# folkol/query-engines

Measured on AMD Instinct MI355X. Metric: rows/sec filter+project+group-by over 1B-row Arrow batch; % HBM roofline, higher is better.
Workload: dtype int64; 1 GPU; C4: SELECT k, SUM(a+b), COUNT(*), MIN(a), MAX(b) WHERE a > 2^19 GROUP BY k; rows_per_gpu=1000000000, groups=1024, columns=k, a, b int64 (Arrow, no nulls), parallelism=hash-sharded partial aggregate x1

## Files before the change

### include/qe_hip.h

```cpp
#ifndef QE_HIP_H
#define QE_HIP_H

#include <stddef.h>
#include <stdint.h>

#ifdef __cplusplus
extern "C" {
#endif

#define QE_ABI_VERSION 1

#define QE_OK 0
#define QE_ERR_INVALID_ARG (-1)
#define QE_ERR_UNSUPPORTED (-2)
#define QE_ERR_OOM (-3)
#define QE_ERR_DEVICE (-4)
#define QE_ERR_CAPACITY (-5)
#define QE_ERR_COMM (-6)
#define QE_NEED_EXACT 1

#define QE_TYPE_INT64 1
#define QE_TYPE_FLOAT64 2
#define QE_TYPE_BOOL 3
#define QE_TYPE_UTF8 4
#define QE_TYPE_INT32 5
#define QE_TYPE_UINT8 6
#define QE_TYPE_DATE32 7

typedef struct qe_column {
  int32_t type;
  int32_t max_len;
  int64_t length;
  uint8_t* validity;
  void* values;
  int32_t* offsets;
} qe_column;

typedef struct qe_scalar {
  int32_t type;
  int32_t is_null;
  int64_t bits;
} qe_scalar;

typedef struct qe_operand {
  const qe_column* col;
  qe_scalar lit;
} qe_operand;

typedef struct qe_ctx qe_ctx;

int qe_ctx_create(int device, void* stream, qe_ctx** out);
int qe_ctx_create_owned(int device, qe_ctx** out);
int qe_ctx_set_jit(qe_ctx* ctx, int32_t enable);
int qe_ctx_destroy(qe_ctx* ctx);
void* qe_ctx_stream(qe_ctx* ctx);
int qe_ctx_synchronize(qe_ctx* ctx);
const char* qe_last_error(void);
int qe_abi_version(void);

int qe_device_alloc(qe_ctx* ctx, size_t bytes, void** out);
int qe_device_free(qe_ctx* ctx, void* ptr);
int qe_release_cached_memory(int device);
int qe_copy_to_device(qe_ctx* ctx, void* dst, const void* src, size_t bytes);
int qe_copy_to_host(qe_ctx* ctx, void* dst, const void* src, size_t bytes);
int qe_file_to_device(qe_ctx* ctx, const char* path, int64_t offset, int64_t bytes, void* dst);

#define QE_GEN_MOD 1
#define QE_GEN_RAW 2
#define QE_GEN_UNIT53 3
#define QE_GEN_MOD_F64 4
int qe_generate(qe_ctx* ctx, qe_column* out, int32_t dist, int64_t param, uint64_t seed,
                uint64_t col, int64_t row0, int32_t null_permille);

int qe_stream_read(qe_ctx* ctx, const qe_column* cols, int32_t ncols, double* ms);
int qe_stream_read_best(qe_ctx* ctx, const qe_column* cols, int32_t ncols, int32_t reps, double* ms,
                        char* shape, int32_t shape_len);

#define QE_OP_ADD 1
#define QE_OP_SUB 2
#define QE_OP_MUL 3
#define QE_OP_DIV 4
#define QE_OP_EQ 10
#define QE_OP_NE 11
#define QE_OP_LT 12
#define QE_OP_LE 13
#define QE_OP_GT 14
#define QE_OP_GE 15
#define QE_OP_AND 20
#define QE_OP_OR 21
#define QE_OP_NOT 22
#define QE_OP_IS_NULL 23
#define QE_OP_IS_NOT_NULL 24

int qe_eval_arith(qe_ctx* ctx, int32_t op, const qe_operand* lhs, const qe_operand* rhs,
                  qe_column* out);

int qe_eval_cmp(qe_ctx* ctx, int32_t op, const qe_operand* lhs, const qe_operand* rhs,
                qe_column* out);

int qe_eval_bool(qe_ctx* ctx, int32_t op, const qe_column* lhs, const qe_column* rhs,
                 qe_column* out);

int qe_cast_utf8_to_f64(qe_ctx* ctx, const qe_column* in, qe_column* out, int64_t* error_row);

int qe_filter_count(qe_ctx* ctx, const qe_column* mask, int64_t* out_count);
int qe_filter_apply(qe_ctx* ctx, const qe_column* mask, const qe_column* inputs,
                    int32_t ncols, qe_column* outs, int64_t* out_count);
int qe_filter_apply_async(qe_ctx* ctx, const qe_column* mask, const qe_column* inputs,
                          int32_t ncols, qe_column* outs, int64_t* d_count);
int qe_eval_arith_dlen(qe_ctx* ctx, int32_t op, const qe_operand* lhs, const qe_operand* rhs,
                       qe_column* out, const int64_t* d_len);

#define QE_SORT_DESC 1
#define QE_SORT_NULLS_FIRST 2
int qe_sort_indices(qe_ctx* ctx, const qe_column* keys, const int32_t* flags, int32_t nkeys,
                    int64_t limit, qe_column* out_indices);
int qe_take(qe_ctx* ctx, const qe_column* indices, const qe_column* inputs, int32_t ncols,
            qe_column* outs, const int64_t* utf8_capacity);
int qe_sort_layout(int32_t* tile_rows, int32_t* small_max);

#define QE_JOIN_INNER 0
#define QE_JOIN_LEFT  1
typedef struct qe_join qe_join;

int qe_join_build(qe_ctx* ctx, const qe_column* key, qe_join** out);
int qe_join_destroy(qe_join* j);
int qe_join_probe(qe_join* j, const qe_column* key, int32_t kind,
                  qe_column* probe_idx, qe_column* build_idx, int64_t* pairs);
int qe_join_probe_mask(qe_join* j, const qe_column* key, int32_t anti, qe_column* mask);
int qe_join_stats(qe_join* j, int64_t* build_rows, int64_t* distinct, int64_t* max_dup, int64_t* slots);
int qe_take_or_null(qe_ctx* ctx, const qe_column* indices, const qe_column* inputs, int32_t ncols,
                    qe_column* outs, const int64_t* utf8_capacity);

#define QE_AGG_SUM 1
#define QE_AGG_MIN 2
#define QE_AGG_MAX 3
#define QE_AGG_COUNT 4
#define QE_AGG_COUNT_STAR 5
#define QE_AGG_AVG 6

typedef struct qe_global_agg {
  int64_t rows;
  int64_t count;
  int32_t type;
  int32_t valid;
  int64_t sum;
  int64_t min;
  int64_t max;
  double avg;
} qe_global_agg;
int qe_agg_global(qe_ctx* ctx, const qe_column* col, const qe_column* mask ,
                  qe_global_agg* out);
#define QE_GLOBAL_PARTIAL_BYTES 128
#define QE_GLOBAL_EXACT_BYTES 320
int qe_agg_global_partial(qe_ctx* ctx, const qe_column* col, const qe_column* mask ,
                          int64_t row_base, void* partial);
int qe_agg_global_merge(qe_ctx* ctx, int32_t type, const void* partials, int32_t n, qe_global_agg* out);
int qe_agg_global_exact_partial(qe_ctx* ctx, const qe_column* col, const qe_column* mask ,
                                void* words);
int qe_agg_global_merge_exact(qe_ctx* ctx, const void* words, int32_t n, qe_global_agg* out);

#define QE_MAX_KEYS 4
#define QE_MAX_AGGS 8
#define QE_MAX_COLS 8
#define QE_MAX_TERMS 8
#define QE_MAX_TOKENS 16

typedef struct qe_agg_desc {
  int32_t fn;
  int32_t input_type;
} qe_agg_desc;

typedef struct qe_hashagg qe_hashagg;
typedef struct qe_strdict qe_strdict;

int qe_hashagg_create(qe_ctx* ctx, int32_t nkeys, const int32_t* key_types, int32_t naggs,
                      const qe_agg_desc* aggs, int64_t expected_groups, qe_hashagg** out);
#define QE_HASHAGG_DETERMINISTIC 1
#define QE_HASHAGG_FAST_FP64 2
int qe_hashagg_create_ex(qe_ctx* ctx, int32_t nkeys, const int32_t* key_types, int32_t naggs,
                         const qe_agg_desc* aggs, int64_t expected_groups, int32_t flags, qe_hashagg** out);
int qe_hashagg_destroy(qe_hashagg* agg);
int qe_hashagg_reset(qe_hashagg* agg);

int qe_hashagg_update(qe_hashagg* agg, const qe_column* keys, const qe_column* agg_inputs,
                      const qe_column* mask);

#define QE_TOK_COL 1
#define QE_TOK_LIT 2
#define QE_TOK_ADD 3
#define QE_TOK_SUB 4
#define QE_TOK_MUL 5
#define QE_TOK_DIV 6

typedef struct qe_pred_term {
  int32_t col;
  int32_t op;
  int32_t rhs_col;
  int32_t reserved;
  qe_scalar lit;
} qe_pred_term;

typedef struct qe_token {
  int32_t op;
  int32_t arg;
  qe_scalar lit;
} qe_token;

typedef struct qe_agg_program {
  int32_t ntokens;
  int32_t reserved;
  qe_token tokens[QE_MAX_TOKENS];
} qe_agg_program;

typedef struct qe_fused_spec {
  int32_t mask_col;
  int32_t nterms;
  qe_pred_term terms[QE_MAX_TERMS];
  int32_t key_cols[QE_MAX_KEYS];
  qe_agg_program inputs[QE_MAX_AGGS];
} qe_fused_spec;

int qe_hashagg_update_fused(qe_hashagg* agg, const qe_column* cols, int32_t ncols,
                            const qe_fused_spec* spec);

typedef struct qe_select_spec {
  int32_t mask_col;
  int32_t nterms;
  qe_pred_term terms[QE_MAX_TERMS];
  int32_t nout;
  int32_t reserved;
  qe_agg_program outputs[QE_MAX_AGGS];
} qe_select_spec;
int qe_select_project(qe_ctx* ctx, const qe_column* cols, int32_t ncols, const qe_select_spec* spec,
                      qe_column* outs, int64_t* out_count);
typedef struct qe_select_pending qe_select_pending;
int qe_select_project_async(qe_ctx* ctx, const qe_column* cols, int32_t ncols, const qe_select_spec* spec,
                            qe_column* outs, qe_select_pending** pending);
int qe_select_pending_wait(qe_select_pending* pending, int64_t* out_count);
#define QE_SELECT_SCHEME_RESIDENT 1
#define QE_SELECT_SCHEME_TWOPASS 2
#define QE_SELECT_SCHEME_SCANNED 3
#define QE_SELECT_SCHEME_LOOKBACK_PERSISTENT 4
#define QE_SELECT_SCHEME_LOOKBACK_COUNTER 5
typedef struct qe_select_layout {
  int32_t scheme;
  int32_t staged;
  int32_t block;
  int32_t reserved;
  int64_t tile_rows;
  int64_t tiles;
  int64_t group_rows;
} qe_select_layout;
int qe_select_project_layout(qe_ctx* ctx, const qe_column* cols, int32_t ncols, const qe_select_spec* spec,
                             const qe_column* outs, qe_select_layout* out);

int qe_hashagg_num_groups(qe_hashagg* agg, int64_t* out);
int qe_hashagg_finalize(qe_hashagg* agg, qe_column* out_keys, qe_column* out_aggs,
                        int64_t* out_groups);
int qe_hashagg_finalize_sizes(qe_hashagg* agg, int64_t* groups, int64_t* key_bytes);
int qe_hashagg_key_bytes_bound(qe_hashagg* agg, int32_t key, int64_t* per_group);

int qe_hashagg_record_bytes(qe_hashagg* agg, int64_t* out);
int qe_hashagg_export_counts(qe_hashagg* agg, int32_t nparts, int64_t* counts);
int qe_hashagg_export(qe_hashagg* agg, int32_t nparts, void* dst);
int qe_hashagg_import(qe_hashagg* agg, const void* records, int64_t nrecords);

#define QE_KEYED_HEADER 128
int qe_hashagg_export_keyed_sizes(qe_hashagg* agg, int32_t nparts, int64_t* block_bytes);
int qe_hashagg_export_keyed(qe_hashagg* agg, int32_t nparts, void* dst);
int qe_hashagg_import_keyed(qe_hashagg* agg, const void* blocks, int32_t nblocks, const int64_t* block_bytes);
int qe_hashagg_merge(qe_hashagg* dst, qe_hashagg* src);
int qe_hashagg_bind_key_dict(qe_hashagg* agg, int32_t key, qe_strdict* dict);
int qe_hashagg_key_layout(qe_hashagg* agg, int32_t* dictionary_keyed, int32_t* device_nkeys, int32_t* device_types);

#define QE_SLOT_HEADER 64
int qe_hashagg_export_slots(qe_hashagg* agg, int32_t nparts, int64_t slot_records, void* dst);
int qe_hashagg_import_slots(qe_hashagg* agg, const void* slots, int32_t nslots, int64_t slot_records,
                            int64_t* max_count, int64_t* nrecords);
int qe_hashagg_slot_capacity(qe_hashagg* agg, int32_t world, int64_t* slot_records);

int qe_hashagg_set_async(qe_hashagg* agg, int32_t enable);

#define QE_COMM_ID_BYTES 128
typedef struct qe_comm qe_comm;
int qe_comm_unique_id(void* id );
int qe_comm_create(qe_ctx* ctx, int32_t world, int32_t rank, const void* id, qe_comm** out);
int qe_comm_destroy(qe_comm* comm);
int qe_comm_loopback_hub_create(int32_t world, void** hub);
int qe_comm_loopback_hub_destroy(void* hub);
int qe_comm_create_loopback(qe_ctx* ctx, int32_t world, int32_t rank, void* hub, qe_comm** out);
int qe_hashagg_exchange(qe_comm* comm, qe_hashagg* partial, qe_hashagg* owner, int64_t slot_records,
                        int64_t* nrecords);

int qe_hashagg_set_row_base(qe_hashagg* agg, int64_t row_base);

int qe_hashagg_last_kernel_time(qe_hashagg* agg, double* ms, int32_t* launches);
int qe_hashagg_last_kernel_signature(qe_hashagg* agg, uint64_t* sig);
int qe_hashagg_last_kernel_kind(qe_hashagg* agg, int32_t* specialized, char* note, int32_t note_len);
int qe_hashagg_last_chunk_stats(qe_hashagg* agg, int64_t* chunks, int64_t* full_chunks, int64_t* records);

int qe_strdict_create(qe_ctx* ctx, int64_t expected_distinct, qe_strdict** out);
int qe_strdict_destroy(qe_strdict* dict);
int qe_strdict_size(qe_strdict* dict, int64_t* out);
int qe_strdict_encode(qe_strdict* dict, const qe_column* in, qe_column* codes);
int qe_strdict_decode_bytes(qe_strdict* dict, const qe_column* codes, int64_t* out_bytes);
int qe_strdict_decode(qe_strdict* dict, const qe_column* codes, qe_column* out);
int qe_strdict_decode_trusted(qe_strdict* dict, const qe_column* codes, qe_column* out);
int qe_strdict_encode_packed(qe_ctx* ctx, const qe_column* in, qe_column* codes);
int qe_strdict_decode_packed(qe_ctx* ctx, const qe_column* codes, qe_column* out);
int qe_strdict_encode_tuple(qe_strdict* dict, const qe_column* keys, int32_t nkeys, qe_column* codes);
int qe_strdict_decode_tuple(qe_strdict* dict, const qe_column* codes, int32_t nkeys, qe_column* outs);
int qe_hash_partition(qe_ctx* ctx, const qe_column* cols, int32_t ncols, int32_t nparts, int32_t* part);

#ifndef ARROW_C_DATA_INTERFACE
#define ARROW_C_DATA_INTERFACE
#define ARROW_FLAG_DICTIONARY_ORDERED 1
#define ARROW_FLAG_NULLABLE 2
#define ARROW_FLAG_MAP_KEYS_SORTED 4
struct ArrowSchema {
  const char* format;
  const char* name;
  const char* metadata;
  int64_t flags;
  int64_t n_children;
  struct ArrowSchema** children;
  struct ArrowSchema* dictionary;
  void (*release)(struct ArrowSchema*);
  void* private_data;
};
struct ArrowArray {
  int64_t length;
  int64_t null_count;
  int64_t offset;
  int64_t n_buffers;
  int64_t n_children;
  const void** buffers;
  struct ArrowArray** children;
  struct ArrowArray* dictionary;
  void (*release)(struct ArrowArray*);
  void* private_data;
};
#endif
#ifndef ARROW_C_DEVICE_DATA_INTERFACE
#define ARROW_C_DEVICE_DATA_INTERFACE
typedef int32_t ArrowDeviceType;
struct ArrowDeviceArray {
  struct ArrowArray array;
  int64_t device_id;
  ArrowDeviceType device_type;
  void* sync_event;
  int64_t reserved[3];
};
#endif
#define QE_ARROW_DEVICE_CPU 1
#define QE_ARROW_DEVICE_ROCM 10
typedef struct ArrowSchema ArrowSchema;
typedef struct ArrowArray ArrowArray;
typedef struct ArrowDeviceArray ArrowDeviceArray;

typedef struct qe_batch qe_batch;
int qe_batch_import(qe_ctx* ctx, const ArrowSchema* schema, const ArrowArray* array, qe_batch** out);
int qe_batch_import_device(qe_ctx* ctx, const ArrowSchema* schema, const ArrowDeviceArray* array,
                           qe_batch** out);
int qe_batch_destroy(qe_batch* batch);
int qe_batch_num_columns(const qe_batch* batch, int32_t* ncols, int64_t* length);
int qe_batch_column(const qe_batch* batch, int32_t i, qe_column* out, const char** name);
int qe_batch_export(qe_ctx* ctx, const qe_column* cols, int32_t ncols, const char* const* names,
                    ArrowSchema* out_schema, ArrowArray* out_array);

typedef struct qe_csv_options {
  int32_t delimiter;
  int32_t has_header;
  int32_t nfields;
  int32_t flags;
  const int32_t* field_index;
} qe_csv_options;
#define QE_CSV_PARTIAL_TAIL 1
typedef struct qe_csv_table qe_csv_table;
int qe_csv_parse(qe_ctx* ctx, const uint8_t* data, int64_t nbytes, const qe_csv_options* opt,
                 qe_csv_table** out);
int qe_csv_rows(const qe_csv_table* table, int64_t* rows);
int qe_csv_consumed(const qe_csv_table* table, int64_t* bytes);
int qe_csv_column(const qe_csv_table* table, int32_t i, qe_column* out);
int qe_csv_column_bytes(const qe_csv_table* table, int32_t i, int64_t* nbytes);
int qe_csv_column_copy(const qe_csv_table* table, int32_t i, qe_column* dst);
int qe_csv_column_max_len(const qe_csv_table* table, int32_t i, int64_t* nbytes);
int qe_csv_destroy(qe_csv_table* table);
int qe_csv_record_end(const uint8_t* data, int64_t nbytes, int32_t eof, int64_t* cut);

#ifdef __cplusplus
}
#endif
#endif
```

### query-engines_amd/csrc/qe_comm.hip

```cpp
#include <dlfcn.h>
#include <rccl/rccl.h>
#include <string.h>

#include <condition_variable>
#include <mutex>
#include <string>
#include <type_traits>
#include <vector>

#include "qe_internal.hpp"

namespace {

struct Rccl {
  ncclResult_t (*get_unique_id)(ncclUniqueId*) = nullptr;
  ncclResult_t (*comm_init_rank)(ncclComm_t*, int, ncclUniqueId, int) = nullptr;
  ncclResult_t (*comm_destroy)(ncclComm_t) = nullptr;
  ncclResult_t (*send)(const void*, size_t, ncclDataType_t, int, ncclComm_t, hipStream_t) = nullptr;
  ncclResult_t (*recv)(void*, size_t, ncclDataType_t, int, ncclComm_t, hipStream_t) = nullptr;
  ncclResult_t (*group_start)() = nullptr;
  ncclResult_t (*group_end)() = nullptr;
  const char* (*error_string)(ncclResult_t) = nullptr;
  bool ok = false;
  std::string why;
};

const Rccl& rccl() {
  static Rccl r;
  static std::once_flag once;
  std::call_once(once, [] {
    void* h = nullptr;
    for (const char* name : {"librccl.so.1", "librccl.so"}) {
      h = dlopen(name, RTLD_NOW | RTLD_LOCAL);
      if (h) break;
    }
    if (!h) {
      const char* e = dlerror();
      r.why = e ? e : "librccl.so.1 not found";
      return;
    }
    bool all = true;
    auto sym = [&](auto& fp, const char* name) {
      fp = reinterpret_cast<std::remove_reference_t<decltype(fp)>>(dlsym(h, name));
      all = all && fp != nullptr;
    };
    sym(r.get_unique_id, "ncclGetUniqueId");
    sym(r.comm_init_rank, "ncclCommInitRank");
    sym(r.comm_destroy, "ncclCommDestroy");
    sym(r.send, "ncclSend");
    sym(r.recv, "ncclRecv");
    sym(r.group_start, "ncclGroupStart");
    sym(r.group_end, "ncclGroupEnd");
    sym(r.error_string, "ncclGetErrorString");
    r.ok = all;
    if (!all) r.why = "librccl is missing an entry point";
  });
  return r;
}

#define QE_NCCL(call)                                                                               \
  do {                                                                                              \
    const ncclResult_t qe_r_ = (call);                                                              \
    if (qe_r_ != ncclSuccess)                                                                       \
      return ::qe::fail(QE_ERR_COMM, "%s failed: %s", #call, rccl().error_string(qe_r_));           \
  } while (0)

}

struct qe_loop_hub {
  int32_t world = 0;
  std::mutex mu;
  std::condition_variable cv;
  int32_t arrived = 0;
  uint64_t generation = 0;
  std::vector<const uint8_t*> send;
  std::vector<const size_t*> soff, sbytes;
  std::vector<int> failed;
  void barrier() {
    std::unique_lock<std::mutex> g(mu);
    const uint64_t gen = generation;
    if (++arrived == world) {
      arrived = 0;
      ++generation;
      cv.notify_all();
    } else {
      cv.wait(g, [&] { return generation != gen; });
    }
  }
};

struct qe_comm {
  qe_ctx* ctx = nullptr;
  ncclComm_t comm = nullptr;
  qe_loop_hub* hub = nullptr;
  int32_t world = 0, rank = 0;
  uint8_t* buf = nullptr;
  size_t buf_bytes = 0;
};

using namespace qe;

namespace {

int comm_buffer(qe_comm* c, size_t bytes) {
  if (bytes <= c->buf_bytes) return QE_OK;
  dev_free(c->ctx, c->buf);
  c->buf = nullptr;
  c->buf_bytes = 0;
  QE_TRY(dev_alloc(c->ctx, bytes, (void**)&c->buf));
  c->buf_bytes = bytes;
  return QE_OK;
}

int exchange_bytes(qe_comm* c, const uint8_t* send, const size_t* soff, const size_t* sbytes, uint8_t* recv,
                   const size_t* roff, const size_t* rbytes) {
  if (c->hub) {
    qe_loop_hub* h = c->hub;
    int st = ctx_sync(c->ctx);
    h->send[c->rank] = send;
    h->soff[c->rank] = soff;
    h->sbytes[c->rank] = sbytes;
    h->failed[c->rank] = st != QE_OK;
    h->barrier();
    for (int p = 0; p < c->world && st == QE_OK; ++p)
      if (h->failed[p]) st = fail(QE_ERR_COMM, "loopback exchange: rank %d failed before the exchange", p);
    for (int p = 0; p < c->world && st == QE_OK; ++p) {
      if (h->sbytes[p][c->rank] != rbytes[p])
        st = fail(QE_ERR_COMM, "loopback exchange: rank %d sends %zu bytes to rank %d, which expects %zu", p,
                  h->sbytes[p][c->rank], c->rank, rbytes[p]);
      else if (rbytes[p] && hipMemcpyAsync(recv + roff[p], h->send[p] + h->soff[p][c->rank], rbytes[p],
                                           hipMemcpyDeviceToDevice, c->ctx->stream) != hipSuccess)
        st = fail(QE_ERR_DEVICE, "loopback exchange: copy from rank %d failed", p);
    }
    if (st == QE_OK) st = ctx_sync(c->ctx);
    h->barrier();
    return st;
  }
  const Rccl& R = rccl();
  QE_NCCL(R.group_start());
  ncclResult_t r = ncclSuccess;
  for (int p = 0; p < c->world && r == ncclSuccess; ++p) {
    if (sbytes[p]) r = R.send(send + soff[p], sbytes[p], ncclUint8, p, c->comm, c->ctx->stream);
    if (r == ncclSuccess && rbytes[p]) r = R.recv(recv + roff[p], rbytes[p], ncclUint8, p, c->comm, c->ctx->stream);
  }
  const ncclResult_t e = R.group_end();
  QE_NCCL(r);
  QE_NCCL(e);
  return QE_OK;
}

int exchange_keyed(qe_comm* c, qe_hashagg* partial, qe_hashagg* owner, int64_t* nrecords) {
  const int world = c->world;
  std::vector<int64_t> sb(world), rb(world);
  QE_TRY(qe_hashagg_export_keyed_sizes(partial, world, sb.data()));
  QE_TRY(comm_buffer(c, (size_t)2 * world * 8));
  int64_t* dsz = (int64_t*)c->buf;
  QE_HIP(hipMemcpyAsync(dsz, sb.data(), (size_t)world * 8, hipMemcpyHostToDevice, c->ctx->stream));
  std::vector<size_t> o8(world), l8(world, 8);
  for (int p = 0; p < world; ++p) o8[p] = (size_t)p * 8;
  QE_TRY(exchange_bytes(c, (const uint8_t*)dsz, o8.data(), l8.data(), (uint8_t*)(dsz + world), o8.data(), l8.data()));
  QE_HIP(hipMemcpyAsync(rb.data(), dsz + world, (size_t)world * 8, hipMemcpyDeviceToHost, c->ctx->stream));
  QE_TRY(ctx_sync(c->ctx));
  std::vector<size_t> so(world), sl(world), ro(world), rl(world);
  size_t a = 0, b = 0;
  for (int p = 0; p < world; ++p) {
    so[p] = a;
    sl[p] = (size_t)sb[p];
    a += sl[p];
    ro[p] = b;
    rl[p] = (size_t)rb[p];
    b += rl[p];
  }
  QE_TRY(comm_buffer(c, std::max<size_t>(a + b, 8)));
  uint8_t* send = c->buf;
  uint8_t* recv = c->buf + a;
  QE_TRY(qe_hashagg_export_keyed(partial, world, send));
  QE_TRY(exchange_bytes(c, send, so.data(), sl.data(), recv, ro.data(), rl.data()));
  QE_TRY(qe_hashagg_import_keyed(owner, recv, world, rb.data()));
  if (nrecords) {
    std::vector<int64_t> nrec(world, 0);
    for (int p = 0; p < world; ++p)
      if (rb[p]) QE_HIP(hipMemcpyAsync(&nrec[p], recv + ro[p] + 8, 8, hipMemcpyDeviceToHost, c->ctx->stream));
    QE_TRY(ctx_sync(c->ctx));
    int64_t n = 0;
    for (int64_t x : nrec) n += x;
    *nrecords = n;
  }
  return QE_OK;
}

}

extern "C" {

int qe_comm_unique_id(void* id) {
  QE_CHECK(id, QE_ERR_INVALID_ARG, "null id");
  const Rccl& R = rccl();
  QE_CHECK(R.ok, QE_ERR_COMM, "RCCL unavailable: %s", R.why.c_str());
  static_assert(sizeof(ncclUniqueId) == QE_COMM_ID_BYTES, "unique id size");
  ncclUniqueId u;
  QE_NCCL(R.get_unique_id(&u));
  memcpy(id, &u, sizeof u);
  return QE_OK;
}

int qe_comm_create(qe_ctx* ctx, int32_t world, int32_t rank, const void* id, qe_comm** out) {
  QE_TRY(ctx_enter(ctx));
  QE_CHECK(out && id && world >= 1 && rank >= 0 && rank < world, QE_ERR_INVALID_ARG, "bad arguments");
  const Rccl& R = rccl();
  QE_CHECK(R.ok, QE_ERR_COMM, "RCCL unavailable: %s", R.why.c_str());
  ncclUniqueId u;
  memcpy(&u, id, sizeof u);
  ncclComm_t comm = nullptr;
  QE_NCCL(R.comm_init_rank(&comm, world, u, rank));
  qe_comm* c = new qe_comm();
  c->ctx = ctx;
  c->comm = comm;
  c->world = world;
  c->rank = rank;
  *out = c;
  return QE_OK;
}

int qe_comm_destroy(qe_comm* c) {
  if (!c) return QE_OK;
  (void)hipSetDevice(c->ctx->device);
  (void)hipStreamSynchronize(c->ctx->stream);
  dev_free(c->ctx, c->buf);
  if (c->comm) (void)rccl().comm_destroy(c->comm);
  delete c;
  return QE_OK;
}

int qe_comm_loopback_hub_create(int32_t world, void** hub) {
  QE_CHECK(hub && world >= 1, QE_ERR_INVALID_ARG, "bad arguments");
  qe_loop_hub* h = new qe_loop_hub();
  h->world = world;
  h->send.assign(world, nullptr);
  h->soff.assign(world, nullptr);
  h->sbytes.assign(world, nullptr);
  h->failed.assign(world, 0);
  *hub = h;
  return QE_OK;
}

int qe_comm_loopback_hub_destroy(void* hub) {
  delete (qe_loop_hub*)hub;
  return QE_OK;
}

int qe_comm_create_loopback(qe_ctx* ctx, int32_t world, int32_t rank, void* hub, qe_comm** out) {
  QE_TRY(ctx_enter(ctx));
  qe_loop_hub* h = (qe_loop_hub*)hub;
  QE_CHECK(out && h && world == h->world && rank >= 0 && rank < world, QE_ERR_INVALID_ARG, "bad arguments");
  qe_comm* c = new qe_comm();
  c->ctx = ctx;
  c->hub = h;
  c->world = world;
  c->rank = rank;
  *out = c;
  return QE_OK;
}

int qe_hashagg_slot_capacity(qe_hashagg* h, int32_t world, int64_t* cap) {
  QE_CHECK(h && cap && world >= 1, QE_ERR_INVALID_ARG, "bad arguments");
  int64_t eg = 0;
  QE_TRY(hashagg_expected_groups(h, &eg));
  eg = std::max<int64_t>(eg, 1);
  *cap = std::min<int64_t>(eg, (3 * eg + 2 * world - 1) / (2 * world) + 32);
  return QE_OK;
}

int qe_hashagg_exchange(qe_comm* c, qe_hashagg* partial, qe_hashagg* owner, int64_t slot_records,
                        int64_t* nrecords) {
  QE_CHECK(c && partial && owner, QE_ERR_INVALID_ARG, "null argument");
  QE_TRY(ctx_enter(c->ctx));
  const int world = c->world;
  int64_t rb = 0;
  QE_TRY(qe_hashagg_record_bytes(partial, &rb));
  QE_CHECK(hashagg_ctx(partial) == c->ctx && hashagg_ctx(owner) == c->ctx, QE_ERR_INVALID_ARG,
           "partial, owner and communicator must share one qe_ctx (one stream)");
  if (keyed_dict(hashagg_info(partial).keyed) || keyed_dict(hashagg_info(owner).keyed))
    return exchange_keyed(c, partial, owner, nrecords);
  int64_t cap = slot_records;
  if (cap <= 0) QE_TRY(qe_hashagg_slot_capacity(partial, world, &cap));
  const size_t slot_bytes = (size_t)QE_SLOT_HEADER + (size_t)cap * (size_t)rb;
  QE_TRY(comm_buffer(c, 2 * (size_t)world * slot_bytes));
  uint8_t* send = c->buf;
  uint8_t* recv = c->buf + (size_t)world * slot_bytes;
  QE_TRY(qe_hashagg_export_slots(partial, world, cap, send));
  std::vector<size_t> off(world), len(world, slot_bytes);
  for (int p = 0; p < world; ++p) off[p] = (size_t)p * slot_bytes;
  QE_TRY(exchange_bytes(c, send, off.data(), len.data(), recv, off.data(), len.data()));
  int64_t mx = 0, n = 0;
  QE_TRY(qe_hashagg_import_slots(owner, recv, world, cap, &mx, &n));
  if (mx <= cap) {
    if (nrecords) *nrecords = n;
    return QE_OK;
  }
  std::vector<int64_t> counts(world);
  QE_TRY(qe_hashagg_export_counts(partial, world, counts.data()));
  int64_t total = 0;
  for (int64_t x : counts) total += x;
  QE_TRY(comm_buffer(c, (size_t)2 * world * 8 + (size_t)std::max<int64_t>(total, 1) * rb));
  int64_t* dcnt = (int64_t*)c->buf;
  QE_HIP(hipMemcpyAsync(dcnt, counts.data(), (size_t)world * 8, hipMemcpyHostToDevice, c->ctx->stream));
  std::vector<size_t> o8(world), l8(world, 8);
  for (int p = 0; p < world; ++p) o8[p] = (size_t)p * 8;
  QE_TRY(exchange_bytes(c, (const uint8_t*)dcnt, o8.data(), l8.data(), (uint8_t*)(dcnt + world), o8.data(),
                        l8.data()));
  std::vector<int64_t> rcounts(world);
  QE_HIP(hipMemcpyAsync(rcounts.data(), dcnt + world, (size_t)world * 8, hipMemcpyDeviceToHost, c->ctx->stream));
  QE_TRY(ctx_sync(c->ctx));
  int64_t rtotal = 0;
  for (int64_t x : rcounts) rtotal += x;
  const size_t head = (size_t)2 * world * 8;
  QE_TRY(comm_buffer(c, head + (size_t)(std::max<int64_t>(total, 1) + std::max<int64_t>(rtotal, 1)) * rb));
  uint8_t* srec = c->buf + head;
  uint8_t* rrec = srec + (size_t)std::max<int64_t>(total, 1) * rb;
  QE_TRY(qe_hashagg_export(partial, world, srec));
  std::vector<size_t> so(world), sl(world), ro(world), rl(world);
  size_t a = 0, b = 0;
  for (int p = 0; p < world; ++p) {
    so[p] = a;
    sl[p] = (size_t)counts[p] * rb;
    a += sl[p];
    ro[p] = b;
    rl[p] = (size_t)rcounts[p] * rb;
    b += rl[p];
  }
  QE_TRY(exchange_bytes(c, srec, so.data(), sl.data(), rrec, ro.data(), rl.data()));
  QE_TRY(qe_hashagg_import(owner, rrec, rtotal));
  if (nrecords) *nrecords = rtotal;
  return QE_OK;
}

}
```

### query-engines_amd/csrc/qe_hashagg.hip

```cpp
#include <map>
#include <memory>
#include <mutex>

#include "qe_internal.hpp"

namespace qe {

constexpr int HA_THREADS = 512;

__device__ __forceinline__ qi64* lds_keys(char* smem) { return (qi64*)smem; }

__device__ __forceinline__ void lds_init(const Plan& P, char* smem) {
  const int SS = (1 << P.lds_log2) + 2;
  qi64* keys = lds_keys(smem);
  qu32* cst = (qu32*)(smem + P.off_cstar);
  for (int s = threadIdx.x; s < SS; s += blockDim.x) {
    keys[s] = EMPTY_KEY;
    cst[s] = 0;
  }
#pragma unroll
  for (int j = 0; j < QE_MAX_AGGS; ++j) {
    if (j >= P.naggs) break;
    const DAgg& a = P.aggs[j];
    if (a.acc != ACC_NONE) {
// ... 626 lines not shown
      gadd_cstar(P.t, gs, 1);
      const qu64 row = (qu64)(P.row_base + lr);
      for (int j = 0; j < P.naggs; ++j) {
        const DAgg& a = P.aggs[j];
        if (a.pkind == 0) continue;
        bool valid;
        const qi64 x = a.pkind == 2 ? eval_program<NC>(a, R, r, valid) : eval_fast<NC>(a, R, r, valid);
        if (!valid) continue;
        const RowVal rv = row_partial(a.acc, x, row);
        gcombine(P.t, a.acc, j, gs, rv.acc, 1, rv.i0, rv.i1, rv.i2, rv.i3);
      }
    }
  }
}

template <int NC, bool USE_LDS>
__global__ void __launch_bounds__(HA_THREADS, 4) k_hashagg(const Plan P) {
  extern __shared__ __attribute__((aligned(16))) char smem[];
  if (USE_LDS) {
    lds_init(P, smem);
    __syncthreads();
  }
  const int lane = threadIdx.x & 63;
  const qi64 wave = (blockIdx.x * (qi64)blockDim.x + threadIdx.x) >> 6;
  const qi64 stride = (((qi64)gridDim.x * blockDim.x) >> 6) * 256;
  ColRegs<NC> cur, nxt;
  qi64 base = wave * 256;
  if (base < P.n) load_cols<NC>(P, base, lane, base + 256 <= P.n, cur);
  for (; base < P.n; base += stride) {
    const qi64 nb = base + stride;
    if (nb < P.n) load_cols<NC>(P, nb, lane, nb + 256 <= P.n, nxt);
    process_step<NC, USE_LDS>(P, smem, cur, base, lane);
    cur = nxt;
  }
  if (USE_LDS) {
    __syncthreads();
    lds_flush(P, smem);
  }
}

struct AggMeta {
  qi32 naggs;
  qi32 fn[QE_MAX_AGGS];
  qi32 acc[QE_MAX_AGGS];
  qi32 nn_implicit;
  qi32 any_x;
};

__device__ __forceinline__ qu64 slot_nn(const DTable& t, const AggMeta& m, int j, qu64 s) {
  return ((m.nn_implicit >> j) & 1) ? t.cstar[s] : t.nn[j][s];
}

__global__ void __launch_bounds__(1024) k_part_slices(const qi64* __restrict__ off, qi32 np, qi64 g, qi64 cw,
                                                      qi64* __restrict__ out) {
  __shared__ qi64 s_sum[1024];
  const int per = (np + 1023) / 1024;
  const int b0 = threadIdx.x * per;
  qi64 cnt = 0;
  for (int i = 0; i < per; ++i) {
    const int b = b0 + i;
    if (b < np) cnt += (off[(qi64)(b + 1) * g] - off[(qi64)b * g] + cw - 1) / cw;
  }
  s_sum[threadIdx.x] = cnt;
  __syncthreads();
  for (int d = 1; d < 1024; d <<= 1) {
    const qi64 v = (int)threadIdx.x >= d ? s_sum[threadIdx.x - d] : 0;
    __syncthreads();
    s_sum[threadIdx.x] += v;
    __syncthreads();
  }
  qi64 pos = s_sum[threadIdx.x] - cnt;
  for (int i = 0; i < per; ++i) {
    const int b = b0 + i;
    if (b >= np) break;
    const qi64 s = off[(qi64)b * g], e = off[(qi64)(b + 1) * g];
    const qi64 ns = (e - s + cw - 1) / cw;
    for (qi64 k = 0; k < ns; ++k, ++pos) {
      const qi64 lo = s + k * cw;
      out[2 + 2 * pos] = lo;
      out[3 + 2 * pos] = (lo + cw < e ? lo + cw : e) | (ns == 1 ? PART_EXCL : 0);
    }
  }
  if (threadIdx.x == 1023) out[0] = s_sum[1023];
}

constexpr int CHUNK_PER_WG = 1024;
__global__ void __launch_bounds__(256) k_chunk_hist(const qi64* __restrict__ meta, qi32 np, qu32* __restrict__ cnt,
                                                   unsigned long long* __restrict__ rec) {
  __shared__ qu32 s_cnt[CHUNK_PLAN_MAXB];
  __shared__ unsigned long long s_rec[CHUNK_PLAN_MAXB];
  const qi64 C = meta[0], lo = (qi64)blockIdx.x * CHUNK_PER_WG;
  if (lo >= C) return;
  const qi64 hi = lo + CHUNK_PER_WG < C ? lo + CHUNK_PER_WG : C;
  for (int b = threadIdx.x; b < np; b += blockDim.x) {
    s_cnt[b] = 0;
    s_rec[b] = 0;
  }
  __syncthreads();
  for (qi64 c = lo + threadIdx.x; c < hi; c += blockDim.x) {
    const qi64 w = meta[1 + c];
    if (w < 0) continue;
    const int b = (int)(w >> 32);
    atomicAdd(&s_cnt[b], 1u);
    atomicAdd(&s_rec[b], (unsigned long long)(w & 0xFFFFFFFFll));
  }
  __syncthreads();
  for (int b = threadIdx.x; b < np; b += blockDim.x)
    if (s_cnt[b]) {
      atomicAdd(&cnt[b], s_cnt[b]);
      atomicAdd(&rec[b], s_rec[b]);
    }
}

__global__ void __launch_bounds__(1024) k_chunk_slices(const qi64* __restrict__ meta, qi32 np, qi64 tmax,
                                                      const qu32* __restrict__ cnt,
                                                      const unsigned long long* __restrict__ rec,
                                                      qi64* __restrict__ out, qu32* __restrict__ base) {
  __shared__ qu32 s_a[1024], s_b[1024];
  __shared__ unsigned long long s_r[1024];
  const int t = threadIdx.x;
  const qu32 c = t < np ? cnt[t] : 0u;
  s_r[t] = t < np ? rec[t] : 0ull;
  s_a[t] = c;
  __syncthreads();
  for (int d = 512; d > 0; d >>= 1) {
    if (t < d) {
      s_r[t] += s_r[t + d];
      s_a[t] += s_a[t + d];
    }
    __syncthreads();
  }
  const qi64 C = (qi64)s_a[0], R = (qi64)s_r[0];
  (void)meta;
  __syncthreads();
  const qi64 target = max((qi64)np, min(tmax, R >> 15));
  const qi64 cpc = max((qi64)1, (5 * C + 4 * target - 1) / (4 * target));
  const qu32 ns = (qu32)((c + cpc - 1) / cpc);
  s_a[t] = c;
  s_b[t] = ns;
  __syncthreads();
  for (int d = 1; d < 1024; d <<= 1) {
    const qu32 xa = t >= d ? s_a[t - d] : 0u, xb = t >= d ? s_b[t - d] : 0u;
    __syncthreads();
    s_a[t] += xa;
    s_b[t] += xb;
    __syncthreads();
  }
  if (t < np) {
    const qi64 s0 = s_a[t] - c, e0 = s0 + c, sl = s_b[t] - ns;
    base[t] = (qu32)s0;
    for (qi64 k = 0; k < ns; ++k) {
      const qi64 lo = s0 + k * cpc;
      out[2 + 2 * (sl + k)] = lo;
      out[3 + 2 * (sl + k)] = (lo + cpc < e0 ? lo + cpc : e0) | (ns == 1 ? PART_EXCL : 0);
    }
  }
  if (t == 1023) out[0] = s_b[1023];
}

__global__ void __launch_bounds__(256) k_chunk_place(const qi64* __restrict__ meta, qi32 np,
                                                    const qu32* __restrict__ base, qu32* __restrict__ cur,
                                                    qi32* __restrict__ sorted) {
  constexpr int PER = CHUNK_PER_WG / 256;
  __shared__ qu32 s_cnt[CHUNK_PLAN_MAXB];
  const qi64 C = meta[0], lo = (qi64)blockIdx.x * CHUNK_PER_WG;
  if (lo >= C) return;
  for (int b = threadIdx.x; b < np; b += blockDim.x) s_cnt[b] = 0;
  __syncthreads();
  int bk[PER];
  qu32 rk[PER];
#pragma unroll
  for (int i = 0; i < PER; ++i) {
    const qi64 c = lo + threadIdx.x + 256 * i;
    bk[i] = -1;
    if (c < C && meta[1 + c] >= 0) {
      bk[i] = (int)(meta[1 + c] >> 32);
      rk[i] = atomicAdd(&s_cnt[bk[i]], 1u);
    }
  }
  __syncthreads();
  for (int b = threadIdx.x; b < np; b += blockDim.x)
    if (s_cnt[b]) s_cnt[b] = base[b] + atomicAdd(&cur[b], s_cnt[b]);
  __syncthreads();
#pragma unroll
  for (int i = 0; i < PER; ++i)
    if (bk[i] >= 0) sorted[s_cnt[bk[i]] + rk[i]] = (qi32)(lo + threadIdx.x + 256 * i);
}

__global__ void k_spill_plan(const qi64* __restrict__ meta, qi64 tmax, qi64* __restrict__ out, qi32* __restrict__ sorted) {
  const qi64 C = meta[0];
  const qi64 c = (qi64)blockIdx.x * blockDim.x + threadIdx.x;
  if (c < C) sorted[c] = (qi32)c;
  if (blockIdx.x != 0) return;
  qi64 target = (C * PART_CH) >> 15;
  target = target < 1 ? 1 : (target > tmax ? tmax : target);
  const qi64 cpc = (C + target - 1) / target > 0 ? (C + target - 1) / target : 1;
  const qi64 ns = (C + cpc - 1) / cpc;
  for (qi64 k = threadIdx.x; k < ns; k += blockDim.x) {
    const qi64 lo = k * cpc;
    out[2 + 2 * k] = lo;
    out[3 + 2 * k] = (lo + cpc < C ? lo + cpc : C) | (ns == 1 ? PART_EXCL : 0);
  }
  if (threadIdx.x == 0) out[0] = ns;
}

__global__ void k_table_init(DTable t, AggMeta m, qu64* zero_ctl, int reset) {
  const qu64 SS = t.cap + 2;
  if (zero_ctl && blockIdx.x == 0 && threadIdx.x < 8) zero_ctl[threadIdx.x] = 0;
  for (qu64 s = blockIdx.x * (qu64)blockDim.x + threadIdx.x; s < SS; s += (qu64)gridDim.x * blockDim.x) {
    t.keys[s] = EMPTY_KEY;
    t.cstar[s] = 0;
    for (int j = 0; j < m.naggs; ++j) {
      if (reset && m.acc[j] == ACC_SUM_X && (t.idx[j][3 * SS + s] & FX_EXT))
        for (int w = 0; w < FXE_WORDS; ++w) t.ext[j][s * FXE_WORDS + w] = 0;
      t.acc[j][s] = acc_identity(m.acc[j]);
      t.nn[j][s] = 0;
      if (acc_has_idx(m.acc[j]))
        for (int k = 0; k < 4; ++k) t.idx[j][k * SS + s] = idx_identity(m.acc[j]);
    }
  }
}

__global__ void k_nn_materialize(DTable t, qi32 mask) {
  const qu64 SS = t.cap + 2;
  for (qu64 s = blockIdx.x * (qu64)blockDim.x + threadIdx.x; s < SS; s += (qu64)gridDim.x * blockDim.x)
    for (int j = 0; j < QE_MAX_AGGS; ++j)
      if ((mask >> j) & 1) t.nn[j][s] = t.cstar[s];
}

__device__ __forceinline__ bool gslot_occupied(const DTable& t, qu64 s) {
  return s < t.cap ? t.keys[s] != EMPTY_KEY : t.cstar[s] > 0;
}

__device__ __forceinline__ void wg_newg_begin(qu32* newg) {
  if (threadIdx.x == 0) *newg = 0;
  __syncthreads();
}
__device__ __forceinline__ void wg_newg_end(qu32* newg, qu64* ctl) {
  __syncthreads();
  if (threadIdx.x == 0 && *newg) atomicAdd((unsigned long long*)&ctl[0], (unsigned long long)*newg);
}

__global__ void k_rehash(DTable src, DTable dst, AggMeta m) {
  __shared__ qu32 newg;
  wg_newg_begin(&newg);
  const qu64 SS = src.cap + 2;
  for (qu64 s = blockIdx.x * (qu64)blockDim.x + threadIdx.x; s < SS; s += (qu64)gridDim.x * blockDim.x) {
    if (!gslot_occupied(src, s)) continue;
    const bool knull = s == src.cap;
    const qi64 key = knull ? 0 : (s == src.cap + 1 ? EMPTY_KEY : src.keys[s]);
    qu64 d;
    if (!gtable_find_wg(dst, key, knull, d, &newg)) {
      atomicAdd((unsigned long long*)&dst.ctl[3], 1ull);
      continue;
    }
    gadd_cstar(dst, d, src.cstar[s]);
    for (int j = 0; j < m.naggs; ++j) {
      DAgg a{};
      a.fn = m.fn[j];
      a.acc = m.acc[j];
      qu64 i[4] = {~0ull, ~0ull, ~0ull, ~0ull};
      if (acc_has_idx(a.acc))
        for (int k = 0; k < 4; ++k) i[k] = src.idx[j][k * SS + s];
      gcombine(dst, a.acc, j, d, src.acc[j][s], slot_nn(src, m, j, s), i[0], i[1], i[2], i[3]);
      if (a.acc == ACC_SUM_X && (i[3] & FX_EXT))
        fxe_add_words<true>(dst.ext[j] + d * FXE_WORDS, 0, src.ext[j] + s * FXE_WORDS, FXE_WORDS);
    }
  }
  wg_newg_end(&newg, dst.ctl);
}

__device__ void import_record(const qu8* __restrict__ rec, DTable& dst, const AggMeta& m, qu32* newg) {
  const qi64 key = ((const qi64*)rec)[0];
  const bool knull = ((const qu64*)rec)[1] & 1;
  const qu64 c = ((const qu64*)rec)[2];
  qu64 d;
  if (!gtable_find_wg(dst, key, knull, d, newg)) {
    atomicAdd((unsigned long long*)&dst.ctl[3], 1ull);
    return;
  }
  gadd_cstar(dst, d, c);
  int off = 24;
  for (int j = 0; j < m.naggs; ++j) {
    DAgg a{};
    a.fn = m.fn[j];
    a.acc = m.acc[j];
    const qu64* f = (const qu64*)(rec + off);
    if (a.fn != QE_AGG_COUNT_STAR) {
      if (acc_has_idx(a.acc)) gcombine(dst, a.acc, j, d, (qi64)f[0], f[1], f[2], f[3], f[4], f[5]);
      else gcombine(dst, a.acc, j, d, (qi64)f[0], f[1], ~0ull, ~0ull, ~0ull, ~0ull);
    }
    off += agg_rec_bytes(a.acc);
  }
}

__global__ void k_import(const qu8* __restrict__ recs, qi64 nrec, qi32 rec_bytes, DTable dst, AggMeta m) {
  __shared__ qu32 newg;
  wg_newg_begin(&newg);
  for (qi64 r = blockIdx.x * (qi64)blockDim.x + threadIdx.x; r < nrec; r += (qi64)gridDim.x * blockDim.x)
    import_record(recs + r * rec_bytes, dst, m, &newg);
  wg_newg_end(&newg, dst.ctl);
}

__global__ void k_import_slots(const qu8* __restrict__ slots, qi32 nslots, qi64 slot_records, qi32 rec_bytes,
                               DTable dst, AggMeta m) {
  __shared__ qu32 newg;
  __shared__ qi32 s_ok;
  const qu64 slot_bytes = QE_SLOT_HEADER + (qu64)slot_records * rec_bytes;
  if (threadIdx.x < 64) {
    qu64 mx = 0, tot = 0;
    for (int i = threadIdx.x; i < nslots; i += 64) {
      const qu64* hd = (const qu64*)(slots + (qu64)i * slot_bytes);
      mx = hd[1] > mx ? hd[1] : mx;
      tot += hd[0] < (qu64)slot_records ? hd[0] : (qu64)slot_records;
    }
    for (int off = 32; off > 0; off >>= 1) {
      const qu64 o = __shfl_xor(mx, off);
      mx = o > mx ? o : mx;
      tot += __shfl_xor(tot, off);
    }
    if (threadIdx.x == 0) {
      s_ok = mx <= (qu64)slot_records;
      if (blockIdx.x == 0) {
        dst.ctl[4] = mx;
        dst.ctl[5] = tot;
      }
    }
  }
  wg_newg_begin(&newg);
  if (s_ok) {
    const qi64 total = (qi64)nslots * slot_records;
    for (qi64 r = blockIdx.x * (qi64)blockDim.x + threadIdx.x; r < total; r += (qi64)gridDim.x * blockDim.x) {
      const qi64 sl = r / slot_records, i = r - sl * slot_records;
      const qu8* base = slots + (qu64)sl * slot_bytes;
      if ((qu64)i >= ((const qu64*)base)[0]) continue;
      import_record(base + QE_SLOT_HEADER + (qu64)i * rec_bytes, dst, m, &newg);
    }
  }
  wg_newg_end(&newg, dst.ctl);
}

__device__ __forceinline__ qu32 partition_of(qi64 key, bool knull, qi32 nparts) {
  const qu64 h = fmix64((qu64)key ^ (knull ? NULL_SALT : 0ull));
  return (qu32)(((h >> 32) * (qu64)nparts) >> 32);
}

__device__ __forceinline__ qu64 wave_cursor(unsigned long long* cursor, bool has, qu32 p, qu32 mult = 1) {
  const int lane = threadIdx.x & 63;
  const qu64 lt = lane ? (~0ull >> (64 - lane)) : 0ull;
  qu64 todo = __ballot(has);
  qu64 pos = 0;
  while (todo) {
    const int leader = __ffsll((long long)todo) - 1;
    const qu32 lp = (qu32)__shfl((int)p, leader);
    const qu64 same = __ballot(has && p == lp);
    qu64 base = 0;
    if (lane == leader) base = atomicAdd(&cursor[lp], (unsigned long long)__popcll(same) * mult);
    base = (qu64)__shfl((long long)base, leader);
    if (has && p == lp) pos = base + (qu64)__popcll(same & lt) * mult;
    todo &= ~same;
  }
  return pos;
}

__device__ __forceinline__ bool slot_has_ext(const DTable& t, const AggMeta& m, qu64 s) {
  bool e = false;
  for (int j = 0; j < m.naggs; ++j)
    if (m.acc[j] == ACC_SUM_X) e = e || (t.idx[j][3 * (t.cap + 2) + s] & FX_EXT) != 0;
  return e;
}

__global__ void k_export_count(DTable t, AggMeta m, qi32 nparts, unsigned long long* counts) {
  const qu64 SS = t.cap + 2;
  const qu64 stride = (qu64)gridDim.x * blockDim.x;
  for (qu64 s0 = blockIdx.x * (qu64)blockDim.x; s0 < SS; s0 += stride) {
    const qu64 s = s0 + threadIdx.x;
    const bool has = s < SS && gslot_occupied(t, s);
    const bool knull = s == t.cap;
    const qi64 key = !has ? 0 : knull ? 0 : (s == t.cap + 1 ? EMPTY_KEY : t.keys[s]);
    const qu32 p = has ? partition_of(key, knull, nparts) : 0;
    (void)wave_cursor(counts, has, p);
    if (m.any_x) (void)wave_cursor(counts, has && slot_has_ext(t, m, s), p, FXE_CHUNKS);
  }
}

__device__ void write_record(qu8* rec, const DTable& t, const AggMeta& m, qu64 s, qi64 key, bool knull) {
  const qu64 SS = t.cap + 2;
  write_record_head(rec, key, knull, t.cstar[s]);
  int off = 24;
  for (int j = 0; j < m.naggs; ++j) {
    qu64* f = (qu64*)(rec + off);
    f[0] = (qu64)t.acc[j][s];
    f[1] = slot_nn(t, m, j, s);
    if (acc_has_idx(m.acc[j]))
      for (int k = 0; k < 4; ++k) f[2 + k] = t.idx[j][k * SS + s];
    off += agg_rec_bytes(m.acc[j]);
  }
}

__device__ void write_chunk_record(qu8* rec, const DTable& t, const AggMeta& m, qu64 s, qi64 key, bool knull,
                                   int c) {
  const qu64 SS = t.cap + 2;
  write_record_head(rec, key, knull, 0);
  int off = 24;
  for (int j = 0; j < m.naggs; ++j) {
    qu64* f = (qu64*)(rec + off);
    const int acc = m.acc[j];
    f[0] = (qu64)acc_identity(acc);
    f[1] = 0;
    if (acc_has_idx(acc))
      for (int k = 0; k < 4; ++k) f[2 + k] = idx_identity(acc);
    if (acc == ACC_SUM_X && (t.idx[j][3 * SS + s] & FX_EXT)) {
      const qu64* e = t.ext[j] + s * FXE_WORDS + 4 * c;
      const int n = c == FXE_CHUNKS - 1 ? FXE_WORDS - 4 * c : 4;
      f[0] = e[0];
      for (int k = 1; k < n; ++k) f[1 + k] = e[k];
      f[5] = FX_CHUNK | ((qu64)c << 8);
    }
    off += agg_rec_bytes(acc);
  }
}

__global__ void k_counts_to_cursors(unsigned long long* c, qi32 nparts) {
  if (threadIdx.x == 0) {
    unsigned long long run = 0;
    for (int p = 0; p < nparts; ++p) {
      const unsigned long long x = c[p];
      c[p] = run;
      run += x;
    }
  }
}

__global__ void k_export(DTable t, AggMeta m, qi32 nparts, qi32 rec_bytes, unsigned long long* cursor,
                         qu8* __restrict__ dst) {
  const qu64 SS = t.cap + 2;
  const qu64 stride = (qu64)gridDim.x * blockDim.x;
  for (qu64 s0 = blockIdx.x * (qu64)blockDim.x; s0 < SS; s0 += stride) {
    const qu64 s = s0 + threadIdx.x;
    const bool has = s < SS && gslot_occupied(t, s);
    const bool knull = s == t.cap;
    const qi64 key = !has ? 0 : knull ? 0 : (s == t.cap + 1 ? EMPTY_KEY : t.keys[s]);
    const qu32 p = has ? partition_of(key, knull, nparts) : 0;
    const qu64 pos = wave_cursor(cursor, has, p);
    if (has) write_record(dst + pos * (qu64)rec_bytes, t, m, s, key, knull);
    if (m.any_x) {
      const bool ext = has && slot_has_ext(t, m, s);
      const qu64 pe = wave_cursor(cursor, ext, p, FXE_CHUNKS);
      if (ext)
        for (int c = 0; c < FXE_CHUNKS; ++c) write_chunk_record(dst + (pe + c) * (qu64)rec_bytes, t, m, s, key, knull, c);
    }
  }
}

__global__ void k_export_slots(DTable t, AggMeta m, qi32 nparts, qi32 rec_bytes, qi64 slot_records,
                               unsigned long long* cursor, qu8* __restrict__ dst) {
  const qu64 SS = t.cap + 2;
  const qu64 slot_bytes = QE_SLOT_HEADER + (qu64)slot_records * rec_bytes;
  const qu64 stride = (qu64)gridDim.x * blockDim.x;
  for (qu64 s0 = blockIdx.x * (qu64)blockDim.x; s0 < SS; s0 += stride) {
    const qu64 s = s0 + threadIdx.x;
    const bool has = s < SS && gslot_occupied(t, s);
    const bool knull = s == t.cap;
    const qi64 key = !has ? 0 : knull ? 0 : (s == t.cap + 1 ? EMPTY_KEY : t.keys[s]);
    const qu32 p = has ? partition_of(key, knull, nparts) : 0;
    const qu64 pos = wave_cursor(cursor, has, p);
    qu8* base = dst + p * slot_bytes + QE_SLOT_HEADER;
    if (has && pos < (qu64)slot_records) write_record(base + pos * (qu64)rec_bytes, t, m, s, key, knull);
    if (m.any_x) {
      const bool ext = has && slot_has_ext(t, m, s);
      const qu64 pe = wave_cursor(cursor, ext, p, FXE_CHUNKS);
      if (ext)
        for (int c = 0; c < FXE_CHUNKS; ++c)
          if (pe + c < (qu64)slot_records) write_chunk_record(base + (pe + c) * (qu64)rec_bytes, t, m, s, key, knull, c);
    }
  }
}

__global__ void k_slot_headers(const unsigned long long* __restrict__ cursor, qi32 nparts, qu64 slot_bytes,
                               qu8* __restrict__ dst, const qu64* __restrict__ guard) {
  qu64 mx = 0;
  for (int p = threadIdx.x; p < nparts; p += blockDim.x) mx = cursor[p] > mx ? cursor[p] : mx;
  for (int off = 32; off > 0; off >>= 1) {
    const qu64 o = __shfl_xor(mx, off);
    mx = o > mx ? o : mx;
  }
  if (guard && (guard[1] | guard[2] | guard[3])) mx = 1ull << 62;
  for (int p = threadIdx.x; p < nparts; p += blockDim.x) {
    qu64* hd = (qu64*)(dst + (qu64)p * slot_bytes);
    hd[0] = cursor[p];
    hd[1] = mx;
    for (int w = 2; w < QE_SLOT_HEADER / 8; ++w) hd[w] = 0;
  }
}

__global__ void k_occ_count(DTable t, qi64* __restrict__ tile_counts, qi32 tile_slots) {
  __shared__ qi64 part[4];
  const qu64 SS = t.cap + 2;
  const qu64 s0 = (qu64)blockIdx.x * tile_slots;
  qi64 c = 0;
  for (int i = threadIdx.x; i < tile_slots; i += blockDim.x) {
    const qu64 s = s0 + i;
    if (s < SS && gslot_occupied(t, s)) ++c;
  }
  for (int off = 32; off > 0; off >>= 1) c += __shfl_xor(c, off);
  if ((threadIdx.x & 63) == 0) part[threadIdx.x >> 6] = c;
  __syncthreads();
  if (threadIdx.x == 0) tile_counts[blockIdx.x] = part[0] + part[1] + part[2] + part[3];
}

struct OutCols {
  qe_column keys[QE_MAX_KEYS];
  qe_column aggs[QE_MAX_AGGS];
};

__device__ __forceinline__ void set_bit(qu8* bm, qi64 i, bool v) {
  if (v) atomicOr((qu32*)bm + (i >> 5), 1u << (i & 31));
}

__device__ __forceinline__ void store_typed(void* p, qi32 type, qi64 i, qi64 x) {
  switch (type) {
    case QE_TYPE_INT64:
    case QE_TYPE_FLOAT64: ((qi64*)p)[i] = x; break;
    case QE_TYPE_INT32:
    case QE_TYPE_DATE32: ((qi32*)p)[i] = (qi32)x; break;
    default: ((qu8*)p)[i] = (qu8)x;
  }
}

constexpr int FS_WORDS = 512;
__device__ __forceinline__ void put_bit(qu8* gbm, qu32* lbits, int col, qi64 o, bool v) {
  if (!v) return;
  if (lbits) atomicOr(lbits + col * FS_WORDS + (o >> 5), 1u << (o & 31));
  else set_bit(gbm, o, true);
}

__device__ __forceinline__ double fx_sum(const DTable& t, int j, qu64 s, qi64 acc) {
  const qu64 SS = t.cap + 2;
  const qu64* ix = t.idx[j];
  return fx_result((qu64)acc, ix[s], ix[SS + s], ix[2 * SS + s], ix[3 * SS + s], t.ext[j] + s * FXE_WORDS);
}

__device__ __forceinline__ void finalize_slot(const DTable& t, const AggMeta& m, const KeyMeta& km,
                                              const OutCols& out, qu64 s, qi64 o, qu32* lbits = nullptr) {
  const qu64 SS = t.cap + 2;
  const bool knull = s == t.cap;
  const qi64 key = knull ? 0 : (s == t.cap + 1 ? EMPTY_KEY : t.keys[s]);
  if (km.mode == 1) {
    store_typed(out.keys[0].values, km.type[0], o, key);
    if (out.keys[0].validity) put_bit(out.keys[0].validity, lbits, 0, o, !knull);
  } else if (km.mode == 2) {
    for (int k = 0; k < km.nkeys; ++k) {
      const bool isn = (key >> km.nullbit[k]) & 1;
      qi64 x = (key >> km.shift[k]) & km.fmask[k];
      if (km.type[k] == QE_TYPE_INT32 || km.type[k] == QE_TYPE_DATE32) x = (qi64)(qi32)x;
      store_typed(out.keys[k].values, km.type[k], o, x);
      if (out.keys[k].validity) put_bit(out.keys[k].validity, lbits, k, o, !isn);
    }
  }
  const qu64 cst = t.cstar[s];
#pragma unroll 1
  for (int j = 0; j < m.naggs; ++j) {
    if (!out.aggs[j].values) continue;
    const qu64 nn = slot_nn(t, m, j, s);
    const qi64 acc = t.acc[j][s];
    qi64 val = 0;
    bool valid = nn > 0;
    switch (m.fn[j]) {
      case QE_AGG_COUNT: val = (qi64)nn; valid = true; break;
      case QE_AGG_COUNT_STAR: val = (qi64)cst; valid = true; break;
      case QE_AGG_AVG:
        if (m.acc[j] == ACC_SUM_X)
          val = f64_bits(fx_sum(t, j, s, acc) / (double)nn);
        else
          val = f64_bits(bits_f64(acc) / (double)nn);
        break;
      default:
        if (m.acc[j] == ACC_SUM_X) {
          val = f64_bits(fx_sum(t, j, s, acc));
        } else if (acc_is_f64mm(m.acc[j])) {
          const qu64 i0 = t.idx[j][s], i1 = t.idx[j][SS + s];
          const qu64 i2 = t.idx[j][2 * SS + s], i3 = t.idx[j][3 * SS + s];
          if (i1 != ~0ull && i1 == i0) {
            val = 0x7FF8000000000000ll;
          } else {
            const double d = okey_f64(acc);
            val = d == 0.0 ? f64_bits(i2 < i3 ? -0.0 : 0.0) : f64_bits(d);
          }
        } else {
          val = acc;
        }
    }
    ((qi64*)out.aggs[j].values)[o] = valid ? val : 0;
    if (out.aggs[j].validity) put_bit(out.aggs[j].validity, lbits, QE_MAX_KEYS + j, o, valid);
  }
}

__global__ void k_finalize(DTable t, AggMeta m, KeyMeta km, const qi64* __restrict__ tile_offsets,
                           qi32 tile_slots, OutCols out) {
  __shared__ int wtot[4];
  const qu64 SS = t.cap + 2;
  const int lane = threadIdx.x & 63, wid = threadIdx.x >> 6;
  const qu64 lt = lane ? (~0ull >> (64 - lane)) : 0ull;
  qi64 base = tile_offsets[blockIdx.x];
  for (int it = 0; it < tile_slots; it += blockDim.x) {
    const qu64 s = (qu64)blockIdx.x * tile_slots + it + threadIdx.x;
    const bool occ = (it + (int)threadIdx.x) < tile_slots && s < SS && gslot_occupied(t, s);
    const qu64 b = __ballot(occ);
    if (lane == 0) wtot[wid] = __popcll(b);
    __syncthreads();
    int woff = 0, btot = 0;
    for (int w = 0; w < 4; ++w) {
      woff += w < wid ? wtot[w] : 0;
      btot += wtot[w];
    }
    if (occ) finalize_slot(t, m, km, out, s, base + woff + __popcll(b & lt));
    base += btot;
    __syncthreads();
  }
}

constexpr int FS_THREADS = 1024, FS_PER = 16, FS_WAVES = FS_THREADS / 64;
static_assert(FS_THREADS * FS_PER / 2 / 32 <= FS_WORDS, "LDS bitmaps hold every group of a small table");
__global__ void __launch_bounds__(FS_THREADS) k_finalize_small(DTable t, AggMeta m, KeyMeta km, OutCols out,
                                                               qi64 groups) {
  __shared__ qi32 wcnt[FS_PER][FS_WAVES];
  __shared__ qu64 wbal[FS_PER][FS_WAVES];
  __shared__ qu32 lbits[(QE_MAX_KEYS + QE_MAX_AGGS) * FS_WORDS];
  const qu64 SS = t.cap + 2;
  const int tid = threadIdx.x, lane = tid & 63, wid = tid >> 6;
  const qu64 lt = lane ? (~0ull >> (64 - lane)) : 0ull;
  const int words = (int)((groups + 31) >> 5);
  for (int w = tid; w < (QE_MAX_KEYS + QE_MAX_AGGS) * FS_WORDS; w += FS_THREADS) lbits[w] = 0;
  qu32 occ = 0;
#pragma unroll
  for (int i = 0; i < FS_PER; ++i) {
    const qu64 s = (qu64)i * FS_THREADS + tid;
    if (s < SS && gslot_occupied(t, s)) occ |= 1u << i;
  }
#pragma unroll
  for (int i = 0; i < FS_PER; ++i) {
    const qu64 b = __ballot((occ >> i) & 1);
    if (lane == 0) {
      wbal[i][wid] = b;
      wcnt[i][wid] = __popcll(b);
    }
  }
  __syncthreads();
  static_assert(FS_PER * FS_WAVES == 4 * 64, "four (chunk, wave) counts per lane");
  if (wid == 0) {
    qi32* flat = &wcnt[0][0];
    const qi32 c0 = flat[4 * lane], c1 = flat[4 * lane + 1], c2 = flat[4 * lane + 2], c3 = flat[4 * lane + 3];
    const qi32 sum = c0 + c1 + c2 + c3;
    qi32 inc = sum;
#pragma unroll
    for (int d = 1; d < 64; d <<= 1) {
      const qi32 y = __shfl_up(inc, d);
      if (lane >= d) inc += y;
    }
    const qi32 ex = inc - sum;
    flat[4 * lane] = ex;
    flat[4 * lane + 1] = ex + c0;
    flat[4 * lane + 2] = ex + c0 + c1;
    flat[4 * lane + 3] = ex + c0 + c1 + c2;
  }
  __syncthreads();
  while (occ) {
    const int i = __ffs(occ) - 1;
    occ &= occ - 1;
    const qi64 o = wcnt[i][wid] + __popcll(wbal[i][wid] & lt);
    finalize_slot(t, m, km, out, (qu64)i * FS_THREADS + tid, o, lbits);
  }
  __syncthreads();
  for (int w = tid; w < words; w += FS_THREADS) {
    for (int k = 0; k < QE_MAX_KEYS; ++k)
      if (k < km.nkeys && out.keys[k].validity) ((qu32*)out.keys[k].validity)[w] = lbits[k * FS_WORDS + w];
    for (int j = 0; j < m.naggs; ++j)
      if (out.aggs[j].validity) ((qu32*)out.aggs[j].validity)[w] = lbits[(QE_MAX_KEYS + j) * FS_WORDS + w];
  }
}

}

using namespace qe;

struct qe_hashagg {
  qe_ctx* ctx = nullptr;
  int32_t nkeys = 0;
  int32_t key_types[QE_MAX_KEYS] = {};
  int32_t naggs = 0;
  qe_agg_desc aggs[QE_MAX_AGGS] = {};
  int32_t acc[QE_MAX_AGGS] = {};
  KeyMeta km{};
  int32_t rec_bytes = 0;
  int32_t nn_implicit = 0;
  int64_t row_base = 0;
  int64_t known_groups = 0;
  void* table_mem = nullptr;
  DTable t{};
  qu64* ctl = nullptr;
  int32_t lds_log2 = 0;
  int32_t lds_log2_min = 0;
  int64_t expected_groups = 0;
  int64_t create_groups = 0;
  int grid = 0;
  int64_t* part_cnt = nullptr;
  size_t part_cnt_bytes = 0;
  int64_t chunk_cap = 0;
  uint8_t* part_rec = nullptr;
  size_t part_rec_bytes = 0;
  int64_t* part_slc = nullptr;
  size_t part_slc_bytes = 0;
  bool part_wide = false;
  bool narrow_failed = false;
  bool compact_off = false;
  uint8_t* ovf = nullptr;
  uint64_t ovf_cap = 0;
  uint32_t* defer[2] = {nullptr, nullptr};
  size_t defer_words = 0;
  bool defer_dirty[2] = {false, false};
  bool ctl_rows_clean = false;
  hipEvent_t ev[2] = {nullptr, nullptr};
  double last_kernel_ms = 0.0;
  int last_launches = 0;
  int last_specialized = 0;
  uint64_t last_sig = 0;
  std::string jit_note;
  bool async = false;
  bool pending = false;
  std::unique_ptr<qe::Plan> pend_plan;
  size_t pend_lds = 0;
  int pend_out_i = 0;
  uint64_t* ctl_pin = nullptr;
  hipEvent_t ev_ctl = nullptr;
  int poisoned = 0;
  std::string poison_msg;
  qe::Keyed* keyed = nullptr;
  int32_t flags = 0;
  uint64_t version = 0;
};

namespace qe {

int hashagg_expected_groups(const qe_hashagg* h, int64_t* out) {
  QE_CHECK(h && out, QE_ERR_INVALID_ARG, "null argument");
  *out = h->create_groups;
  return QE_OK;
}

qe_ctx* hashagg_ctx(const qe_hashagg* h) { return h ? h->ctx : nullptr; }

HashaggInfo hashagg_info(const qe_hashagg* h) {
  HashaggInfo I{};
  I.ctx = h->ctx;
  I.km = h->km;
  I.rec_bytes = h->rec_bytes;
  I.naggs = h->naggs;
  I.flags = h->flags;
  for (int j = 0; j < h->naggs; ++j) I.aggs[j] = h->aggs[j];
  I.version = h->version;
  I.ctl = (uint64_t*)h->ctl;
  I.keyed = h->keyed;
  return I;
}

static AggMeta agg_meta(const qe_hashagg* h) {
  AggMeta m{};
  m.naggs = h->naggs;
  for (int j = 0; j < h->naggs; ++j) {
    m.fn[j] = h->aggs[j].fn;
    m.acc[j] = h->acc[j];
    m.any_x = m.any_x || h->acc[j] == ACC_SUM_X;
  }
  m.nn_implicit = h->nn_implicit;
  return m;
}

static int32_t all_nn_bits(const qe_hashagg* h) {
  if (!agg_knobs().nn_implicit) return 0;
  int32_t b = 0;
  for (int j = 0; j < h->naggs; ++j)
    if (h->aggs[j].fn != QE_AGG_COUNT_STAR) b |= 1 << j;
  return b;
}

static int nn_materialize(qe_hashagg* h, int32_t mask) {
  mask &= h->nn_implicit;
  if (!mask) return QE_OK;
  const int grid = (int)std::min<uint64_t>(div_up(h->t.cap + 2, 256), 4096);
  hipLaunchKernelGGL(k_nn_materialize, dim3(grid), dim3(256), 0, h->ctx->stream, h->t, (qi32)mask);
  QE_TRY(launch_check("k_nn_materialize"));
  h->nn_implicit &= ~mask;
  return QE_OK;
}

static size_t table_bytes(const qe_hashagg* h, uint64_t cap) {
  const uint64_t SS = cap + 2;
  size_t b = 16 * SS;
  for (int j = 0; j < h->naggs; ++j)
    b += (16 + (acc_has_idx(h->acc[j]) ? 32 : 0) + (h->acc[j] == ACC_SUM_X ? 8 * FXE_WORDS : 0)) * SS;
  return b;
}

static int table_alloc(qe_hashagg* h, uint64_t cap, void** mem, DTable* t, qu64* zero_ctl = nullptr) {
  const size_t bytes = table_bytes(h, cap);
  QE_TRY(dev_alloc(h->ctx, bytes, mem));
  const uint64_t SS = cap + 2;
  char* p = (char*)*mem;
  *t = DTable{};
  t->keys = (qi64*)p;
  p += 8 * SS;
  t->cstar = (qu64*)p;
  p += 8 * SS;
  for (int j = 0; j < h->naggs; ++j) {
    t->acc[j] = (qi64*)p;
    p += 8 * SS;
    t->nn[j] = (qu64*)p;
    p += 8 * SS;
    if (acc_has_idx(h->acc[j])) {
      t->idx[j] = (qu64*)p;
      p += 32 * SS;
    }
  }
  char* e0 = p;
  for (int j = 0; j < h->naggs; ++j)
    if (h->acc[j] == ACC_SUM_X) {
      t->ext[j] = (qu64*)p;
      p += 8 * FXE_WORDS * SS;
    }
  if (p > e0) QE_HIP(hipMemsetAsync(e0, 0, (size_t)(p - e0), h->ctx->stream));
  t->cap = cap;
  t->ctl = h->ctl;
  const int grid = (int)std::min<uint64_t>(div_up(SS, 256), 4096);
  hipLaunchKernelGGL(k_table_init, dim3(grid), dim3(256), 0, h->ctx->stream, *t, agg_meta(h), zero_ctl, 0);
  return launch_check("k_table_init");
}

static int read_ctl(qe_hashagg* h, uint64_t out[8]) {
  void* p;
  QE_TRY(ctx_pinned(h->ctx, 64, &p));
  QE_HIP(hipMemcpyAsync(p, h->ctl, 64, hipMemcpyDeviceToHost, h->ctx->stream));
  QE_TRY(ctx_sync(h->ctx));
  memcpy(out, p, 64);
  QE_CHECK((out[3] & CTL_KEY_TOO_LONG) == 0, QE_ERR_INVALID_ARG,
           "a UTF8 group key is longer than its column's max_len promised (qe_column.max_len)");
  QE_CHECK(out[3] == 0, QE_ERR_CAPACITY, "hash aggregate lost %llu groups (probe limit or overflow area)",
           (unsigned long long)out[3]);
  return QE_OK;
}

static uint64_t next_pow2(uint64_t x) {
  uint64_t p = 1;
  while (p < x) p <<= 1;
  return p;
}

static int table_grow(qe_hashagg* h, uint64_t want_cap) {
  const uint64_t cap = next_pow2(want_cap);
  if (cap <= h->t.cap) return QE_OK;
  void* mem;
  DTable nt;
  QE_TRY(table_alloc(h, cap, &mem, &nt));
  QE_HIP(hipMemsetAsync(h->ctl, 0, 8, h->ctx->stream));
  const int grid = (int)std::min<uint64_t>(div_up(h->t.cap + 2, 256), 8192);
  hipLaunchKernelGGL(k_rehash, dim3(grid), dim3(256), 0, h->ctx->stream, h->t, nt, agg_meta(h));
  QE_TRY(launch_check("k_rehash"));
  uint64_t c[8];
  QE_TRY(read_ctl(h, c));
  QE_CHECK(c[3] == 0, QE_ERR_CAPACITY, "hash table rehash lost %llu groups", (unsigned long long)c[3]);
  dev_free(h->ctx, h->table_mem);
  h->table_mem = mem;
  h->t = nt;
  return QE_OK;
}

static int import_records(qe_hashagg* h, const void* recs, int64_t nrec) {
  if (nrec <= 0) return QE_OK;
  const int grid = (int)std::min<uint64_t>(div_up((uint64_t)nrec, 256), 8192);
  hipLaunchKernelGGL(k_import, dim3(grid), dim3(256), 0, h->ctx->stream, (const uint8_t*)recs, nrec, h->rec_bytes,
                     h->t, agg_meta(h));
  QE_TRY(launch_check("k_import"));
  uint64_t c[8];
  QE_TRY(read_ctl(h, c));
  QE_CHECK(c[3] == 0, QE_ERR_CAPACITY, "hash table import lost %llu groups", (unsigned long long)c[3]);
  return QE_OK;
}

static int ensure_defer(qe_hashagg* h, int64_t n) {
  const size_t words = (size_t)div_up((uint64_t)n, 32);
  if (words <= h->defer_words) return QE_OK;
  for (int i = 0; i < 2; ++i) {
    dev_free(h->ctx, h->defer[i]);
    h->defer[i] = nullptr;
  }
  for (int i = 0; i < 2; ++i) {
    QE_TRY(dev_alloc(h->ctx, words * 4, (void**)&h->defer[i]));
    h->defer_dirty[i] = true;
  }
  h->defer_words = words;
  return QE_OK;
}

int compile_inputs(const qe_column* cols, int32_t ncols, int32_t mask_col, int32_t nterms, const qe_pred_term* terms,
                   Plan* P, bool* col_f64) {
  *P = Plan{};
  QE_CHECK(ncols >= 1 && ncols <= QE_MAX_COLS, QE_ERR_UNSUPPORTED, "fused plan takes 1..%d columns (got %d)",
           QE_MAX_COLS, ncols);
  const int64_t n = cols[0].length;
  for (int c = 0; c < ncols; ++c) {
    const qe_column& k = cols[c];
    QE_CHECK(k.length == n, QE_ERR_INVALID_ARG, "column %d has %lld rows, column 0 %lld", c, (long long)k.length,
             (long long)n);
    const int32_t kind = kind_of(k.type);
    QE_CHECK(kind >= K_I64 && kind <= K_BOOL, QE_ERR_UNSUPPORTED, "column %d: type %d not supported", c, k.type);
    QE_CHECK(k.values || n == 0, QE_ERR_INVALID_ARG, "column %d: null values", c);
    P->cols[c] = DCol{k.values, k.validity, kind, 0};
    col_f64[c] = k.type == QE_TYPE_FLOAT64;
  }
  P->ncols = ncols;
  P->all8 = 1;
  for (int c = 0; c < ncols; ++c) P->all8 &= (cols[c].type == QE_TYPE_INT64 || cols[c].type == QE_TYPE_FLOAT64) ? 1 : 0;
  P->n = n;
  P->mask_col = mask_col;
  if (mask_col >= 0) {
    QE_CHECK(mask_col < ncols && cols[mask_col].type == QE_TYPE_BOOL, QE_ERR_INVALID_ARG,
             "mask_col must name a BOOL column");
  }
  QE_CHECK(nterms >= 0 && nterms <= QE_MAX_TERMS, QE_ERR_UNSUPPORTED, "too many predicate terms");
  P->nterms = nterms;
  for (int i = 0; i < nterms; ++i) {
    const qe_pred_term& s = terms[i];
    DTerm& d = P->terms[i];
    QE_CHECK(s.col >= 0 && s.col < ncols && is_fixed(cols[s.col].type), QE_ERR_INVALID_ARG, "term %d: bad lhs column", i);
    QE_CHECK(s.op >= QE_OP_EQ && s.op <= QE_OP_GE, QE_ERR_INVALID_ARG, "term %d: bad comparison op", i);
    d.lhs = s.col;
    d.op = s.op;
    d.lhs_f = col_f64[s.col];
    d.rhs = s.rhs_col;
    if (s.rhs_col >= 0) {
      QE_CHECK(s.rhs_col < ncols && is_fixed(cols[s.rhs_col].type), QE_ERR_INVALID_ARG, "term %d: bad rhs column", i);
      d.rhs_f = col_f64[s.rhs_col];
      d.f64 = d.lhs_f || d.rhs_f;
    } else {
      QE_CHECK(s.lit.type == QE_TYPE_INT64 || s.lit.type == QE_TYPE_FLOAT64, QE_ERR_UNSUPPORTED,
               "term %d: literal type", i);
      const bool lf = s.lit.type == QE_TYPE_FLOAT64;
      d.f64 = d.lhs_f || lf;
      d.rhs_f = 1;
      d.lit_null = s.lit.is_null;
      d.lit = (d.f64 && !lf) ? f64_bits((double)s.lit.bits) : s.lit.bits;
    }
  }
  return QE_OK;
}

int compile_program(const qe_column* cols, int32_t ncols, const bool* col_f64, const qe_agg_program& pg, int j,
                    DAgg* a, bool* is_f, bool* nullable) {
  QE_CHECK(pg.ntokens >= 1 && pg.ntokens <= QE_MAX_TOKENS, QE_ERR_INVALID_ARG, "expression %d: empty program", j);
  bool st_f[QE_MAX_TOKENS + 4];
  int depth = 0, nt = 0;
  *nullable = false;
  auto emit = [&](int32_t op, int32_t arg, int64_t lit, int32_t lit_null, int32_t lit_f64 = 0) -> int {
    QE_CHECK(nt < QE_MAX_TOKENS, QE_ERR_UNSUPPORTED, "expression %d: program too long after type promotion", j);
    a->tok[nt++] = DTok{(short)op, (char)lit_null, (char)lit_f64, arg, lit};
    return QE_OK;
  };
  for (int t = 0; t < pg.ntokens; ++t) {
    const qe_token& tk = pg.tokens[t];
    if (tk.op == QE_TOK_COL) {
      QE_CHECK(tk.arg >= 0 && tk.arg < ncols && is_fixed(cols[tk.arg].type), QE_ERR_INVALID_ARG,
               "expression %d: bad column slot %d", j, tk.arg);
      QE_CHECK(depth < 4, QE_ERR_UNSUPPORTED, "expression %d: deeper than 4", j);
      QE_TRY(emit(T_COL, tk.arg, 0, 0));
      st_f[depth++] = col_f64[tk.arg];
      *nullable = *nullable || cols[tk.arg].validity != nullptr;
    } else if (tk.op == QE_TOK_LIT) {
      QE_CHECK(tk.lit.type == QE_TYPE_INT64 || tk.lit.type == QE_TYPE_FLOAT64, QE_ERR_UNSUPPORTED,
               "expression %d: literal type", j);
      QE_CHECK(depth < 4, QE_ERR_UNSUPPORTED, "expression %d: deeper than 4", j);
      QE_TRY(emit(T_LIT, 0, tk.lit.bits, tk.lit.is_null, tk.lit.type == QE_TYPE_FLOAT64 ? 1 : 0));
      st_f[depth++] = tk.lit.type == QE_TYPE_FLOAT64;
      *nullable = *nullable || tk.lit.is_null;
// ... 737 lines not shown
    return code;
  };
  int32_t dev_types[QE_MAX_KEYS] = {};
  {
    int32_t dn = 0;
    const int st = keyed_create(ctx, nkeys, key_types, expected_groups > 0 ? expected_groups : 1024, &h->keyed, &dn,
                                dev_types);
    if (st != QE_OK) return bail(st);
    nkeys = dn;
    key_types = dev_types;
  }
  h->nkeys = nkeys;
  if (nkeys == 0) {
    h->km.mode = 0;
  } else if (nkeys == 1 && (key_types[0] == QE_TYPE_INT64 || key_types[0] == QE_TYPE_FLOAT64)) {
    h->km.mode = 1;
  } else {
    h->km.mode = 2;
    int bit = 0;
    for (int k = 0; k < nkeys; ++k) {
      int w;
      switch (key_types[k]) {
        case QE_TYPE_INT32:
        case QE_TYPE_DATE32: w = 32; break;
        case QE_TYPE_UINT8: w = 8; break;
        default:
          return bail(fail(QE_ERR_UNSUPPORTED,
                           "group key %d: type %d cannot be packed (multi-key groups take uint8/int32/date32)", k,
                           key_types[k]));
      }
      h->km.shift[k] = bit;
      h->km.fmask[k] = (int64_t)((1ull << w) - 1);
      bit += w;
      h->km.nullbit[k] = bit;
      bit += 1;
    }
    if (bit > 63) return bail(fail(QE_ERR_UNSUPPORTED, "group keys need %d bits (max 63)", bit));
  }
  h->km.nkeys = nkeys;
  for (int k = 0; k < nkeys; ++k) {
    h->key_types[k] = key_types[k];
    h->km.type[k] = key_types[k];
  }
  h->rec_bytes = 24;
  for (int j = 0; j < naggs; ++j) {
    const qe_agg_desc& d = aggs[j];
    h->aggs[j] = d;
    const bool f = d.input_type == QE_TYPE_FLOAT64;
    const bool i = d.input_type == QE_TYPE_INT64 || d.input_type == QE_TYPE_INT32 ||
                   d.input_type == QE_TYPE_DATE32 || d.input_type == QE_TYPE_UINT8;
    if (d.fn != QE_AGG_COUNT_STAR && d.fn != QE_AGG_COUNT && !i && !f)
      return bail(fail(QE_ERR_UNSUPPORTED, "aggregate %d: input type %d (int64/int32/date32/uint8/fp64 only)", j,
                       d.input_type));
    switch (d.fn) {
      case QE_AGG_SUM: h->acc[j] = f ? (det ? ACC_SUM_X : ACC_SUM_F) : ACC_SUM_I; break;
      case QE_AGG_MIN: h->acc[j] = f ? ACC_MIN_F : ACC_MIN_I; break;
      case QE_AGG_MAX: h->acc[j] = f ? ACC_MAX_F : ACC_MAX_I; break;
      case QE_AGG_AVG: h->acc[j] = det ? ACC_SUM_X : ACC_SUM_F; break;
      case QE_AGG_COUNT:
      case QE_AGG_COUNT_STAR: h->acc[j] = ACC_NONE; break;
      default: return bail(fail(QE_ERR_UNSUPPORTED, "aggregate %d: unknown function %d", j, d.fn));
    }
    h->rec_bytes += agg_rec_bytes(h->acc[j]);
  }
  if (hipEventCreate(&h->ev[0]) != hipSuccess || hipEventCreate(&h->ev[1]) != hipSuccess ||
      hipEventCreateWithFlags(&h->ev_ctl, hipEventDisableTiming) != hipSuccess)
    return bail(fail(QE_ERR_DEVICE, "hipEventCreate failed"));
  if (pinned_slot_alloc(&h->ctl_pin) != QE_OK) return bail(QE_ERR_OOM);
  if (dev_alloc(ctx, 64, (void**)&h->ctl) != QE_OK) return bail(fail(QE_ERR_OOM, "control allocation failed"));
  const int64_t eg = expected_groups > 0 ? expected_groups : 1024;
  h->expected_groups = eg;
  h->create_groups = eg;
  const LdsRange lr = lds_table_range(eg, h->acc, naggs, !ctx->jit, lds_budget(ctx));
  h->lds_log2 = lr.log2;
  h->lds_log2_min = lr.log2_min;
  const int per_cu = h->lds_log2 ? std::max<int>(1, std::min<int>(8, (int)((160 * 1024) / lds_bytes_min(h->acc, naggs, h->lds_log2, !ctx->jit)))) : 8;
  h->grid = ctx->num_cus * per_cu;
  if (h->lds_log2) {
    h->ovf_cap = (uint64_t)h->grid * (((uint64_t)1 << h->lds_log2) + 2);
    if (dev_alloc(ctx, h->ovf_cap * h->rec_bytes, (void**)&h->ovf) != QE_OK) {
      dev_free(ctx, h->ctl);
      return bail(fail(QE_ERR_OOM, "overflow area allocation failed"));
    }
  }
  const int st = table_alloc(h, std::max<uint64_t>(1024, next_pow2((uint64_t)(2 * eg))), &h->table_mem, &h->t, h->ctl);
  h->nn_implicit = all_nn_bits(h);
  if (st != QE_OK) {
    dev_free(ctx, h->ovf);
    dev_free(ctx, h->ctl);
    return bail(st);
  }
  h->ctl_rows_clean = true;
  *out = h;
  return QE_OK;
}

int qe_hashagg_destroy(qe_hashagg* h) {
  if (!h) return QE_OK;
  (void)hipSetDevice(h->ctx->device);
  qe_ctx* ctx = h->ctx;
  void* bufs[] = {h->table_mem, h->ctl, h->ovf, h->part_cnt, h->part_rec, h->part_slc, h->defer[0], h->defer[1]};
  for (void* b : bufs) dev_free(ctx, b);
  if (h->keyed) keyed_destroy(ctx, h->keyed);
  for (int i = 0; i < 2; ++i) {
    if (h->ev[i]) (void)hipEventDestroy(h->ev[i]);
  }
  if (h->ev_ctl) (void)hipEventDestroy(h->ev_ctl);
  pinned_slot_free(h->ctl_pin, ctx->stream);
  delete h;
  return QE_OK;
}

int qe_hashagg_last_kernel_kind(qe_hashagg* h, int32_t* specialized, char* note, int32_t note_len) {
  QE_CHECK(h && specialized, QE_ERR_INVALID_ARG, "null argument");
  *specialized = h->last_specialized;
  if (note && note_len > 0) {
    strncpy(note, h->jit_note.c_str(), (size_t)note_len - 1);
    note[note_len - 1] = 0;
  }
  return QE_OK;
}

int qe_hashagg_last_kernel_signature(qe_hashagg* h, uint64_t* sig) {
  QE_CHECK(h && sig, QE_ERR_INVALID_ARG, "null argument");
  *sig = h->last_sig;
  return QE_OK;
}

int qe_hashagg_last_kernel_time(qe_hashagg* h, double* ms, int32_t* launches) {
  QE_CHECK(h && ms, QE_ERR_INVALID_ARG, "null argument");
  QE_TRY(ctx_enter(h->ctx));
  QE_TRY(settle_pending(h));
  *ms = h->last_kernel_ms;
  if (launches) *launches = h->last_launches;
  return QE_OK;
}

int qe_hashagg_last_chunk_stats(qe_hashagg* h, int64_t* chunks, int64_t* full_chunks, int64_t* records) {
  QE_CHECK(h && chunks && full_chunks && records, QE_ERR_INVALID_ARG, "null argument");
  QE_TRY(ctx_enter(h->ctx));
  QE_TRY(settle_pending(h));
  *chunks = *full_chunks = *records = 0;
  if (h->chunk_cap <= 0 || !h->part_cnt) return QE_OK;
  QE_TRY(ctx_sync(h->ctx));
  int64_t ids = 0;
  QE_HIP(hipMemcpy(&ids, h->part_cnt, 8, hipMemcpyDeviceToHost));
  ids = std::max<int64_t>(0, std::min<int64_t>(ids, h->chunk_cap));
  std::vector<int64_t> meta((size_t)ids);
  if (ids) QE_HIP(hipMemcpy(meta.data(), h->part_cnt + 1, (size_t)ids * 8, hipMemcpyDeviceToHost));
  for (const int64_t w : meta) {
    if (w < 0) continue;
    const int64_t fill = w & 0xFFFFFFFFll;
    *chunks += 1;
    *full_chunks += fill == PART_CH ? 1 : 0;
    *records += fill;
  }
  return QE_OK;
}

int qe_hashagg_set_async(qe_hashagg* h, int32_t enable) {
  QE_CHECK(h, QE_ERR_INVALID_ARG, "null state");
  QE_TRY(ctx_enter(h->ctx));
  if (!enable) QE_TRY(settle_pending(h));
  h->async = enable != 0;
  return QE_OK;
}

int qe_hashagg_reset(qe_hashagg* h) {
  QE_CHECK(h, QE_ERR_INVALID_ARG, "null state");
  QE_TRY(ctx_enter(h->ctx));
  if (h->pending) {
    h->pending = false;
    h->defer_dirty[h->pend_out_i] = true;
  }
  h->poisoned = 0;
  h->poison_msg.clear();
  const int grid = (int)std::min<uint64_t>(div_up(h->t.cap + 2, 256), 4096);
  hipLaunchKernelGGL(k_table_init, dim3(grid), dim3(256), 0, h->ctx->stream, h->t, agg_meta(h), (qu64*)h->ctl, 1);
  QE_TRY(launch_check("k_table_init"));
  h->nn_implicit = all_nn_bits(h);
  h->ctl_rows_clean = true;
  h->row_base = 0;
  h->known_groups = 0;
  ++h->version;
  return QE_OK;
}

int qe_hashagg_set_row_base(qe_hashagg* h, int64_t row_base) {
  QE_CHECK(h && row_base >= 0, QE_ERR_INVALID_ARG, "bad arguments");
  h->row_base = row_base;
  return QE_OK;
}

static_assert(sizeof(Plan) <= 4096, "kernel argument must stay under 4 KiB");

int qe_hashagg_update_fused(qe_hashagg* h, const qe_column* cols, int32_t ncols, const qe_fused_spec* spec) {
  QE_CHECK(h && cols && spec, QE_ERR_INVALID_ARG, "null argument");
  QE_TRY(ctx_enter(h->ctx));
  if (keyed_dict(h->keyed)) return keyed_update_fused(h, cols, ncols, spec);
  return hashagg_update_fused_raw(h, cols, ncols, spec);
}

int qe_hashagg_update(qe_hashagg* h, const qe_column* keys, const qe_column* agg_inputs, const qe_column* mask) {
  QE_CHECK(h, QE_ERR_INVALID_ARG, "null state");
  QE_TRY(ctx_enter(h->ctx));
  QE_CHECK(h->nkeys == 0 || keys, QE_ERR_INVALID_ARG, "null keys");
  if (keyed_dict(h->keyed)) return keyed_update(h, keys, agg_inputs, mask);
  return hashagg_update_raw(h, keys, agg_inputs, mask);
}

}

namespace qe {

int hashagg_update_fused_raw(qe_hashagg* h, const qe_column* cols, int32_t ncols, const qe_fused_spec* spec) {
  Plan P;
  QE_TRY(compile_plan(h, cols, ncols, spec, &P));
  ++h->version;
  return run_update(h, P);
}

int hashagg_update_raw(qe_hashagg* h, const qe_column* keys, const qe_column* agg_inputs, const qe_column* mask) {
  QE_CHECK(h->naggs == 0 || agg_inputs, QE_ERR_INVALID_ARG, "null agg_inputs");
  qe_column cols[QE_MAX_COLS];
  int ncols = 0;
  int64_t n = -1;
  auto slot_of = [&](const qe_column& c, int* slot) -> int {
    if (n < 0) n = c.length;
    QE_CHECK(c.length == n, QE_ERR_INVALID_ARG, "input columns differ in length (%lld vs %lld)",
             (long long)c.length, (long long)n);
    for (int i = 0; i < ncols; ++i)
      if (cols[i].values == c.values && cols[i].validity == c.validity && cols[i].type == c.type) {
        *slot = i;
        return QE_OK;
      }
    QE_CHECK(ncols < QE_MAX_COLS, QE_ERR_UNSUPPORTED, "more than %d distinct input columns", QE_MAX_COLS);
    cols[ncols] = c;
    *slot = ncols++;
    return QE_OK;
  };
  qe_fused_spec spec;
  memset(&spec, 0, sizeof(spec));
  spec.mask_col = -1;
  for (int k = 0; k < h->nkeys; ++k) QE_TRY(slot_of(keys[k], &spec.key_cols[k]));
  for (int j = 0; j < h->naggs; ++j) {
    if (h->aggs[j].fn == QE_AGG_COUNT_STAR) continue;
    int s;
    QE_TRY(slot_of(agg_inputs[j], &s));
    spec.inputs[j].ntokens = 1;
    spec.inputs[j].tokens[0].op = QE_TOK_COL;
    spec.inputs[j].tokens[0].arg = s;
  }
  if (mask) QE_TRY(slot_of(*mask, &spec.mask_col));
  if (ncols == 0) {
    for (int j = 0; j < h->naggs && ncols == 0; ++j) {
      const qe_column& c = agg_inputs[j];
      if (h->aggs[j].fn != QE_AGG_COUNT_STAR || c.type == 0) continue;
      qe_column r = c;
      if (c.type == QE_TYPE_UTF8) {
        QE_CHECK(c.offsets || c.length == 0, QE_ERR_INVALID_ARG, "COUNT(*) row source: null offsets");
        r.type = QE_TYPE_INT32;
        r.values = c.offsets;
        r.offsets = nullptr;
      }
      int s;
      QE_TRY(slot_of(r, &s));
    }
    if (ncols == 0) return fail(QE_ERR_INVALID_ARG, "update needs at least one input column");
  }
  Plan P;
  QE_TRY(compile_plan(h, cols, ncols, &spec, &P));
  ++h->version;
  return run_update(h, P);
}

}

extern "C" {

int qe_hashagg_num_groups(qe_hashagg* h, int64_t* out) {
  QE_CHECK(h && out, QE_ERR_INVALID_ARG, "null argument");
  QE_TRY(ctx_enter(h->ctx));
  QE_TRY(settle_pending(h));
  if (h->known_groups >= 0) {
    *out = h->known_groups;
    return QE_OK;
  }
  uint64_t c[8];
  QE_TRY(read_ctl(h, c));
  QE_CHECK(c[3] == 0, QE_ERR_CAPACITY, "hash table lost %llu groups", (unsigned long long)c[3]);
  *out = h->known_groups = (int64_t)c[0];
  return QE_OK;
}

int qe_hashagg_finalize(qe_hashagg* h, qe_column* out_keys, qe_column* out_aggs, int64_t* out_groups) {
  QE_CHECK(h, QE_ERR_INVALID_ARG, "null state");
  QE_TRY(ctx_enter(h->ctx));
  if (keyed_dict(h->keyed)) return keyed_finalize(h, out_keys, out_aggs, out_groups);
  return hashagg_finalize_raw(h, out_keys, out_aggs, out_groups, false);
}

}

int qe::hashagg_finalize_raw(qe_hashagg* h, qe_column* out_keys, qe_column* out_aggs, int64_t* out_groups,
                             bool keys_only) {
  qe_ctx* ctx = h->ctx;
  int64_t groups;
  QE_TRY(qe_hashagg_num_groups(h, &groups));
  if (out_groups) *out_groups = groups;
  const bool small = h->t.cap + 2 <= (uint64_t)FS_THREADS * FS_PER && groups <= (int64_t)FS_WORDS * 32;
  OutCols oc{};
  for (int k = 0; k < h->nkeys; ++k) {
    QE_CHECK(out_keys, QE_ERR_INVALID_ARG, "null out_keys");
    const qe_column& c = out_keys[k];
    QE_CHECK(c.type == h->key_types[k], QE_ERR_INVALID_ARG, "key output %d: type %d, expected %d", k, c.type,
             h->key_types[k]);
    QE_CHECK(c.length >= groups && (c.values || groups == 0), QE_ERR_CAPACITY, "key output %d holds %lld rows, need %lld",
             k, (long long)c.length, (long long)groups);
    QE_CHECK(!c.validity || ((uintptr_t)c.validity & 3) == 0, QE_ERR_INVALID_ARG, "validity must be 4-byte aligned");
    oc.keys[k] = c;
    if (c.validity && !small) QE_HIP(hipMemsetAsync(c.validity, 0, div_up((uint64_t)groups, 32) * 4, ctx->stream));
  }
  for (int j = 0; j < h->naggs && !keys_only; ++j) {
    QE_CHECK(out_aggs, QE_ERR_INVALID_ARG, "null out_aggs");
    const qe_column& c = out_aggs[j];
    const int fn = h->aggs[j].fn;
    const int32_t want = (fn == QE_AGG_COUNT || fn == QE_AGG_COUNT_STAR) ? QE_TYPE_INT64
                         : (fn == QE_AGG_AVG || h->aggs[j].input_type == QE_TYPE_FLOAT64) ? QE_TYPE_FLOAT64
                                                                                          : QE_TYPE_INT64;
    QE_CHECK(c.type == want, QE_ERR_INVALID_ARG, "aggregate output %d: type %d, expected %d", j, c.type, want);
    QE_CHECK(c.length >= groups && (c.values || groups == 0), QE_ERR_CAPACITY,
             "aggregate output %d holds %lld rows, need %lld", j, (long long)c.length, (long long)groups);
    QE_CHECK(!c.validity || ((uintptr_t)c.validity & 3) == 0, QE_ERR_INVALID_ARG, "validity must be 4-byte aligned");
    oc.aggs[j] = c;
    if (c.validity && !small) QE_HIP(hipMemsetAsync(c.validity, 0, div_up((uint64_t)groups, 32) * 4, ctx->stream));
  }
  for (int k = 0; k < h->nkeys; ++k) out_keys[k].length = groups;
  for (int j = 0; j < h->naggs && !keys_only; ++j) out_aggs[j].length = groups;
  if (groups == 0) return QE_OK;
  if (small) {
    hipLaunchKernelGGL(k_finalize_small, dim3(1), dim3(FS_THREADS), 0, ctx->stream, h->t, agg_meta(h), h->km, oc,
                       (qi64)groups);
    QE_TRY(launch_check("k_finalize_small"));
    return QE_OK;
  }
  const int32_t tile_slots = 256;
  const uint64_t SS = h->t.cap + 2;
  const int64_t ntiles = (int64_t)div_up(SS, tile_slots);
  void* s;
  QE_TRY(ctx_scratch(ctx, (size_t)(2 * ntiles + 1) * 8, &s));
  int64_t* counts = (int64_t*)s;
  int64_t* offs = counts + ntiles;
  hipLaunchKernelGGL(k_occ_count, dim3((unsigned)ntiles), dim3(256), 0, ctx->stream, h->t, (qi64*)counts, tile_slots);
  QE_TRY(launch_check("k_occ_count"));
  QE_TRY(exclusive_scan_i64(ctx, counts, offs, ntiles));
  hipLaunchKernelGGL(k_finalize, dim3((unsigned)ntiles), dim3(256), 0, ctx->stream, h->t, agg_meta(h), h->km, (const qi64*)offs,
                     tile_slots, oc);
  QE_TRY(launch_check("k_finalize"));
  return QE_OK;
}

namespace {
int refuse_dict_records(const qe_hashagg* h) {
  QE_CHECK(!keyed_dict(h->keyed), QE_ERR_UNSUPPORTED,
           "dictionary-keyed state (UTF8 / key-tuple codes are local to it): merge by key content with "
           "qe_hashagg_merge or qe_hashagg_export_keyed / qe_hashagg_import_keyed");
  return QE_OK;
}
}

extern "C" {

int qe_hashagg_record_bytes(qe_hashagg* h, int64_t* out) {
  QE_CHECK(h && out, QE_ERR_INVALID_ARG, "null argument");
  *out = h->rec_bytes;
  return QE_OK;
}

int qe_hashagg_export_counts(qe_hashagg* h, int32_t nparts, int64_t* counts) {
  QE_CHECK(h && counts && nparts >= 1, QE_ERR_INVALID_ARG, "bad arguments");
  QE_TRY(refuse_dict_records(h));
  QE_TRY(ctx_enter(h->ctx));
  return hashagg_export_counts_raw(h, nparts, counts);
}

}

int qe::hashagg_export_counts_raw(qe_hashagg* h, int32_t nparts, int64_t* counts) {
  QE_TRY(settle_pending(h));
  qe_ctx* ctx = h->ctx;
  void* s;
  QE_TRY(ctx_scratch(ctx, (size_t)nparts * 8, &s));
  QE_HIP(hipMemsetAsync(s, 0, (size_t)nparts * 8, ctx->stream));
  const int grid = (int)std::min<uint64_t>(div_up(h->t.cap + 2, 256), 8192);
  hipLaunchKernelGGL(k_export_count, dim3(grid), dim3(256), 0, ctx->stream, h->t, agg_meta(h), nparts,
                     (unsigned long long*)s);
  QE_TRY(launch_check("k_export_count"));
  QE_HIP(hipMemcpyAsync(counts, s, (size_t)nparts * 8, hipMemcpyDeviceToHost, ctx->stream));
  QE_TRY(ctx_sync(ctx));
  return QE_OK;
}

extern "C" {

int qe_hashagg_export(qe_hashagg* h, int32_t nparts, void* dst) {
  QE_CHECK(h && nparts >= 1, QE_ERR_INVALID_ARG, "bad arguments");
  QE_TRY(refuse_dict_records(h));
  QE_TRY(ctx_enter(h->ctx));
  return hashagg_export_raw(h, nparts, dst);
}

}

int qe::hashagg_export_raw(qe_hashagg* h, int32_t nparts, void* dst) {
  qe_ctx* ctx = h->ctx;
  int64_t groups;
  QE_TRY(qe_hashagg_num_groups(h, &groups));
  if (groups == 0) return QE_OK;
  QE_CHECK(dst, QE_ERR_INVALID_ARG, "null destination");
  void* s;
  QE_TRY(ctx_scratch(ctx, (size_t)nparts * 8, &s));
  QE_HIP(hipMemsetAsync(s, 0, (size_t)nparts * 8, ctx->stream));
  const int grid = (int)std::min<uint64_t>(div_up(h->t.cap + 2, 256), 8192);
  hipLaunchKernelGGL(k_export_count, dim3(grid), dim3(256), 0, ctx->stream, h->t, agg_meta(h), nparts,
                     (unsigned long long*)s);
  QE_TRY(launch_check("k_export_count"));
  hipLaunchKernelGGL(k_counts_to_cursors, dim3(1), dim3(64), 0, ctx->stream, (unsigned long long*)s, nparts);
  QE_TRY(launch_check("k_counts_to_cursors"));
  hipLaunchKernelGGL(k_export, dim3(grid), dim3(256), 0, ctx->stream, h->t, agg_meta(h), nparts, h->rec_bytes,
                     (unsigned long long*)s, (uint8_t*)dst);
  QE_TRY(launch_check("k_export"));
  return QE_OK;
}

extern "C" {

int qe_hashagg_export_slots(qe_hashagg* h, int32_t nparts, int64_t slot_records, void* dst) {
  QE_CHECK(h && nparts >= 1 && slot_records >= 1 && dst, QE_ERR_INVALID_ARG, "bad arguments");
  QE_TRY(refuse_dict_records(h));
  QE_TRY(ctx_enter(h->ctx));
  const bool speculative = h->pending;
  qe_ctx* ctx = h->ctx;
  void* s;
  QE_TRY(ctx_scratch(ctx, (size_t)nparts * 8, &s));
  QE_HIP(hipMemsetAsync(s, 0, (size_t)nparts * 8, ctx->stream));
  const int grid = (int)std::min<uint64_t>(div_up(h->t.cap + 2, 256), 8192);
  hipLaunchKernelGGL(k_export_slots, dim3(grid), dim3(256), 0, ctx->stream, h->t, agg_meta(h), nparts, h->rec_bytes,
                     (qi64)slot_records, (unsigned long long*)s, (uint8_t*)dst);
  QE_TRY(launch_check("k_export_slots"));
  const uint64_t slot_bytes = QE_SLOT_HEADER + (uint64_t)slot_records * h->rec_bytes;
  hipLaunchKernelGGL(k_slot_headers, dim3(1), dim3(64), 0, ctx->stream, (const unsigned long long*)s, nparts,
                     (qu64)slot_bytes, (uint8_t*)dst, speculative ? (const qu64*)h->ctl : (const qu64*)nullptr);
  QE_TRY(launch_check("k_slot_headers"));
  return QE_OK;
}

int qe_hashagg_import_slots(qe_hashagg* h, const void* slots, int32_t nslots, int64_t slot_records,
                            int64_t* max_count, int64_t* nrecords) {
  QE_CHECK(h && slots && nslots >= 1 && slot_records >= 1 && max_count, QE_ERR_INVALID_ARG, "bad arguments");
  QE_TRY(refuse_dict_records(h));
  QE_TRY(ctx_enter(h->ctx));
  QE_TRY(settle_pending(h));
  ++h->version;
  QE_TRY(nn_materialize(h, h->nn_implicit));
  qe_ctx* ctx = h->ctx;
  uint64_t groups_before;
  if (h->known_groups >= 0) {
    groups_before = (uint64_t)h->known_groups;
  } else {
    uint64_t c[8];
    QE_TRY(read_ctl(h, c));
    groups_before = c[0];
  }
  const uint64_t bound = groups_before + (uint64_t)nslots * (uint64_t)slot_records;
  if (2 * bound > h->t.cap) QE_TRY(table_grow(h, 2 * bound));
  h->known_groups = -1;
  const int grid = (int)std::min<uint64_t>(div_up((uint64_t)nslots * slot_records, 256), 8192);
  hipLaunchKernelGGL(k_import_slots, dim3(grid), dim3(256), 0, ctx->stream, (const uint8_t*)slots, nslots,
                     (qi64)slot_records, h->rec_bytes, h->t, agg_meta(h));
  QE_TRY(launch_check("k_import_slots"));
  uint64_t c[8];
  QE_TRY(read_ctl(h, c));
  *max_count = (int64_t)c[4];
  if (nrecords) *nrecords = (int64_t)c[5];
  h->known_groups = (int64_t)c[0];
  return QE_OK;
}

int qe_hashagg_import(qe_hashagg* h, const void* records, int64_t nrecords) {
  QE_CHECK(h && nrecords >= 0 && (records || nrecords == 0), QE_ERR_INVALID_ARG, "bad arguments");
  QE_TRY(refuse_dict_records(h));
  QE_TRY(ctx_enter(h->ctx));
  return hashagg_import_raw(h, records, nrecords);
}

int qe_hashagg_key_layout(qe_hashagg* h, int32_t* dictionary_keyed, int32_t* device_nkeys, int32_t* device_types) {
  QE_CHECK(h, QE_ERR_INVALID_ARG, "null state");
  if (dictionary_keyed) *dictionary_keyed = !keyed_dict(h->keyed) ? 0 : keyed_tuple(h->keyed) ? 2 : 1;
  if (device_nkeys) *device_nkeys = h->nkeys;
  if (device_types)
    for (int k = 0; k < QE_MAX_KEYS; ++k) device_types[k] = k < h->nkeys ? h->key_types[k] : 0;
  return QE_OK;
}

}

int qe::hashagg_import_raw(qe_hashagg* h, const void* records, int64_t nrecords) {
  QE_TRY(settle_pending(h));
  if (nrecords == 0) return QE_OK;
  ++h->version;
  QE_TRY(nn_materialize(h, h->nn_implicit));
  h->known_groups = -1;
  uint64_t c[8];
  QE_TRY(read_ctl(h, c));
  if (2 * (c[0] + (uint64_t)nrecords) > h->t.cap) QE_TRY(table_grow(h, 2 * (c[0] + (uint64_t)nrecords)));
  return import_records(h, records, nrecords);
}
```

### query-engines_amd/csrc/qe_internal.hpp

```cpp
#pragma once

#include <hip/hip_runtime.h>
#include <stdint.h>
#include <string.h>

#include <algorithm>
#include <cmath>
#include <string>

#include "qe_hip.h"
#include "qe_dev.hpp"
#include "qe_agg_paths.hpp"

struct qe_ctx {
  int device = 0;
  hipStream_t stream = nullptr;
  bool own_stream = false;
  int num_cus = 256;
  void* scratch = nullptr;
  size_t scratch_bytes = 0;
  uint64_t scratch_epoch = 0;
  void* pinned = nullptr;
  size_t pinned_bytes = 0;
  void* pinned_fg = nullptr;
  size_t pinned_fg_bytes = 0;
  int jit = 1;
  void* scan_tmp = nullptr;
  size_t scan_tmp_bytes = 0;
  void* ws[8] = {};
  size_t ws_bytes[8] = {};
  void* sp_status = nullptr;
  size_t sp_status_bytes = 0;
  uint32_t sp_epoch = 0;
};

namespace qe {

int fail(int code, const char* fmt, ...) __attribute__((format(printf, 2, 3)));
void clear_error();

#define QE_HIP(call)                                                                   \
  do {                                                                                 \
    hipError_t qe_e_ = (call);                                                         \
    if (qe_e_ != hipSuccess)                                                           \
      return ::qe::fail(QE_ERR_DEVICE, "%s failed: %s", #call, hipGetErrorString(qe_e_)); \
  } while (0)

#define QE_CHECK(cond, code, ...)                  \
  do {                                             \
    if (!(cond)) return ::qe::fail(code, __VA_ARGS__); \
  } while (0)

#define QE_TRY(expr)           \
  do {                         \
    int qe_s_ = (expr);        \
    if (qe_s_ != QE_OK) return qe_s_; \
  } while (0)

int ctx_enter(qe_ctx* ctx);
int dev_alloc(qe_ctx* ctx, size_t bytes, void** out);
void dev_free(qe_ctx* ctx, void* p);
void dev_forget_stream(qe_ctx* ctx);
int dev_release(int device);
int ctx_scratch(qe_ctx* ctx, size_t bytes, void** out);
int ctx_pinned(qe_ctx* ctx, size_t bytes, void** out);
int ctx_pinned_coherent(qe_ctx* ctx, size_t bytes, void** out);
int pinned_slot_alloc(uint64_t** out);
void pinned_slot_free(uint64_t* p, hipStream_t stream);
void pinned_slot_free_idle(uint64_t* p);
int ctx_sync(qe_ctx* ctx);
int launch_check(const char* what);
int ctx_workspace(qe_ctx* ctx, int slot, size_t bytes, void** out);
int parallel_h2d_copy(qe_ctx* ctx, void* dst, const void* src, size_t n);
int parallel_h2d_file(qe_ctx* ctx, void* dst, int fd, int64_t off, size_t n);
bool gen_fused_source(const qe::Plan& P, int log2, std::string* src, size_t* lds_bytes, bool spill = false);
bool compact_ok(const qe::Plan& P);
size_t compact_slot_bytes(const qe::Plan& P);
bool compact_acc32(const qe::Plan& P, int j);
struct PartLayout {
  int words = 0;
  bool colmode = false;
  int val_word[QE_MAX_AGGS] = {};
  int col_word[QE_MAX_COLS] = {};
  int flags_word = -1;
  int row_word = -1;
  bool row = false;
  bool narrow = false;
  int bytes() const { return (narrow ? 4 : 8) * words; }
};
PartLayout part_layout(const qe::Plan& P);
bool gen_part_source(const qe::Plan& P, int log2p, bool scatter, std::string* src);
int pagg_fast_slots(const qe::Plan& P);
bool gen_pagg_source(const qe::Plan& P, int log2, std::string* src, size_t* lds_bytes, bool chunked = false,
                     bool soa = false, int64_t bucket_groups = 0);
bool part_staged_ok(const qe::Plan& P, int log2p);
int pscatter_block();
bool pscatter_wide();
int pscatter_block_for(int log2p);
int pagg_block();
bool fused_prefetch();
int fused_block(int lds_log2);
int hashagg_expected_groups(const qe_hashagg* h, int64_t* out);
qe_ctx* hashagg_ctx(const qe_hashagg* h);
struct KeyMeta {
  int32_t mode, nkeys;
  int32_t type[QE_MAX_KEYS], shift[QE_MAX_KEYS], nullbit[QE_MAX_KEYS];
  int64_t fmask[QE_MAX_KEYS];
};
struct Keyed;
struct HashaggInfo {
  qe_ctx* ctx;
  KeyMeta km;
  int32_t rec_bytes, naggs, flags;
  qe_agg_desc aggs[QE_MAX_AGGS];
  uint64_t version;
  uint64_t* ctl;
  Keyed* keyed;
};
HashaggInfo hashagg_info(const qe_hashagg* h);
int hashagg_export_raw(qe_hashagg* h, int32_t nparts, void* dst);
int hashagg_export_counts_raw(qe_hashagg* h, int32_t nparts, int64_t* counts);
int hashagg_import_raw(qe_hashagg* h, const void* recs, int64_t nrec);
int hashagg_update_raw(qe_hashagg* h, const qe_column* dev_keys, const qe_column* agg_inputs, const qe_column* mask);
int hashagg_update_fused_raw(qe_hashagg* h, const qe_column* cols, int32_t ncols, const qe_fused_spec* spec);
int hashagg_finalize_raw(qe_hashagg* h, qe_column* dev_keys, qe_column* out_aggs, int64_t* out_groups, bool keys_only);
int keyed_create(qe_ctx* ctx, int32_t nkeys, const int32_t* types, int64_t expected, Keyed** out, int32_t* dev_nkeys,
                 int32_t* dev_types);
void keyed_destroy(qe_ctx* ctx, Keyed* K);
bool keyed_dict(const Keyed* K);
bool keyed_tuple(const Keyed* K);
int keyed_update(qe_hashagg* h, const qe_column* keys, const qe_column* agg_inputs, const qe_column* mask);
int keyed_update_fused(qe_hashagg* h, const qe_column* cols, int32_t ncols, const qe_fused_spec* spec);
int keyed_finalize(qe_hashagg* h, qe_column* out_keys, qe_column* out_aggs, int64_t* out_groups);
int strdict_encode_packed_checked(qe_ctx* ctx, const qe_column* in, qe_column* codes, unsigned long long* err);
constexpr uint64_t CTL_KEY_TOO_LONG = 1ull << 62;
bool gen_pscatter_staged_source(const qe::Plan& P, int log2p, std::string* src, bool chunked = false, bool soa = false);
bool part_static();
bool part_soa();
int jit_kernel(qe_ctx* ctx, const std::string& src, hipFunction_t* fn, int* blocks_per_cu,
               const char* name = "qe_fused", int block = 512);
int jit_launch(qe_ctx* ctx, hipFunction_t fn, int grid, const qe::Plan& P, int block = 512);
std::string plan_shape_key(const qe_ctx* ctx, const qe::Plan& P);
int compile_inputs(const qe_column* cols, int32_t ncols, int32_t mask_col, int32_t nterms, const qe_pred_term* terms,
                   qe::Plan* P, bool* col_f64);
int compile_program(const qe_column* cols, int32_t ncols, const bool* col_f64, const qe_agg_program& pg, int j,
                    qe::DAgg* a, bool* is_f, bool* nullable);
enum { SP_COUNTER = 0, SP_PERSIST = 1, SP_COUNT = 2, SP_WRITE = 3, SP_WRITE_SCAN = 4, SP_RESIDENT = 5 };
int selproj_resident_rows(const qe::Plan& P, const int32_t* out_kind, int nout, int64_t n, int cus);
bool gen_selproj_resident_source(const qe::Plan& P, const int32_t* out_kind, int nout, int R, std::string* src);
bool gen_selproj_source(const qe::Plan& P, const int32_t* out_kind, int nout, std::string* src, int mode);
int selproj_block(int mode);
int selproj_rows_per_thread(const qe::Plan& P, int mode);
uint64_t jit_kernel_signature(hipFunction_t fn);
bool selproj_pipelined();
int selproj_rows(const qe::Plan& P, int mode);
bool selproj_nt(const qe::Plan& P);
bool selproj_staged(const qe::Plan& P, const int32_t* out_kind, int nout, int mode);
inline int selproj_resident_group(int R) { return R < 8 ? R : 8; }
int exclusive_scan_i64(qe_ctx* ctx, const int64_t* in, int64_t* out, int64_t n);
int64_t utf8_gather_tiles(int64_t rows);
int utf8_gather_lengths(qe_ctx* ctx, const int2* sl, int64_t rows, int64_t* tsum);
int utf8_gather_copy(qe_ctx* ctx, const int2* sl, int64_t rows, const int64_t* tsum, const uint8_t* src,
                     int32_t* out_offs, uint8_t* out_values);
size_t sort_pairs_scratch_bytes(int64_t n);
int sort_pairs(qe_ctx* ctx, uint64_t* const words[2], int32_t* const idx[2], int64_t n, int bits, void* scratch, int* cur);

inline int type_width(int32_t t) {
  switch (t) {
    case QE_TYPE_INT64:
    case QE_TYPE_FLOAT64: return 8;
    case QE_TYPE_INT32:
    case QE_TYPE_DATE32: return 4;
    case QE_TYPE_UINT8: return 1;
    default: return 0;
  }
}
inline bool is_fixed(int32_t t) { return type_width(t) > 0; }
inline bool is_integral(int32_t t) {
  return t == QE_TYPE_INT64 || t == QE_TYPE_INT32 || t == QE_TYPE_DATE32 || t == QE_TYPE_UINT8;
}

inline int32_t kind_of(int32_t type) {
  switch (type) {
    case QE_TYPE_INT64: return K_I64;
    case QE_TYPE_FLOAT64: return K_F64;
    case QE_TYPE_INT32:
    case QE_TYPE_DATE32: return K_I32;
    case QE_TYPE_UINT8: return K_U8;
    case QE_TYPE_BOOL: return K_BOOL;
    default: return -1;
  }
}

inline uint64_t div_up(uint64_t a, uint64_t b) { return (a + b - 1) / b; }

constexpr uint64_t PHI64 = 0x9E3779B97F4A7C15ull;

__host__ __device__ __forceinline__ uint64_t splitmix64(uint64_t x) {
  uint64_t z = x + PHI64;
  z = (z ^ (z >> 30)) * 0xBF58476D1CE4E5B9ull;
  z = (z ^ (z >> 27)) * 0x94D049BB133111EBull;
  return z ^ (z >> 31);
}

__host__ __device__ __forceinline__ uint64_t gen_u64(uint64_t seed, uint64_t col, uint64_t row) {
  return splitmix64(seed ^ (col * PHI64) ^ row);
}

template <typename T, int NW = 16>
__device__ __forceinline__ T tile_excl(const T (&v)[8], T (&ex)[8], T* ws) {
  const int lane = threadIdx.x & 63, wid = threadIdx.x >> 6;
  T s = 0;
#pragma unroll
  for (int k = 0; k < 8; ++k) {
    ex[k] = s;
    s += v[k];
  }
  T x = s;
#pragma unroll
  for (int off = 1; off < 64; off <<= 1) {
    const T y = __shfl_up(x, off);
    if (lane >= off) x += y;
  }
  if (lane == 63) ws[wid] = x;
  __syncthreads();
  T wp = 0, all = 0;
#pragma unroll
  for (int w = 0; w < NW; ++w) {
    if (w < wid) wp += ws[w];
    all += ws[w];
  }
  __syncthreads();
  const T base = wp + x - s;
#pragma unroll
  for (int k = 0; k < 8; ++k) ex[k] += base;
  return all;
}

__device__ __forceinline__ int64_t tile_elem(int64_t g0, int k) { return g0 + (int64_t)threadIdx.x * 8 + k; }

__device__ __forceinline__ void tile_load_u32(const uint32_t* __restrict__ p, int64_t g0, int64_t n, uint32_t (&v)[8],
                                              uint32_t fill = 0) {
  const int64_t e0 = g0 + (int64_t)threadIdx.x * 8;
  if (e0 + 8 <= n) {
    const uint4 a = *(const uint4*)(p + e0), b = *(const uint4*)(p + e0 + 4);
    v[0] = a.x; v[1] = a.y; v[2] = a.z; v[3] = a.w;
    v[4] = b.x; v[5] = b.y; v[6] = b.z; v[7] = b.w;
  } else {
#pragma unroll
    for (int k = 0; k < 8; ++k) v[k] = e0 + k < n ? p[e0 + k] : fill;
  }
}

}
```

### query-engines_amd/kquery/aggregate.py

```python
from __future__ import annotations

from typing import List, Optional, Sequence, Tuple

from . import native as N
from .columnar import Context, DeviceColumn


def output_type(fn: int, input_type: int) -> int:
    if fn in (N.AGG_COUNT, N.AGG_COUNT_STAR):
        return N.TYPE_INT64
    if fn == N.AGG_AVG or input_type == N.TYPE_FLOAT64:
        return N.TYPE_FLOAT64
    return N.TYPE_INT64


_KEY_BITS = {N.TYPE_INT32: 32, N.TYPE_DATE32: 32, N.TYPE_UINT8: 8}


def packable(key_types) -> bool:
    if len(key_types) == 0:
        return True
    if len(key_types) == 1 and key_types[0] in (N.TYPE_INT64, N.TYPE_FLOAT64):
        return True
    if any(t not in _KEY_BITS for t in key_types) or len(key_types) > N.MAX_KEYS:
        return False
    return sum(_KEY_BITS[t] + 1 for t in key_types) <= 63


def _carve(ctx: Context, n: int, specs) -> List[DeviceColumn]:
    import torch

    from .columnar import _torch_dtype, bitmap_bytes

    dev = ctx.torch_device
    vals = torch.empty((len(specs), max(n, 1)), dtype=torch.int64, device=dev).unbind(0)
    nv = sum(1 for _, nullable in specs if nullable)
    bits = torch.empty((max(nv, 1), max(bitmap_bytes(n), 4)), dtype=torch.uint8, device=dev).unbind(0) if nv else []
    out, b = [], 0
    for (t, nullable), v in zip(specs, vals):
        if t not in (N.TYPE_INT64, N.TYPE_FLOAT64):
            v = v.view(_torch_dtype(t))
        elif t == N.TYPE_FLOAT64:
            v = v.view(torch.float64)
        out.append(DeviceColumn(t, n, v, bits[b] if nullable else None, None, ctx))
        b += 1 if nullable else 0
    return out


def _trim(c: DeviceColumn, n: int) -> DeviceColumn:
    from .columnar import bitmap_bytes

    vb = c.validity[: max(bitmap_bytes(n), 4)] if c.validity is not None else None
    if c.type == N.TYPE_UTF8:
        return DeviceColumn(c.type, n, c.values, vb, c.offsets[: n + 1], c.ctx)
    if c.type == N.TYPE_BOOL:
        return DeviceColumn(c.type, n, c.values[: max(bitmap_bytes(n), 4)], vb, None, c.ctx)
    return DeviceColumn(c.type, n, c.values[: max(n, 1)], vb, None, c.ctx)


def _order_for_reader(ctx: Context) -> None:
    import torch

    raw = getattr(torch._C, "_cuda_getCurrentRawStream", None)
    cur = raw(ctx.device) if raw is not None else torch.cuda.current_stream(ctx.torch_device).cuda_stream
    if cur != ctx.stream:
        ctx.synchronize()


def dictionary_keys(key_types) -> Optional[int]:
    member = [N.TYPE_INT32 if t == N.TYPE_UTF8 else t for t in key_types]
    if len(key_types) == 1 and key_types[0] == N.TYPE_UTF8:
        member = [N.TYPE_INT64]
    if not packable(member):
        return len(key_types) + 1
    return len(key_types) if N.TYPE_UTF8 in key_types else None


class HashAggregateState:

    def __init__(self, ctx: Context, key_types: Sequence[int], aggs: Sequence[Tuple[int, int]],
                 expected_groups: int = 1024, async_update: bool = False, deterministic: bool = False,
                 fast_fp64: bool = False):
        self.ctx = ctx
        self.expected_groups = int(expected_groups)
        self.key_types = list(key_types)
        self.aggs = [(int(f), int(t)) for f, t in aggs]
        kt = (N.C.c_int32 * max(1, len(self.key_types)))(*self.key_types)
        ad = (N.QeAggDesc * max(1, len(self.aggs)))(*[N.QeAggDesc(f, t) for f, t in self.aggs])
        h = N.C.c_void_p()
        N.check(N.lib().qe_hashagg_create_ex(ctx.handle, len(self.key_types), kt, len(self.aggs), ad,
                                             int(expected_groups),
                                             (N.HASHAGG_DETERMINISTIC if deterministic else 0) |
                                             (N.HASHAGG_FAST_FP64 if fast_fp64 else 0),
                                             N.C.byref(h)))
        self.deterministic = not fast_fp64
        self.handle = h
        kind, nd = N.C.c_int32(), N.C.c_int32()
        dt = (N.C.c_int32 * N.MAX_KEYS)()
        N.check(N.lib().qe_hashagg_key_layout(h, N.C.byref(kind), N.C.byref(nd), dt))
        self.key_layout = kind.value
        self.device_key_types = list(dt)[: nd.value]
        self._out_rows = max(1, 2 * self.expected_groups)
        self.async_update = bool(async_update)
        self._held = None
        if async_update:
            N.check(N.lib().qe_hashagg_set_async(h, 1))

    def close(self) -> None:
        if getattr(self, "handle", None) is not None:
            N.lib().qe_hashagg_destroy(self.handle)
            self.handle = None

    def __del__(self):
        try:
            self.close()
        except Exception:
            pass

    def bind_key_dict(self, key: int, dictionary) -> None:
        N.check(N.lib().qe_hashagg_bind_key_dict(self.handle, int(key), dictionary.handle))
        self.key_types[key] = N.TYPE_UTF8
        self._bound = getattr(self, "_bound", []) + [dictionary]
        self.key_layout = 1

    @property
    def keyed_by_dictionary(self) -> bool:
        return self.key_layout != 0

    def update(self, keys: Sequence[DeviceColumn], inputs: Sequence[Optional[DeviceColumn]],
               mask: Optional[DeviceColumn] = None) -> None:
        kc = (N.QeColumn * max(1, len(keys)))(*[k.as_c() for k in keys])
        ic = (N.QeColumn * max(1, len(self.aggs)))(
            *[(x.as_c() if x is not None else N.QeColumn()) for x in inputs])
        mc = mask.as_c() if mask is not None else None
        N.check(N.lib().qe_hashagg_update(self.handle, kc, ic, N.C.byref(mc) if mc is not None else None))
        if self.async_update:
            self._held = (keys, inputs, mask)

    def update_fused(self, cols: Sequence[DeviceColumn], spec: N.QeFusedSpec,
                     key_cols: Optional[Sequence[DeviceColumn]] = None) -> None:
        cols = list(cols)
        if self.keyed_by_dictionary:
            if key_cols is None:
                raise N.IllegalStateException(N.QE_ERR_UNSUPPORTED,
                                              "fused update with dictionary-encoded keys needs the key columns")
            if len(cols) + dictionary_keys(self.key_types) > N.MAX_COLS:
                raise N.IllegalStateException(N.QE_ERR_UNSUPPORTED, f"fused plan takes at most {N.MAX_COLS} columns")
            spec = N.QeFusedSpec.from_buffer_copy(spec)
            for k in range(len(key_cols)):
                spec.key_cols[k] = len(cols) + k
            cols += list(key_cols)
        cc = (N.QeColumn * len(cols))(*[c.as_c() for c in cols])
        N.check(N.lib().qe_hashagg_update_fused(self.handle, cc, len(cols), N.C.byref(spec)))
        if self.async_update:
            self._held = cols

    def slot_capacity(self, world: int) -> int:
        cap = N.C.c_int64()
        N.check(N.lib().qe_hashagg_slot_capacity(self.handle, int(world), N.C.byref(cap)))
        return cap.value

    def set_row_base(self, row_base: int) -> None:
        N.check(N.lib().qe_hashagg_set_row_base(self.handle, int(row_base)))

    def last_kernel_time(self):
        ms = N.C.c_double()
        k = N.C.c_int32()
        N.check(N.lib().qe_hashagg_last_kernel_time(self.handle, N.C.byref(ms), N.C.byref(k)))
        return ms.value, k.value

    def last_kernel_signature(self) -> str:
        sig = N.C.c_uint64()
        N.check(N.lib().qe_hashagg_last_kernel_signature(self.handle, N.C.byref(sig)))
        return f"{sig.value:016x}"

    def last_kernel_kind(self):
        k = N.C.c_int32()
        buf = N.C.create_string_buffer(512)
        N.check(N.lib().qe_hashagg_last_kernel_kind(self.handle, N.C.byref(k), buf, 512))
        return bool(k.value), buf.value.decode(errors="replace")

    def last_chunk_stats(self):
        c, f, r = N.C.c_int64(), N.C.c_int64(), N.C.c_int64()
        N.check(N.lib().qe_hashagg_last_chunk_stats(self.handle, N.C.byref(c), N.C.byref(f), N.C.byref(r)))
        return c.value, f.value, r.value

    def reset(self) -> None:
        N.check(N.lib().qe_hashagg_reset(self.handle))

    def num_groups(self) -> int:
        n = N.C.c_int64()
        N.check(N.lib().qe_hashagg_num_groups(self.handle, N.C.byref(n)))
        return n.value

    def prepare_output(self) -> None:
        if getattr(self, "_stash", None) is None and N.TYPE_UTF8 not in self.key_types:
            self._stash = self._carve_c(self._out_rows)

    def _carve_c(self, rows: int, key_bytes=None):
        import torch

        from .columnar import bitmap_bytes

        specs = ([(t, True) for t in self.key_types if t not in (N.TYPE_UTF8, N.TYPE_BOOL)] +
                 [(output_type(f, t), f not in (N.AGG_COUNT, N.AGG_COUNT_STAR)) for f, t in self.aggs])
        fixed = _carve(self.ctx, rows, specs) if specs else []
        dev = self.ctx.torch_device
        keys, it = [], iter(fixed)
        for k, t in enumerate(self.key_types):
            if t == N.TYPE_UTF8:
                nb = int(key_bytes[k]) if key_bytes is not None else 7 * rows
                keys.append(DeviceColumn(N.TYPE_UTF8, rows, torch.empty(max(1, nb), dtype=torch.uint8, device=dev),
                                         torch.empty(max(bitmap_bytes(rows), 4), dtype=torch.uint8, device=dev),
                                         torch.empty(rows + 1, dtype=torch.int32, device=dev), self.ctx))
            elif t == N.TYPE_BOOL:
                keys.append(DeviceColumn.empty(N.TYPE_BOOL, rows, True, ctx=self.ctx))
            else:
                keys.append(next(it))
        cols = keys + list(it)
        nk = len(self.key_types)
        kc = (N.QeColumn * max(1, nk))(*[k.as_c() for k in cols[:nk]])
        ac = (N.QeColumn * max(1, len(cols) - nk))(*[a.as_c() for a in cols[nk:]])
        return rows, cols, kc, ac

    def finalize(self) -> Tuple[List[DeviceColumn], List[DeviceColumn]]:
        nk = len(self.key_types)
        out = N.C.c_int64(-1)
        stash, self._stash = getattr(self, "_stash", None), None
        if N.TYPE_UTF8 in self.key_types:
            bound = N.C.c_int64()
            packed = True
            for k, t in enumerate(self.key_types):
                if t == N.TYPE_UTF8:
                    N.check(N.lib().qe_hashagg_key_bytes_bound(self.handle, k, N.C.byref(bound)))
                    packed = packed and bound.value == 7
            if packed:
                stash = self._carve_c(self._out_rows)
            else:
                g = N.C.c_int64()
                kb = (N.C.c_int64 * max(1, nk))()
                N.check(N.lib().qe_hashagg_finalize_sizes(self.handle, N.C.byref(g), kb))
                stash = self._carve_c(max(1, g.value), list(kb))
        while True:
            rows, cols, kc, ac = stash if stash is not None else self._carve_c(self._out_rows)
            stash = None
            st = N.lib().qe_hashagg_finalize(self.handle, kc, ac, N.C.byref(out))
            if st == N.QE_ERR_CAPACITY and out.value > rows:
                self._out_rows = out.value
                continue
            N.check(st)
            break
        g = out.value
        self._out_rows = max(1, g)
        _order_for_reader(self.ctx)
        if g != rows:
            cols = [_trim(c, g) for c in cols]
        return cols[:nk], cols[nk:]

    def record_bytes(self) -> int:
        n = N.C.c_int64()
        N.check(N.lib().qe_hashagg_record_bytes(self.handle, N.C.byref(n)))
        return n.value

    def export_counts(self, nparts: int) -> List[int]:
        arr = (N.C.c_int64 * nparts)()
        N.check(N.lib().qe_hashagg_export_counts(self.handle, nparts, arr))
        return list(arr)

    def export(self, nparts: int):
        import torch

        counts = self.export_counts(nparts)
        rb = self.record_bytes()
        buf = torch.empty(max(1, sum(counts) * rb), dtype=torch.uint8, device=self.ctx.torch_device)
        N.check(N.lib().qe_hashagg_export(self.handle, nparts, N.C.c_void_p(buf.data_ptr())))
        return buf[: sum(counts) * rb], counts

    def slot_bytes(self, slot_records: int) -> int:
        return N.SLOT_HEADER + int(slot_records) * self.record_bytes()

    def export_slots(self, nparts: int, slot_records: int):
        import torch

        buf = torch.empty(nparts * self.slot_bytes(slot_records), dtype=torch.uint8, device=self.ctx.torch_device)
        N.check(N.lib().qe_hashagg_export_slots(self.handle, int(nparts), int(slot_records),
                                                N.C.c_void_p(buf.data_ptr())))
        return buf

    def import_slots(self, slots, nslots: int, slot_records: int) -> Optional[int]:
        mx, n = N.C.c_int64(), N.C.c_int64()
        N.check(N.lib().qe_hashagg_import_slots(self.handle, N.C.c_void_p(slots.data_ptr()), int(nslots),
                                                int(slot_records), N.C.byref(mx), N.C.byref(n)))
        return None if mx.value > slot_records else n.value

    def import_records(self, records, nrecords: int) -> None:
        if nrecords == 0:
            return
        N.check(N.lib().qe_hashagg_import(self.handle, N.C.c_void_p(records.data_ptr()), int(nrecords)))

    def export_keyed(self, nparts: int):
        import torch

        sizes = (N.C.c_int64 * nparts)()
        N.check(N.lib().qe_hashagg_export_keyed_sizes(self.handle, int(nparts), sizes))
        sizes = list(sizes)
        buf = torch.empty(max(1, sum(sizes)), dtype=torch.uint8, device=self.ctx.torch_device)
        N.check(N.lib().qe_hashagg_export_keyed(self.handle, int(nparts), N.C.c_void_p(buf.data_ptr())))
        return buf, sizes

    def import_keyed(self, blocks, sizes: Sequence[int]) -> int:
        import numpy as np

        n = len(sizes)
        arr = (N.C.c_int64 * max(1, n))(*[int(x) for x in sizes])
        N.check(N.lib().qe_hashagg_import_keyed(self.handle, N.C.c_void_p(blocks.data_ptr()), n, arr))
        recs, off = 0, 0
        for sz in sizes:
            if sz:
                recs += int(np.frombuffer(blocks[off + 8: off + 16].cpu().numpy().tobytes(), dtype=np.int64)[0])
            off += int(sz)
        return recs

    def merge(self, other: "HashAggregateState") -> None:
        N.check(N.lib().qe_hashagg_merge(self.handle, other.handle))
```

### query-engines_amd/kquery/exchange.py

```python
from __future__ import annotations

from typing import List, Optional, Tuple

import torch
import torch.distributed as dist


def all_to_all_records(payload: torch.Tensor, counts: List[int], record_bytes: int,
                       group: Optional[dist.ProcessGroup] = None) -> Tuple[torch.Tensor, int]:
    world = dist.get_world_size(group)
    assert len(counts) == world
    dev = payload.device
    send_counts = torch.tensor(counts, dtype=torch.int64, device=dev)
    recv_counts = torch.empty(world, dtype=torch.int64, device=dev)
    dist.all_to_all_single(recv_counts, send_counts, group=group)
    rc = [int(x) for x in recv_counts.cpu().tolist()]
    out = torch.empty(max(1, sum(rc) * record_bytes), dtype=torch.uint8, device=dev)
    in_split = [c * record_bytes for c in counts]
    out_split = [c * record_bytes for c in rc]
    if payload.numel() == 0:
        payload = torch.empty(0, dtype=torch.uint8, device=dev)
    dist.all_to_all_single(out[: sum(out_split)], payload[: sum(in_split)], out_split, in_split, group=group)
    return out[: sum(out_split)], sum(rc)


def _a2a_bytes(chunks: List[torch.Tensor], group=None) -> Tuple[torch.Tensor, List[int]]:
    world = dist.get_world_size(group)
    dev = chunks[0].device
    stage = dist.get_backend(group) == "gloo" and dev.type != "cpu"
    send = torch.cat([c.reshape(-1) for c in chunks]) if any(c.numel() for c in chunks) else \
        torch.empty(0, dtype=torch.uint8, device=dev)
    sizes = torch.tensor([c.numel() for c in chunks], dtype=torch.int64)
    rsizes = torch.empty(world, dtype=torch.int64)
    if not stage and dev.type != "cpu":
        sizes, rsizes = sizes.to(dev), rsizes.to(dev)
    dist.all_to_all_single(rsizes, sizes, group=group)
    rs = [int(x) for x in rsizes.cpu().tolist()]
    out = torch.empty(sum(rs), dtype=torch.uint8, device="cpu" if stage else dev)
    dist.all_to_all_single(out, send.cpu() if stage else send, rs, [c.numel() for c in chunks], group=group)
    return (out.to(dev) if stage else out), rs


def exchange_keyed_partials(partial, owner, group: Optional[dist.ProcessGroup] = None) -> int:
    world = dist.get_world_size(group)
    blocks, sizes = partial.export_keyed(world)
    chunks, off = [], 0
    for sz in sizes:
        chunks.append(blocks[off: off + sz])
        off += sz
    rblocks, rsz = _a2a_bytes(chunks, group)
    return owner.import_keyed(rblocks, rsz)


def all_to_all_slots(send: torch.Tensor, group: Optional[dist.ProcessGroup] = None) -> torch.Tensor:
    stage = dist.get_backend(group) == "gloo" and send.device.type != "cpu"
    src = send.cpu() if stage else send
    out = torch.empty_like(src)
    dist.all_to_all_single(out, src, group=group)
    return out.to(send.device) if stage else out


def exchange_partials(partial, owner, group: Optional[dist.ProcessGroup] = None,
                      slot_records: Optional[int] = None) -> int:
    if getattr(partial, "keyed_by_dictionary", False) or getattr(owner, "keyed_by_dictionary", False):
        return exchange_keyed_partials(partial, owner, group)
    world = dist.get_world_size(group)
    cap = int(slot_records or partial.slot_capacity(world))
    recv = all_to_all_slots(partial.export_slots(world, cap), group)
    owner.prepare_output()
    n = owner.import_slots(recv, world, cap)
    if n is not None:
        return n
    recs, counts = partial.export(world)
    recv, n = all_to_all_records(recs, counts, partial.record_bytes(), group)
    owner.import_records(recv, n)
    return n


class NativeComm:

    def __init__(self, ctx, group: Optional[dist.ProcessGroup] = None):
        from . import native as N

        world = dist.get_world_size(group) if dist.is_initialized() else 1
        rank = dist.get_rank(group) if dist.is_initialized() else 0
        uid = (N.C.c_char * N.COMM_ID_BYTES)()
        if rank == 0:
            N.check(N.lib().qe_comm_unique_id(uid))
        if world > 1:
            box = [bytes(uid)]
            dist.broadcast_object_list(box, src=0, group=group)
            uid = (N.C.c_char * N.COMM_ID_BYTES).from_buffer_copy(box[0])
        h = N.C.c_void_p()
        N.check(N.lib().qe_comm_create(ctx.handle, world, rank, uid, N.C.byref(h)))
        self.handle, self.ctx, self.world, self.rank = h, ctx, world, rank

    def close(self) -> None:
        from . import native as N

        if getattr(self, "handle", None) is not None:
            N.lib().qe_comm_destroy(self.handle)
            self.handle = None

    def __del__(self):
        try:
            self.close()
        except Exception:
            pass


def exchange_partials_native(partial, owner, comm: NativeComm, slot_records: int = 0) -> int:
    from . import native as N

    owner.prepare_output()
    n = N.C.c_int64()
    N.check(N.lib().qe_hashagg_exchange(comm.handle, partial.handle, owner.handle, int(slot_records), N.C.byref(n)))
    return n.value


def _all_gather_bytes(part, world: int, group):
    if world == 1:
        return part
    if dist.get_backend(group) == "gloo":
        got = [torch.empty_like(part, device="cpu") for _ in range(world)]
        dist.all_gather(got, part.cpu(), group=group)
        return torch.cat(got).to(part.device)
    parts = torch.empty(world * part.numel(), dtype=torch.uint8, device=part.device)
    dist.all_gather_into_tensor(parts, part, group=group)
    return parts


def global_aggregate(col, mask=None, row_base: int = 0, group: Optional[dist.ProcessGroup] = None):
    from . import native as N

    ctx = col.ctx
    world = dist.get_world_size(group) if dist.is_initialized() else 1
    part = torch.empty(N.GLOBAL_PARTIAL_BYTES, dtype=torch.uint8, device=ctx.torch_device)
    cc = col.as_c()
    mc = mask.as_c() if mask is not None else None
    mp = N.C.byref(mc) if mc is not None else None
    N.check(N.lib().qe_agg_global_partial(ctx.handle, N.C.byref(cc), mp, int(row_base), N.C.c_void_p(part.data_ptr())))
    parts = _all_gather_bytes(part, world, group)
    out = N.QeGlobalAgg()
    st = N.lib().qe_agg_global_merge(ctx.handle, col.type, N.C.c_void_p(parts.data_ptr()), world, N.C.byref(out))
    if st == N.QE_NEED_EXACT:
        words = torch.empty(N.GLOBAL_EXACT_BYTES, dtype=torch.uint8, device=ctx.torch_device)
        N.check(N.lib().qe_agg_global_exact_partial(ctx.handle, N.C.byref(cc), mp, N.C.c_void_p(words.data_ptr())))
        allw = _all_gather_bytes(words, world, group)
        st = N.lib().qe_agg_global_merge_exact(ctx.handle, N.C.c_void_p(allw.data_ptr()), world, N.C.byref(out))
    N.check(st)
    return out
```

### query-engines_amd/kquery/native.py

```python
from __future__ import annotations

import ctypes as C
import os
import pathlib

_ROOT = pathlib.Path(__file__).resolve().parents[1]
LIB_PATH = _ROOT / "lib" / "libqe_hip.so"

QE_OK = 0
QE_ERR_INVALID_ARG = -1
QE_ERR_UNSUPPORTED = -2
QE_ERR_OOM = -3
QE_ERR_DEVICE = -4
QE_ERR_CAPACITY = -5
QE_ERR_COMM = -6
COMM_ID_BYTES = 128

TYPE_INT64 = 1
TYPE_FLOAT64 = 2
TYPE_BOOL = 3
TYPE_UTF8 = 4
TYPE_INT32 = 5
TYPE_UINT8 = 6
TYPE_DATE32 = 7

GEN_MOD = 1
GEN_RAW = 2
GEN_UNIT53 = 3
GEN_MOD_F64 = 4

OP_ADD, OP_SUB, OP_MUL, OP_DIV = 1, 2, 3, 4
OP_EQ, OP_NE, OP_LT, OP_LE, OP_GT, OP_GE = 10, 11, 12, 13, 14, 15
OP_AND, OP_OR, OP_NOT, OP_IS_NULL, OP_IS_NOT_NULL = 20, 21, 22, 23, 24

AGG_SUM, AGG_MIN, AGG_MAX, AGG_COUNT, AGG_COUNT_STAR, AGG_AVG = 1, 2, 3, 4, 5, 6

SORT_DESC, SORT_NULLS_FIRST = 1, 2
JOIN_INNER, JOIN_LEFT = 0, 1

MAX_KEYS, MAX_AGGS, MAX_COLS, MAX_TERMS, MAX_TOKENS = 4, 8, 8, 8, 16
TOK_COL, TOK_LIT, TOK_ADD, TOK_SUB, TOK_MUL, TOK_DIV = 1, 2, 3, 4, 5, 6

FIXED_WIDTH = {TYPE_INT64: 8, TYPE_FLOAT64: 8, TYPE_INT32: 4, TYPE_DATE32: 4, TYPE_UINT8: 1}


class QueryEngineError(RuntimeError):

    def __init__(self, status: int, message: str):
        super().__init__(f"[{status}] {message}")
        self.status = status


class IllegalStateException(QueryEngineError):
    """QE_ERR_UNSUPPORTED (Main.kt:195, :469, :677, :792, :799)."""


class IllegalArgumentException(QueryEngineError):
    """QE_ERR_INVALID_ARG (Main.kt:49)."""


class NumberFormatException(IllegalArgumentException):
    """CAST(utf8 AS double) of a string outside java.lang.Double.parseDouble's grammar (K:791)."""


class CapacityError(QueryEngineError):
    """QE_ERR_CAPACITY: an output buffer is too small."""


class DeviceError(QueryEngineError):
    """QE_ERR_DEVICE / QE_ERR_OOM."""


class CommError(QueryEngineError):
    """QE_ERR_COMM: RCCL missing or a collective failed."""


_ERR_CLASS = {
    QE_ERR_UNSUPPORTED: IllegalStateException,
    QE_ERR_INVALID_ARG: IllegalArgumentException,
    QE_ERR_CAPACITY: CapacityError,
    QE_ERR_COMM: CommError,
}


class QeColumn(C.Structure):
    _fields_ = [
        ("type", C.c_int32),
        ("max_len", C.c_int32),
        ("length", C.c_int64),
        ("validity", C.c_void_p),
        ("values", C.c_void_p),
        ("offsets", C.c_void_p),
    ]


class QeScalar(C.Structure):
    _fields_ = [("type", C.c_int32), ("is_null", C.c_int32), ("bits", C.c_int64)]


class QeOperand(C.Structure):
    _fields_ = [("col", C.POINTER(QeColumn)), ("lit", QeScalar)]


class QeGlobalAgg(C.Structure):
    _fields_ = [
        ("rows", C.c_int64),
        ("count", C.c_int64),
        ("type", C.c_int32),
        ("valid", C.c_int32),
        ("sum", C.c_int64),
        ("min", C.c_int64),
        ("max", C.c_int64),
        ("avg", C.c_double),
    ]


class QeAggDesc(C.Structure):
    _fields_ = [("fn", C.c_int32), ("input_type", C.c_int32)]


class QePredTerm(C.Structure):
    _fields_ = [
        ("col", C.c_int32),
        ("op", C.c_int32),
        ("rhs_col", C.c_int32),
        ("reserved", C.c_int32),
        ("lit", QeScalar),
    ]


class QeToken(C.Structure):
    _fields_ = [("op", C.c_int32), ("arg", C.c_int32), ("lit", QeScalar)]


class QeAggProgram(C.Structure):
    _fields_ = [("ntokens", C.c_int32), ("reserved", C.c_int32), ("tokens", QeToken * MAX_TOKENS)]


class QeFusedSpec(C.Structure):
    _fields_ = [
        ("mask_col", C.c_int32),
        ("nterms", C.c_int32),
        ("terms", QePredTerm * MAX_TERMS),
        ("key_cols", C.c_int32 * MAX_KEYS),
        ("inputs", QeAggProgram * MAX_AGGS),
    ]


class QeCsvOptions(C.Structure):
    _fields_ = [("delimiter", C.c_int32), ("has_header", C.c_int32), ("nfields", C.c_int32),
                ("flags", C.c_int32), ("field_index", C.POINTER(C.c_int32))]


CSV_PARTIAL_TAIL = 1


class QeSelectSpec(C.Structure):
    _fields_ = [
        ("mask_col", C.c_int32),
        ("nterms", C.c_int32),
        ("terms", QePredTerm * MAX_TERMS),
        ("nout", C.c_int32),
        ("reserved", C.c_int32),
        ("outputs", QeAggProgram * MAX_AGGS),
    ]


SELECT_RESIDENT, SELECT_TWOPASS, SELECT_SCANNED, SELECT_LOOKBACK_PERSISTENT, SELECT_LOOKBACK_COUNTER = 1, 2, 3, 4, 5


class QeSelectLayout(C.Structure):
    _fields_ = [
        ("scheme", C.c_int32),
        ("staged", C.c_int32),
        ("block", C.c_int32),
        ("reserved", C.c_int32),
        ("tile_rows", C.c_int64),
        ("tiles", C.c_int64),
        ("group_rows", C.c_int64),
    ]


_lib = None

HASHAGG_DETERMINISTIC = 1
HASHAGG_FAST_FP64 = 2
_P = C.c_void_p
_PP = C.POINTER(C.c_void_p)
_I64P = C.POINTER(C.c_int64)
_COLP = C.POINTER(QeColumn)
_OPP = C.POINTER(QeOperand)
SLOT_HEADER = 64
KEYED_HEADER = 128
GLOBAL_PARTIAL_BYTES = 128
GLOBAL_EXACT_BYTES = 320
QE_NEED_EXACT = 1

SIGNATURES = [
    ("qe_ctx_create", C.c_int, [C.c_int, _P, _PP]),
    ("qe_ctx_create_owned", C.c_int, [C.c_int, _PP]),
    ("qe_ctx_set_jit", C.c_int, [_P, C.c_int32]),
    ("qe_ctx_destroy", C.c_int, [_P]),
    ("qe_ctx_stream", _P, [_P]),
    ("qe_ctx_synchronize", C.c_int, [_P]),
    ("qe_last_error", C.c_char_p, []),
    ("qe_abi_version", C.c_int, []),
    ("qe_device_alloc", C.c_int, [_P, C.c_size_t, _PP]),
    ("qe_device_free", C.c_int, [_P, _P]),
    ("qe_release_cached_memory", C.c_int, [C.c_int]),
    ("qe_copy_to_device", C.c_int, [_P, _P, _P, C.c_size_t]),
    ("qe_file_to_device", C.c_int, [_P, C.c_char_p, C.c_int64, C.c_int64, _P]),
    ("qe_copy_to_host", C.c_int, [_P, _P, _P, C.c_size_t]),
    ("qe_generate", C.c_int, [_P, _COLP, C.c_int32, C.c_int64, C.c_uint64, C.c_uint64, C.c_int64, C.c_int32]),
    ("qe_stream_read", C.c_int, [_P, _COLP, C.c_int32, C.POINTER(C.c_double)]),
    ("qe_stream_read_best", C.c_int, [_P, _COLP, C.c_int32, C.c_int32, C.POINTER(C.c_double), C.c_char_p, C.c_int32]),
    ("qe_eval_arith", C.c_int, [_P, C.c_int32, _OPP, _OPP, _COLP]),
    ("qe_eval_cmp", C.c_int, [_P, C.c_int32, _OPP, _OPP, _COLP]),
    ("qe_eval_bool", C.c_int, [_P, C.c_int32, _COLP, _COLP, _COLP]),
    ("qe_cast_utf8_to_f64", C.c_int, [_P, _COLP, _COLP, _I64P]),
    ("qe_filter_count", C.c_int, [_P, _COLP, _I64P]),
    ("qe_filter_apply", C.c_int, [_P, _COLP, _COLP, C.c_int32, _COLP, _I64P]),
    ("qe_filter_apply_async", C.c_int, [_P, _COLP, _COLP, C.c_int32, _COLP, _P]),
    ("qe_eval_arith_dlen", C.c_int, [_P, C.c_int32, _OPP, _OPP, _COLP, _P]),
    ("qe_sort_indices", C.c_int, [_P, _COLP, C.POINTER(C.c_int32), C.c_int32, C.c_int64, _COLP]),
    ("qe_take", C.c_int, [_P, _COLP, _COLP, C.c_int32, _COLP, _I64P]),
    ("qe_sort_layout", C.c_int, [C.POINTER(C.c_int32), C.POINTER(C.c_int32)]),
    ("qe_join_build", C.c_int, [_P, _COLP, _PP]),
    ("qe_join_destroy", C.c_int, [_P]),
    ("qe_join_probe", C.c_int, [_P, _COLP, C.c_int32, _COLP, _COLP, _I64P]),
    ("qe_join_probe_mask", C.c_int, [_P, _COLP, C.c_int32, _COLP]),
    ("qe_join_stats", C.c_int, [_P, _I64P, _I64P, _I64P, _I64P]),
    ("qe_take_or_null", C.c_int, [_P, _COLP, _COLP, C.c_int32, _COLP, _I64P]),
    ("qe_agg_global", C.c_int, [_P, _COLP, _COLP, C.POINTER(QeGlobalAgg)]),
    ("qe_agg_global_partial", C.c_int, [_P, _COLP, _COLP, C.c_int64, _P]),
    ("qe_agg_global_merge", C.c_int, [_P, C.c_int32, _P, C.c_int32, C.POINTER(QeGlobalAgg)]),
    ("qe_agg_global_exact_partial", C.c_int, [_P, _COLP, _COLP, _P]),
    ("qe_agg_global_merge_exact", C.c_int, [_P, _P, C.c_int32, C.POINTER(QeGlobalAgg)]),
    ("qe_hashagg_create", C.c_int,
     [_P, C.c_int32, C.POINTER(C.c_int32), C.c_int32, C.POINTER(QeAggDesc), C.c_int64, _PP]),
    ("qe_hashagg_create_ex", C.c_int,
     [_P, C.c_int32, C.POINTER(C.c_int32), C.c_int32, C.POINTER(QeAggDesc), C.c_int64, C.c_int32, _PP]),
    ("qe_hashagg_destroy", C.c_int, [_P]),
    ("qe_hashagg_reset", C.c_int, [_P]),
    ("qe_hashagg_update", C.c_int, [_P, _COLP, _COLP, _COLP]),
    ("qe_hashagg_update_fused", C.c_int, [_P, _COLP, C.c_int32, C.POINTER(QeFusedSpec)]),
    ("qe_hashagg_num_groups", C.c_int, [_P, _I64P]),
    ("qe_hashagg_finalize", C.c_int, [_P, _COLP, _COLP, _I64P]),
    ("qe_hashagg_record_bytes", C.c_int, [_P, _I64P]),
    ("qe_hashagg_export_counts", C.c_int, [_P, C.c_int32, _I64P]),
    ("qe_hashagg_export", C.c_int, [_P, C.c_int32, _P]),
    ("qe_hashagg_import", C.c_int, [_P, _P, C.c_int64]),
    ("qe_hashagg_export_slots", C.c_int, [_P, C.c_int32, C.c_int64, _P]),
    ("qe_hashagg_import_slots", C.c_int, [_P, _P, C.c_int32, C.c_int64, _I64P, _I64P]),
    ("qe_hashagg_slot_capacity", C.c_int, [_P, C.c_int32, _I64P]),
    ("qe_hashagg_finalize_sizes", C.c_int, [_P, _I64P, _I64P]),
    ("qe_hashagg_export_keyed_sizes", C.c_int, [_P, C.c_int32, _I64P]),
    ("qe_hashagg_export_keyed", C.c_int, [_P, C.c_int32, _P]),
    ("qe_hashagg_import_keyed", C.c_int, [_P, _P, C.c_int32, _I64P]),
    ("qe_hashagg_merge", C.c_int, [_P, _P]),
    ("qe_hashagg_bind_key_dict", C.c_int, [_P, C.c_int32, _P]),
    ("qe_hashagg_key_bytes_bound", C.c_int, [_P, C.c_int32, _I64P]),
    ("qe_hashagg_key_layout", C.c_int, [_P, C.POINTER(C.c_int32), C.POINTER(C.c_int32), C.POINTER(C.c_int32)]),
    ("qe_comm_unique_id", C.c_int, [_P]),
    ("qe_comm_create", C.c_int, [_P, C.c_int32, C.c_int32, _P, C.POINTER(C.c_void_p)]),
    ("qe_comm_destroy", C.c_int, [_P]),
    ("qe_comm_loopback_hub_create", C.c_int, [C.c_int32, C.POINTER(C.c_void_p)]),
    ("qe_comm_loopback_hub_destroy", C.c_int, [_P]),
    ("qe_comm_create_loopback", C.c_int, [_P, C.c_int32, C.c_int32, _P, C.POINTER(C.c_void_p)]),
    ("qe_hashagg_exchange", C.c_int, [_P, _P, _P, C.c_int64, _I64P]),
    ("qe_hashagg_set_row_base", C.c_int, [_P, C.c_int64]),
    ("qe_hashagg_set_async", C.c_int, [_P, C.c_int32]),
    ("qe_hashagg_last_kernel_time", C.c_int, [_P, C.POINTER(C.c_double), C.POINTER(C.c_int32)]),
    ("qe_hashagg_last_kernel_signature", C.c_int, [_P, C.POINTER(C.c_uint64)]),
    ("qe_hashagg_last_kernel_kind", C.c_int, [_P, C.POINTER(C.c_int32), C.c_char_p, C.c_int32]),
    ("qe_hashagg_last_chunk_stats", C.c_int, [_P, C.POINTER(C.c_int64), C.POINTER(C.c_int64), C.POINTER(C.c_int64)]),
    ("qe_strdict_create", C.c_int, [_P, C.c_int64, _PP]),
    ("qe_strdict_destroy", C.c_int, [_P]),
    ("qe_strdict_size", C.c_int, [_P, _I64P]),
    ("qe_strdict_encode", C.c_int, [_P, _COLP, _COLP]),
    ("qe_strdict_decode_bytes", C.c_int, [_P, _COLP, _I64P]),
    ("qe_strdict_decode", C.c_int, [_P, _COLP, _COLP]),
    ("qe_strdict_decode_trusted", C.c_int, [_P, _COLP, _COLP]),
    ("qe_strdict_encode_packed", C.c_int, [_P, _COLP, _COLP]),
    ("qe_strdict_decode_packed", C.c_int, [_P, _COLP, _COLP]),
    ("qe_strdict_encode_tuple", C.c_int, [_P, _COLP, C.c_int32, _COLP]),
    ("qe_strdict_decode_tuple", C.c_int, [_P, _COLP, C.c_int32, _COLP]),
    ("qe_hash_partition", C.c_int, [_P, _COLP, C.c_int32, C.c_int32, _P]),
    ("qe_select_project", C.c_int, [_P, _COLP, C.c_int32, C.POINTER(QeSelectSpec), _COLP, _I64P]),
    ("qe_select_project_async", C.c_int, [_P, _COLP, C.c_int32, C.POINTER(QeSelectSpec), _COLP, C.POINTER(_P)]),
    ("qe_select_project_layout", C.c_int, [_P, _COLP, C.c_int32, C.POINTER(QeSelectSpec), _COLP,
                                           C.POINTER(QeSelectLayout)]),
    ("qe_select_pending_wait", C.c_int, [_P, _I64P]),
    ("qe_csv_parse", C.c_int, [_P, _P, C.c_int64, C.POINTER(QeCsvOptions), _PP]),
    ("qe_csv_rows", C.c_int, [_P, _I64P]),
    ("qe_csv_consumed", C.c_int, [_P, _I64P]),
    ("qe_csv_column", C.c_int, [_P, C.c_int32, _COLP]),
    ("qe_csv_column_bytes", C.c_int, [_P, C.c_int32, _I64P]),
    ("qe_csv_column_max_len", C.c_int, [_P, C.c_int32, _I64P]),
    ("qe_csv_column_copy", C.c_int, [_P, C.c_int32, _COLP]),
    ("qe_csv_destroy", C.c_int, [_P]),
    ("qe_csv_record_end", C.c_int, [_P, C.c_int64, C.c_int32, _I64P]),
    ("qe_batch_import", C.c_int, [_P, _P, _P, _PP]),
    ("qe_batch_import_device", C.c_int, [_P, _P, _P, _PP]),
    ("qe_batch_destroy", C.c_int, [_P]),
    ("qe_batch_num_columns", C.c_int, [_P, C.POINTER(C.c_int32), _I64P]),
    ("qe_batch_column", C.c_int, [_P, C.c_int32, _COLP, C.POINTER(C.c_char_p)]),
    ("qe_batch_export", C.c_int, [_P, _COLP, C.c_int32, C.POINTER(C.c_char_p), _P, _P]),
]


def load_library(path: os.PathLike | str | None = None) -> C.CDLL:
    global _lib
    if _lib is not None and path is None:
        return _lib
    p = pathlib.Path(path) if path else pathlib.Path(os.environ.get("QE_LIB") or LIB_PATH)
    if not p.exists():
        raise ImportError(
            f"libqe_hip.so not found at {p}: build it with `python -c 'import __graft_entry__ as g; g.build()'` "
            "(there is no CPU fallback)"
        )
    lib = C.CDLL(str(p))
    for name, res, args in SIGNATURES:
        fn = getattr(lib, name)
        fn.restype = res
        fn.argtypes = args
    if path is None:
        _lib = lib
    return lib


def lib() -> C.CDLL:
    return load_library()


def check(status: int) -> None:
    if status != QE_OK:
        msg = lib().qe_last_error().decode(errors="replace")
        raise _ERR_CLASS.get(status, DeviceError)(status, msg)


def scalar(value, type_id: int | None = None) -> QeScalar:
    import struct

    if value is None:
        return QeScalar(type_id or TYPE_INT64, 1, 0)
    if type_id == TYPE_FLOAT64 or (type_id is None and isinstance(value, float)):
        return QeScalar(TYPE_FLOAT64, 0, struct.unpack("<q", struct.pack("<d", float(value)))[0])
    v = int(value)
    if not -(1 << 63) <= v < (1 << 63):
        raise IllegalArgumentException(QE_ERR_INVALID_ARG, f"int64 literal out of range: {v}")
    return QeScalar(TYPE_INT64, 0, v)
```

Before: 274.3 billion rows/s.

## Fuse slot import with finalize in a single-workgroup LDS kernel for small merges

Adds a fused import+finalize path. When the received slots fit an LDS hash table, one workgroup merges them there and writes the finalized output columns directly. Also adds a single-workgroup small export kernel with LDS cursors, and caches the finalized batch keyed by a table version so a later finalize() can skip its work. This cuts kernel launches and global-table round trips in the exchange tail. The cost is extra code paths with fallbacks on overflow or capacity errors. Since this workload runs one GPU with 1024 groups, the exchange tail is small next to the 1B-row scan.

```diff
diff --git a/include/qe_hip.h b/include/qe_hip.h
--- a/include/qe_hip.h
+++ b/include/qe_hip.h
@@ -278,6 +278,10 @@
 int qe_hashagg_export_slots(qe_hashagg* agg, int32_t nparts, int64_t slot_records, void* dst);
 int qe_hashagg_import_slots(qe_hashagg* agg, const void* slots, int32_t nslots, int64_t slot_records,
                             int64_t* max_count, int64_t* nrecords);
+int qe_hashagg_import_slots_finalize(qe_hashagg* agg, const void* slots, int32_t nslots, int64_t slot_records,
+                                     qe_column* out_keys, qe_column* out_aggs, int64_t* max_count,
+                                     int64_t* nrecords, int64_t* out_groups);
+int qe_hashagg_version(qe_hashagg* agg, uint64_t* version);
 int qe_hashagg_slot_capacity(qe_hashagg* agg, int32_t world, int64_t* slot_records);
 
 int qe_hashagg_set_async(qe_hashagg* agg, int32_t enable);
@@ -292,6 +296,9 @@
 int qe_comm_create_loopback(qe_ctx* ctx, int32_t world, int32_t rank, void* hub, qe_comm** out);
 int qe_hashagg_exchange(qe_comm* comm, qe_hashagg* partial, qe_hashagg* owner, int64_t slot_records,
                         int64_t* nrecords);
+int qe_hashagg_exchange_finalize(qe_comm* comm, qe_hashagg* partial, qe_hashagg* owner, int64_t slot_records,
+                                 qe_column* out_keys, qe_column* out_aggs, int64_t* nrecords,
+                                 int64_t* out_groups);
 
 int qe_hashagg_set_row_base(qe_hashagg* agg, int64_t row_base);
 
diff --git a/query-engines_amd/csrc/qe_comm.hip b/query-engines_amd/csrc/qe_comm.hip
--- a/query-engines_amd/csrc/qe_comm.hip
+++ b/query-engines_amd/csrc/qe_comm.hip
@@ -271,8 +271,10 @@
   return QE_OK;
 }
 
-int qe_hashagg_exchange(qe_comm* c, qe_hashagg* partial, qe_hashagg* owner, int64_t slot_records,
-                        int64_t* nrecords) {
+}
+
+static int exchange_impl(qe_comm* c, qe_hashagg* partial, qe_hashagg* owner, int64_t slot_records, bool fin,
+                         qe_column* out_keys, qe_column* out_aggs, int64_t* nrecords, int64_t* out_groups) {
   QE_CHECK(c && partial && owner, QE_ERR_INVALID_ARG, "null argument");
   QE_TRY(ctx_enter(c->ctx));
   const int world = c->world;
@@ -281,7 +283,10 @@
   QE_CHECK(hashagg_ctx(partial) == c->ctx && hashagg_ctx(owner) == c->ctx, QE_ERR_INVALID_ARG,
            "partial, owner and communicator must share one qe_ctx (one stream)");
   if (keyed_dict(hashagg_info(partial).keyed) || keyed_dict(hashagg_info(owner).keyed))
-    return exchange_keyed(c, partial, owner, nrecords);
+  {
+    QE_TRY(exchange_keyed(c, partial, owner, nrecords));
+    return fin ? qe_hashagg_finalize(owner, out_keys, out_aggs, out_groups) : QE_OK;
+  }
   int64_t cap = slot_records;
   if (cap <= 0) QE_TRY(qe_hashagg_slot_capacity(partial, world, &cap));
   const size_t slot_bytes = (size_t)QE_SLOT_HEADER + (size_t)cap * (size_t)rb;
@@ -293,7 +298,14 @@
   for (int p = 0; p < world; ++p) off[p] = (size_t)p * slot_bytes;
   QE_TRY(exchange_bytes(c, send, off.data(), len.data(), recv, off.data(), len.data()));
   int64_t mx = 0, n = 0;
-  QE_TRY(qe_hashagg_import_slots(owner, recv, world, cap, &mx, &n));
+  if (fin) {
+    int64_t g = -1;
+    const int st = qe_hashagg_import_slots_finalize(owner, recv, world, cap, out_keys, out_aggs, &mx, &n, &g);
+    if (out_groups && g >= 0) *out_groups = g;
+    if (st == QE_ERR_CAPACITY && g >= 0 && nrecords) *nrecords = n;
+    QE_TRY(st);
+  } else
+    QE_TRY(qe_hashagg_import_slots(owner, recv, world, cap, &mx, &n));
   if (mx <= cap) {
     if (nrecords) *nrecords = n;
     return QE_OK;
@@ -332,7 +344,19 @@
   QE_TRY(exchange_bytes(c, srec, so.data(), sl.data(), rrec, ro.data(), rl.data()));
   QE_TRY(qe_hashagg_import(owner, rrec, rtotal));
   if (nrecords) *nrecords = rtotal;
-  return QE_OK;
-}
-
-}
+  return fin ? qe_hashagg_finalize(owner, out_keys, out_aggs, out_groups) : QE_OK;
+}
+
+extern "C" {
+
+int qe_hashagg_exchange(qe_comm* c, qe_hashagg* partial, qe_hashagg* owner, int64_t slot_records,
+                        int64_t* nrecords) {
+  return exchange_impl(c, partial, owner, slot_records, false, nullptr, nullptr, nrecords, nullptr);
+}
+
+int qe_hashagg_exchange_finalize(qe_comm* c, qe_hashagg* partial, qe_hashagg* owner, int64_t slot_records,
+                                 qe_column* out_keys, qe_column* out_aggs, int64_t* nrecords, int64_t* out_groups) {
+  return exchange_impl(c, partial, owner, slot_records, true, out_keys, out_aggs, nrecords, out_groups);
+}
+
+}
diff --git a/query-engines_amd/csrc/qe_exchange_paths.hpp b/query-engines_amd/csrc/qe_exchange_paths.hpp
--- /dev/null
+++ b/query-engines_amd/csrc/qe_exchange_paths.hpp
@@ -0,0 +1,44 @@
+#pragma once
+
+#include <stddef.h>
+#include <stdint.h>
+
+namespace qe {
+
+constexpr int SMALL_WG_THREADS = 1024, SMALL_WG_PER = 16;
+constexpr uint64_t SMALL_TABLE_SLOTS = (uint64_t)SMALL_WG_THREADS * SMALL_WG_PER;
+
+constexpr int32_t EXPORT_SMALL_MAX_PARTS = SMALL_WG_THREADS;
+inline bool export_slots_small_ok(uint64_t cap, int32_t nparts) {
+  return cap + 2 <= SMALL_TABLE_SLOTS && nparts >= 1 && nparts <= EXPORT_SMALL_MAX_PARTS;
+}
+
+constexpr size_t MERGE_LDS_LIMIT = 160 * 1024;
+constexpr size_t MERGE_LDS_FIXED = 28 * 1024;
+constexpr int64_t MERGE_LDS_MIN_SLOTS = 64;
+
+struct MergeLds {
+  bool ok = false;
+  int64_t slots = 0;
+  size_t bytes = 0;
+};
+
+inline size_t merge_lds_slot_bytes(int lds_aggs) { return 16 + 16 * (size_t)lds_aggs; }
+
+inline MergeLds merge_finalize_lds(int64_t nslots, int64_t slot_records, int lds_aggs) {
+  MergeLds r;
+  if (nslots < 1 || slot_records < 1 || lds_aggs < 0) return r;
+  if (slot_records > (int64_t)SMALL_TABLE_SLOTS || nslots > (int64_t)SMALL_TABLE_SLOTS) return r;
+  const int64_t bound = nslots * slot_records;
+  int64_t slots = MERGE_LDS_MIN_SLOTS;
+  while (slots - slots / 8 < bound && slots < (int64_t)SMALL_TABLE_SLOTS) slots <<= 1;
+  if (slots - slots / 8 < bound) return r;
+  const size_t bytes = (size_t)(slots + 2) * merge_lds_slot_bytes(lds_aggs);
+  if (bytes + MERGE_LDS_FIXED > MERGE_LDS_LIMIT) return r;
+  r.ok = true;
+  r.slots = slots;
+  r.bytes = bytes;
+  return r;
+}
+
+}
diff --git a/query-engines_amd/csrc/qe_hashagg.hip b/query-engines_amd/csrc/qe_hashagg.hip
--- a/query-engines_amd/csrc/qe_hashagg.hip
+++ b/query-engines_amd/csrc/qe_hashagg.hip
@@ -952,23 +952,43 @@
   wg_newg_end(&newg, dst.ctl);
 }
 
+__device__ __forceinline__ void slots_verdict(const qu8* __restrict__ slots, qi32 nslots, qi64 slot_records,
+                                              qu64 slot_bytes, qu64* mx_out, qu64* tot_out) {
+  qu64 mx = 0, tot = 0;
+  for (int i = threadIdx.x; i < nslots; i += 64) {
+    const qu64* hd = (const qu64*)(slots + (qu64)i * slot_bytes);
+    mx = hd[1] > mx ? hd[1] : mx;
+    tot += hd[0] < (qu64)slot_records ? hd[0] : (qu64)slot_records;
+  }
+  for (int off = 32; off > 0; off >>= 1) {
+    const qu64 o = __shfl_xor(mx, off);
+    mx = o > mx ? o : mx;
+    tot += __shfl_xor(tot, off);
+  }
+  *mx_out = mx;
+  *tot_out = tot;
+}
+
+__device__ __forceinline__ void import_slot_records(const qu8* __restrict__ slots, qi32 nslots, qi64 slot_records,
+                                                    qi32 rec_bytes, qu64 slot_bytes, DTable& dst, const AggMeta& m,
+                                                    qu32* newg) {
+  const qi64 total = (qi64)nslots * slot_records;
+  for (qi64 r = blockIdx.x * (qi64)blockDim.x + threadIdx.x; r < total; r += (qi64)gridDim.x * blockDim.x) {
+    const qi64 sl = r / slot_records, i = r - sl * slot_records;
+    const qu8* base = slots + (qu64)sl * slot_bytes;
+    if ((qu64)i >= ((const qu64*)base)[0]) continue;
+    import_record(base + QE_SLOT_HEADER + (qu64)i * rec_bytes, dst, m, newg);
+  }
+}
+
 __global__ void k_import_slots(const qu8* __restrict__ slots, qi32 nslots, qi64 slot_records, qi32 rec_bytes,
                                DTable dst, AggMeta m) {
   __shared__ qu32 newg;
   __shared__ qi32 s_ok;
   const qu64 slot_bytes = QE_SLOT_HEADER + (qu64)slot_records * rec_bytes;
   if (threadIdx.x < 64) {
-    qu64 mx = 0, tot = 0;
-    for (int i = threadIdx.x; i < nslots; i += 64) {
-      const qu64* hd = (const qu64*)(slots + (qu64)i * slot_bytes);
-      mx = hd[1] > mx ? hd[1] : mx;
-      tot += hd[0] < (qu64)slot_records ? hd[0] : (qu64)slot_records;
-    }
-    for (int off = 32; off > 0; off >>= 1) {
-      const qu64 o = __shfl_xor(mx, off);
-      mx = o > mx ? o : mx;
-      tot += __shfl_xor(tot, off);
-    }
+    qu64 mx, tot;
+    slots_verdict(slots, nslots, slot_records, slot_bytes, &mx, &tot);
     if (threadIdx.x == 0) {
       s_ok = mx <= (qu64)slot_records;
       if (blockIdx.x == 0) {
@@ -978,15 +998,7 @@
     }
   }
   wg_newg_begin(&newg);
-  if (s_ok) {
-    const qi64 total = (qi64)nslots * slot_records;
-    for (qi64 r = blockIdx.x * (qi64)blockDim.x + threadIdx.x; r < total; r += (qi64)gridDim.x * blockDim.x) {
-      const qi64 sl = r / slot_records, i = r - sl * slot_records;
-      const qu8* base = slots + (qu64)sl * slot_bytes;
-      if ((qu64)i >= ((const qu64*)base)[0]) continue;
-      import_record(base + QE_SLOT_HEADER + (qu64)i * rec_bytes, dst, m, &newg);
-    }
-  }
+  if (s_ok) import_slot_records(slots, nslots, slot_records, rec_bytes, slot_bytes, dst, m, &newg);
   wg_newg_end(&newg, dst.ctl);
 }
 
@@ -1103,28 +1115,42 @@
   }
 }
 
+__device__ __forceinline__ void export_slot_records(const DTable& t, const AggMeta& m, qi32 nparts, qi32 rec_bytes,
+                                                    qi64 slot_records, qu64 slot_bytes, unsigned long long* cursor,
+                                                    qu8* __restrict__ dst, qu64 s) {
+  const bool has = s < t.cap + 2 && gslot_occupied(t, s);
+  const bool knull = s == t.cap;
+  const qi64 key = !has ? 0 : knull ? 0 : (s == t.cap + 1 ? EMPTY_KEY : t.keys[s]);
+  const qu32 p = has ? partition_of(key, knull, nparts) : 0;
+  const qu64 pos = wave_cursor(cursor, has, p);
+  qu8* base = dst + p * slot_bytes + QE_SLOT_HEADER;
+  if (has && pos < (qu64)slot_records) write_record(base + pos * (qu64)rec_bytes, t, m, s, key, knull);
+  if (m.any_x) {
+    const bool ext = has && slot_has_ext(t, m, s);
+    const qu64 pe = wave_cursor(cursor, ext, p, FXE_CHUNKS);
+    if (ext)
+      for (int c = 0; c < FXE_CHUNKS; ++c)
+        if (pe + c < (qu64)slot_records) write_chunk_record(base + (pe + c) * (qu64)rec_bytes, t, m, s, key, knull, c);
+  }
+}
+
 __global__ void k_export_slots(DTable t, AggMeta m, qi32 nparts, qi32 rec_bytes, qi64 slot_records,
                                unsigned long long* cursor, qu8* __restrict__ dst) {
   const qu64 SS = t.cap + 2;
   const qu64 slot_bytes = QE_SLOT_HEADER + (qu64)slot_records * rec_bytes;
   const qu64 stride = (qu64)gridDim.x * blockDim.x;
-  for (qu64 s0 = blockIdx.x * (qu64)blockDim.x; s0 < SS; s0 += stride) {
-    const qu64 s = s0 + threadIdx.x;
-    const bool has = s < SS && gslot_occupied(t, s);
-    const bool knull = s == t.cap;
-    const qi64 key = !has ? 0 : knull ? 0 : (s == t.cap + 1 ? EMPTY_KEY : t.keys[s]);
-    const qu32 p = has ? partition_of(key, knull, nparts) : 0;
-    const qu64 pos = wave_cursor(cursor, has, p);
-    qu8* base = dst + p * slot_bytes + QE_SLOT_HEADER;
-    if (has && pos < (qu64)slot_records) write_record(base + pos * (qu64)rec_bytes, t, m, s, key, knull);
-    if (m.any_x) {
-      const bool ext = has && slot_has_ext(t, m, s);
-      const qu64 pe = wave_cursor(cursor, ext, p, FXE_CHUNKS);
-      if (ext)
-        for (int c = 0; c < FXE_CHUNKS; ++c)
-          if (pe + c < (qu64)slot_records) write_chunk_record(base + (pe + c) * (qu64)rec_bytes, t, m, s, key, knull, c);
-    }
-  }
+  for (qu64 s0 = blockIdx.x * (qu64)blockDim.x; s0 < SS; s0 += stride)
+    export_slot_records(t, m, nparts, rec_bytes, slot_records, slot_bytes, cursor, dst, s0 + threadIdx.x);
+}
+
+__device__ __forceinline__ qu64 slot_header_max(qu64 mx, const qu64* __restrict__ guard) {
+  return guard && (guard[1] | guard[2] | guard[3]) ? 1ull << 62 : mx;
+}
+__device__ __forceinline__ void write_slot_header(qu8* __restrict__ dst, qu64 slot_bytes, int p, qu64 count, qu64 mx) {
+  qu64* hd = (qu64*)(dst + (qu64)p * slot_bytes);
+  hd[0] = count;
+  hd[1] = mx;
+  for (int w = 2; w < QE_SLOT_HEADER / 8; ++w) hd[w] = 0;
 }
 
 __global__ void k_slot_headers(const unsigned long long* __restrict__ cursor, qi32 nparts, qu64 slot_bytes,
@@ -1135,13 +1161,34 @@
     const qu64 o = __shfl_xor(mx, off);
     mx = o > mx ? o : mx;
   }
-  if (guard && (guard[1] | guard[2] | guard[3])) mx = 1ull << 62;
-  for (int p = threadIdx.x; p < nparts; p += blockDim.x) {
-    qu64* hd = (qu64*)(dst + (qu64)p * slot_bytes);
-    hd[0] = cursor[p];
-    hd[1] = mx;
-    for (int w = 2; w < QE_SLOT_HEADER / 8; ++w) hd[w] = 0;
-  }
+  mx = slot_header_max(mx, guard);
+  for (int p = threadIdx.x; p < nparts; p += blockDim.x) write_slot_header(dst, slot_bytes, p, cursor[p], mx);
+}
+
+__global__ void __launch_bounds__(SMALL_WG_THREADS) k_export_slots_small(DTable t, AggMeta m, qi32 nparts, qi32 rec_bytes,
+                                                                         qi64 slot_records, qu8* __restrict__ dst,
+                                                                         const qu64* __restrict__ guard) {
+  __shared__ unsigned long long cur[EXPORT_SMALL_MAX_PARTS];
+  __shared__ qu64 wmx[SMALL_WG_THREADS / 64];
+  static_assert(EXPORT_SMALL_MAX_PARTS == SMALL_WG_THREADS, "one cursor per thread");
+  const int tid = threadIdx.x;
+  const qu64 SS = t.cap + 2;
+  const qu64 slot_bytes = QE_SLOT_HEADER + (qu64)slot_records * rec_bytes;
+  cur[tid] = 0;
+  __syncthreads();
+  for (qu64 s0 = 0; s0 < SS; s0 += SMALL_WG_THREADS)
+    export_slot_records(t, m, nparts, rec_bytes, slot_records, slot_bytes, cur, dst, s0 + tid);
+  __syncthreads();
+  qu64 mx = tid < nparts ? cur[tid] : 0;
+  for (int off = 32; off > 0; off >>= 1) {
+    const qu64 o = __shfl_xor(mx, off);
+    mx = o > mx ? o : mx;
+  }
+  if ((tid & 63) == 0) wmx[tid >> 6] = mx;
+  __syncthreads();
+  for (int w = 0; w < SMALL_WG_THREADS / 64; ++w) mx = wmx[w] > mx ? wmx[w] : mx;
+  mx = slot_header_max(mx, guard);
+  if (tid < nparts) write_slot_header(dst, slot_bytes, tid, cur[tid], mx);
 }
 
 __global__ void k_occ_count(DTable t, qi64* __restrict__ tile_counts, qi32 tile_slots) {
@@ -1270,10 +1317,10 @@
   }
 }
 
-constexpr int FS_THREADS = 1024, FS_PER = 16, FS_WAVES = FS_THREADS / 64;
+constexpr int FS_THREADS = SMALL_WG_THREADS, FS_PER = SMALL_WG_PER, FS_WAVES = FS_THREADS / 64;
 static_assert(FS_THREADS * FS_PER / 2 / 32 <= FS_WORDS, "LDS bitmaps hold every group of a small table");
-__global__ void __launch_bounds__(FS_THREADS) k_finalize_small(DTable t, AggMeta m, KeyMeta km, OutCols out,
-                                                               qi64 groups) {
+__device__ __forceinline__ void finalize_small_wg(const DTable& t, const AggMeta& m, const KeyMeta& km,
+                                                  const OutCols& out, qi64 groups) {
   __shared__ qi32 wcnt[FS_PER][FS_WAVES];
   __shared__ qu64 wbal[FS_PER][FS_WAVES];
   __shared__ qu32 lbits[(QE_MAX_KEYS + QE_MAX_AGGS) * FS_WORDS];
@@ -1328,6 +1375,94 @@
     for (int j = 0; j < m.naggs; ++j)
       if (out.aggs[j].validity) ((qu32*)out.aggs[j].validity)[w] = lbits[(QE_MAX_KEYS + j) * FS_WORDS + w];
   }
+}
+
+__global__ void __launch_bounds__(FS_THREADS) k_finalize_small(DTable t, AggMeta m, KeyMeta km, OutCols out,
+                                                               qi64 groups) {
+  finalize_small_wg(t, m, km, out, groups);
+}
+
+__global__ void __launch_bounds__(FS_THREADS) k_import_finalize(const qu8* __restrict__ slots, qi32 nslots,
+                                                                qi64 slot_records, qi32 rec_bytes, DTable g, AggMeta m,
+                                                                KeyMeta km, OutCols out, qi64 out_cap, qi64 lslots) {
+  extern __shared__ __attribute__((aligned(16))) qu64 ltab[];
+  __shared__ DTable l;
+  __shared__ qu64 lctl[8];
+  __shared__ qu64 s_mx, s_tot;
+  __shared__ qu32 newg, gnew;
+  const int tid = threadIdx.x;
+  const qu64 LS = (qu64)lslots + 2;
+  const qu64 slot_bytes = QE_SLOT_HEADER + (qu64)slot_records * rec_bytes;
+  if (tid < 64) {
+    qu64 mx, tot;
+    slots_verdict(slots, nslots, slot_records, slot_bytes, &mx, &tot);
+    if (tid == 0) {
+      s_mx = mx;
+      s_tot = tot;
+      newg = gnew = 0;
+      qu64* p = ltab;
+      l.keys = (qi64*)p;
+      l.cstar = p + LS;
+      p += 2 * LS;
+      for (int j = 0; j < QE_MAX_AGGS; ++j) {
+        l.idx[j] = l.ext[j] = nullptr;
+        if (j < m.naggs && m.fn[j] != QE_AGG_COUNT_STAR) {
+          l.acc[j] = (qi64*)p;
+          l.nn[j] = p + LS;
+          p += 2 * LS;
+        } else {
+          l.acc[j] = (qi64*)l.cstar;
+          l.nn[j] = l.cstar;
+        }
+      }
+      l.cap = (qu64)lslots;
+      l.ctl = lctl;
+    }
+  }
+  if (tid < 8) lctl[tid] = 0;
+  __syncthreads();
+  for (qu64 s = tid; s < LS; s += FS_THREADS) {
+    l.keys[s] = EMPTY_KEY;
+    l.cstar[s] = 0;
+    for (int j = 0; j < m.naggs; ++j)
+      if (m.fn[j] != QE_AGG_COUNT_STAR) {
+        l.acc[j][s] = acc_identity(m.acc[j]);
+        l.nn[j][s] = 0;
+      }
+  }
+  __syncthreads();
+  const bool ok = s_mx <= (qu64)slot_records;
+  if (ok) import_slot_records(slots, nslots, slot_records, rec_bytes, slot_bytes, l, m, &newg);
+  __syncthreads();
+  const qu64 groups = lctl[0] + newg;
+  const bool lost = lctl[3] != 0;
+  if (tid == 0) {
+    g.ctl[4] = s_mx;
+    g.ctl[5] = s_tot;
+    g.ctl[6] = lost;
+  }
+  if (!ok || lost) return;
+  for (qu64 s = tid; s < LS; s += FS_THREADS) {
+    if (!gslot_occupied(l, s)) continue;
+    const bool knull = s == l.cap;
+    const qi64 key = knull ? 0 : (s == l.cap + 1 ? EMPTY_KEY : l.keys[s]);
+    qu64 d = s;
+    if (l.cap == g.cap) {
+      if (s < l.cap) g.keys[d] = key;
+    } else if (!gtable_find_wg(g, key, knull, d, &gnew)) {
+      atomicAdd((unsigned long long*)&g.ctl[3], 1ull);
+      continue;
+    }
+    g.cstar[d] = l.cstar[s];
+    for (int j = 0; j < m.naggs; ++j)
+      if (m.fn[j] != QE_AGG_COUNT_STAR) {
+        g.acc[j][d] = l.acc[j][s];
+        g.nn[j][d] = l.nn[j][s];
+      }
+  }
+  if (tid == 0) g.ctl[0] = groups;
+  if (groups == 0 || (qi64)groups > out_cap) return;
+  finalize_small_wg(l, m, km, out, (qi64)groups);
 }
 
 }
@@ -2671,6 +2806,12 @@
 
 }
 
+static int32_t agg_output_type(const qe_agg_desc& d) {
+  return (d.fn == QE_AGG_COUNT || d.fn == QE_AGG_COUNT_STAR)               ? QE_TYPE_INT64
+         : (d.fn == QE_AGG_AVG || d.input_type == QE_TYPE_FLOAT64) ? QE_TYPE_FLOAT64
+                                                                    : QE_TYPE_INT64;
+}
+
 int qe::hashagg_finalize_raw(qe_hashagg* h, qe_column* out_keys, qe_column* out_aggs, int64_t* out_groups,
                              bool keys_only) {
   qe_ctx* ctx = h->ctx;
@@ -2693,10 +2834,7 @@
   for (int j = 0; j < h->naggs && !keys_only; ++j) {
     QE_CHECK(out_aggs, QE_ERR_INVALID_ARG, "null out_aggs");
     const qe_column& c = out_aggs[j];
-    const int fn = h->aggs[j].fn;
-    const int32_t want = (fn == QE_AGG_COUNT || fn == QE_AGG_COUNT_STAR) ? QE_TYPE_INT64
-                         : (fn == QE_AGG_AVG || h->aggs[j].input_type == QE_TYPE_FLOAT64) ? QE_TYPE_FLOAT64
-                                                                                          : QE_TYPE_INT64;
+    const int32_t want = agg_output_type(h->aggs[j]);
     QE_CHECK(c.type == want, QE_ERR_INVALID_ARG, "aggregate output %d: type %d, expected %d", j, c.type, want);
     QE_CHECK(c.length >= groups && (c.values || groups == 0), QE_ERR_CAPACITY,
              "aggregate output %d holds %lld rows, need %lld", j, (long long)c.length, (long long)groups);
@@ -2810,6 +2948,12 @@
   QE_TRY(ctx_enter(h->ctx));
   const bool speculative = h->pending;
   qe_ctx* ctx = h->ctx;
+  const qu64* guard = speculative ? (const qu64*)h->ctl : (const qu64*)nullptr;
+  if (export_slots_small_ok(h->t.cap, nparts)) {
+    hipLaunchKernelGGL(k_export_slots_small, dim3(1), dim3(SMALL_WG_THREADS), 0, ctx->stream, h->t, agg_meta(h), nparts,
+                       h->rec_bytes, (qi64)slot_records, (uint8_t*)dst, guard);
+    return launch_check("k_export_slots_small");
+  }
   void* s;
   QE_TRY(ctx_scratch(ctx, (size_t)nparts * 8, &s));
   QE_HIP(hipMemsetAsync(s, 0, (size_t)nparts * 8, ctx->stream));
@@ -2819,17 +2963,15 @@
   QE_TRY(launch_check("k_export_slots"));
   const uint64_t slot_bytes = QE_SLOT_HEADER + (uint64_t)slot_records * h->rec_bytes;
   hipLaunchKernelGGL(k_slot_headers, dim3(1), dim3(64), 0, ctx->stream, (const unsigned long long*)s, nparts,
-                     (qu64)slot_bytes, (uint8_t*)dst, speculative ? (const qu64*)h->ctl : (const qu64*)nullptr);
+                     (qu64)slot_bytes, (uint8_t*)dst, guard);
   QE_TRY(launch_check("k_slot_headers"));
   return QE_OK;
 }
 
-int qe_hashagg_import_slots(qe_hashagg* h, const void* slots, int32_t nslots, int64_t slot_records,
-                            int64_t* max_count, int64_t* nrecords) {
-  QE_CHECK(h && slots && nslots >= 1 && slot_records >= 1 && max_count, QE_ERR_INVALID_ARG, "bad arguments");
-  QE_TRY(refuse_dict_records(h));
-  QE_TRY(ctx_enter(h->ctx));
-  QE_TRY(settle_pending(h));
+}
+
+static int import_slots_raw(qe_hashagg* h, const void* slots, int32_t nslots, int64_t slot_records, int64_t* max_count,
+                            int64_t* nrecords) {
   ++h->version;
   QE_TRY(nn_materialize(h, h->nn_implicit));
   qe_ctx* ctx = h->ctx;
@@ -2856,6 +2998,93 @@
   return QE_OK;
 }
 
+static bool import_finalize_eligible(const qe_hashagg* h, int32_t nslots, int64_t slot_records, const qe_column* out_keys,
+                                     const qe_column* out_aggs, MergeLds* lds, OutCols* oc, int64_t* out_cap) {
+  if (h->pending || h->poisoned || h->known_groups != 0 || keyed_dict(h->keyed)) return false;
+  int lds_aggs = 0;
+  for (int j = 0; j < h->naggs; ++j) {
+    if (acc_has_idx(h->acc[j])) return false;
+    lds_aggs += h->aggs[j].fn != QE_AGG_COUNT_STAR;
+  }
+  *lds = merge_finalize_lds(nslots, slot_records, lds_aggs);
+  if (!lds->ok) return false;
+  if ((h->nkeys && !out_keys) || (h->naggs && !out_aggs)) return false;
+  int64_t cap = INT64_MAX;
+  auto take = [&](const qe_column& c, int32_t want, qe_column* dst) {
+    if (c.type != want || ((uintptr_t)c.validity & 3) || c.length < 0 || (!c.values && c.length > 0)) return false;
+    cap = std::min<int64_t>(cap, c.length);
+    *dst = c;
+    return true;
+  };
+  for (int k = 0; k < h->nkeys; ++k)
+    if (!take(out_keys[k], h->key_types[k], &oc->keys[k])) return false;
+  for (int j = 0; j < h->naggs; ++j)
+    if (!take(out_aggs[j], agg_output_type(h->aggs[j]), &oc->aggs[j])) return false;
+  *out_cap = cap;
+  return true;
+}
+
+extern "C" {
+
+int qe_hashagg_import_slots(qe_hashagg* h, const void* slots, int32_t nslots, int64_t slot_records,
+                            int64_t* max_count, int64_t* nrecords) {
+  QE_CHECK(h && slots && nslots >= 1 && slot_records >= 1 && max_count, QE_ERR_INVALID_ARG, "bad arguments");
+  QE_TRY(refuse_dict_records(h));
+  QE_TRY(ctx_enter(h->ctx));
+  QE_TRY(settle_pending(h));
+  return import_slots_raw(h, slots, nslots, slot_records, max_count, nrecords);
+}
+
+int qe_hashagg_import_slots_finalize(qe_hashagg* h, const void* slots, int32_t nslots, int64_t slot_records,
+                                     qe_column* out_keys, qe_column* out_aggs, int64_t* max_count, int64_t* nrecords,
+                                     int64_t* out_groups) {
+  QE_CHECK(h && slots && nslots >= 1 && slot_records >= 1 && max_count, QE_ERR_INVALID_ARG, "bad arguments");
+  QE_TRY(refuse_dict_records(h));
+  QE_TRY(ctx_enter(h->ctx));
+  QE_TRY(settle_pending(h));
+  MergeLds lds;
+  OutCols oc{};
+  int64_t out_cap = 0;
+  if (!import_finalize_eligible(h, nslots, slot_records, out_keys, out_aggs, &lds, &oc, &out_cap)) {
+    QE_TRY(import_slots_raw(h, slots, nslots, slot_records, max_count, nrecords));
+    if (*max_count > slot_records) return QE_OK;
+    return hashagg_finalize_raw(h, out_keys, out_aggs, out_groups, false);
+  }
+  qe_ctx* ctx = h->ctx;
+  ++h->version;
+  const uint64_t bound = (uint64_t)nslots * (uint64_t)slot_records;
+  if (2 * bound > h->t.cap) QE_TRY(table_grow(h, 2 * bound));
+  h->nn_implicit = 0;
+  h->known_groups = -1;
+  QE_HIP(hipFuncSetAttribute((const void*)k_import_finalize, hipFuncAttributeMaxDynamicSharedMemorySize, (int)lds.bytes));
+  hipLaunchKernelGGL(k_import_finalize, dim3(1), dim3(FS_THREADS), lds.bytes, ctx->stream, (const uint8_t*)slots, nslots,
+                     (qi64)slot_records, h->rec_bytes, h->t, agg_meta(h), h->km, oc, (qi64)out_cap, (qi64)lds.slots);
+  QE_TRY(launch_check("k_import_finalize"));
+  uint64_t c[8];
+  QE_TRY(read_ctl(h, c));
+  if (c[6]) {
+    h->known_groups = 0;
+    QE_TRY(import_slots_raw(h, slots, nslots, slot_records, max_count, nrecords));
+    if (*max_count > slot_records) return QE_OK;
+    return hashagg_finalize_raw(h, out_keys, out_aggs, out_groups, false);
+  }
+  *max_count = (int64_t)c[4];
+  if (nrecords) *nrecords = (int64_t)c[5];
+  const int64_t groups = h->known_groups = (int64_t)c[0];
+  if (*max_count > slot_records) return QE_OK;
+  if (out_groups) *out_groups = groups;
+  QE_CHECK(out_cap >= groups, QE_ERR_CAPACITY, "outputs hold %lld rows, need %lld", (long long)out_cap, (long long)groups);
+  for (int k = 0; k < h->nkeys; ++k) out_keys[k].length = groups;
+  for (int j = 0; j < h->naggs; ++j) out_aggs[j].length = groups;
+  return QE_OK;
+}
+
+int qe_hashagg_version(qe_hashagg* h, uint64_t* out) {
+  QE_CHECK(h && out, QE_ERR_INVALID_ARG, "null argument");
+  *out = h->version;
+  return QE_OK;
+}
+
 int qe_hashagg_import(qe_hashagg* h, const void* records, int64_t nrecords) {
   QE_CHECK(h && nrecords >= 0 && (records || nrecords == 0), QE_ERR_INVALID_ARG, "bad arguments");
   QE_TRY(refuse_dict_records(h));
diff --git a/query-engines_amd/csrc/qe_internal.hpp b/query-engines_amd/csrc/qe_internal.hpp
--- a/query-engines_amd/csrc/qe_internal.hpp
+++ b/query-engines_amd/csrc/qe_internal.hpp
@@ -11,6 +11,7 @@
 #include "qe_hip.h"
 #include "qe_dev.hpp"
 #include "qe_agg_paths.hpp"
+#include "qe_exchange_paths.hpp"
 
 struct qe_ctx {
   int device = 0;
diff --git a/query-engines_amd/kquery/aggregate.py b/query-engines_amd/kquery/aggregate.py
--- a/query-engines_amd/kquery/aggregate.py
+++ b/query-engines_amd/kquery/aggregate.py
@@ -103,6 +103,7 @@
         self._out_rows = max(1, 2 * self.expected_groups)
         self.async_update = bool(async_update)
         self._held = None
+        self._batch = None
         if async_update:
             N.check(N.lib().qe_hashagg_set_async(h, 1))
 
@@ -225,6 +226,13 @@
 
     def finalize(self) -> Tuple[List[DeviceColumn], List[DeviceColumn]]:
         nk = len(self.key_types)
+        batch, self._batch = getattr(self, "_batch", None), None
+        if batch is not None and batch[0] == self._version():
+            _, rows, cols, g = batch
+            _order_for_reader(self.ctx)
+            if g != rows:
+                cols = [_trim(c, g) for c in cols]
+            return cols[:nk], cols[nk:]
         out = N.C.c_int64(-1)
         stash, self._stash = getattr(self, "_stash", None), None
         if N.TYPE_UTF8 in self.key_types:
@@ -293,6 +301,40 @@
                                                 int(slot_records), N.C.byref(mx), N.C.byref(n)))
         return None if mx.value > slot_records else n.value
 
+    def _version(self) -> int:
+        v = N.C.c_uint64()
+        N.check(N.lib().qe_hashagg_version(self.handle, N.C.byref(v)))
+        return v.value
+
+    def _outputs_for_merge(self):
+        if N.TYPE_UTF8 in self.key_types:
+            return None
+        stash, self._stash = getattr(self, "_stash", None), None
+        return stash if stash is not None else self._carve_c(self._out_rows)
+
+    def _keep_batch(self, st: int, stash, groups: int) -> None:
+        rows, cols, _, _ = stash
+        if st == N.QE_ERR_CAPACITY and groups > rows:
+            self._out_rows = groups
+            return
+        N.check(st)
+        self._out_rows = max(1, groups)
+        self._batch = (self._version(), rows, cols, groups)
+
+    def import_slots_finalize(self, slots, nslots: int, slot_records: int) -> Optional[int]:
+        stash = self._outputs_for_merge()
+        if stash is None:
+            return self.import_slots(slots, nslots, slot_records)
+        mx, n, g = N.C.c_int64(), N.C.c_int64(), N.C.c_int64(-1)
+        st = N.lib().qe_hashagg_import_slots_finalize(self.handle, N.C.c_void_p(slots.data_ptr()), int(nslots),
+                                                      int(slot_records), stash[2], stash[3], N.C.byref(mx),
+                                                      N.C.byref(n), N.C.byref(g))
+        if st == N.QE_OK and mx.value > slot_records:
+            self._stash = stash
+            return None
+        self._keep_batch(st, stash, g.value)
+        return n.value
+
     def import_records(self, records, nrecords: int) -> None:
         if nrecords == 0:
             return
diff --git a/query-engines_amd/kquery/exchange.py b/query-engines_amd/kquery/exchange.py
--- a/query-engines_amd/kquery/exchange.py
+++ b/query-engines_amd/kquery/exchange.py
@@ -68,7 +68,7 @@
     cap = int(slot_records or partial.slot_capacity(world))
     recv = all_to_all_slots(partial.export_slots(world, cap), group)
     owner.prepare_output()
-    n = owner.import_slots(recv, world, cap)
+    n = owner.import_slots_finalize(recv, world, cap)
     if n is not None:
         return n
     recs, counts = partial.export(world)
@@ -114,7 +114,15 @@
 
     owner.prepare_output()
     n = N.C.c_int64()
-    N.check(N.lib().qe_hashagg_exchange(comm.handle, partial.handle, owner.handle, int(slot_records), N.C.byref(n)))
+    stash = owner._outputs_for_merge()
+    if stash is None:
+        N.check(N.lib().qe_hashagg_exchange(comm.handle, partial.handle, owner.handle, int(slot_records),
+                                            N.C.byref(n)))
+        return n.value
+    g = N.C.c_int64(-1)
+    st = N.lib().qe_hashagg_exchange_finalize(comm.handle, partial.handle, owner.handle, int(slot_records),
+                                              stash[2], stash[3], N.C.byref(n), N.C.byref(g))
+    owner._keep_batch(st, stash, g.value)
     return n.value
 
 
diff --git a/query-engines_amd/kquery/native.py b/query-engines_amd/kquery/native.py
--- a/query-engines_amd/kquery/native.py
+++ b/query-engines_amd/kquery/native.py
@@ -252,6 +252,9 @@
     ("qe_hashagg_import", C.c_int, [_P, _P, C.c_int64]),
     ("qe_hashagg_export_slots", C.c_int, [_P, C.c_int32, C.c_int64, _P]),
     ("qe_hashagg_import_slots", C.c_int, [_P, _P, C.c_int32, C.c_int64, _I64P, _I64P]),
+    ("qe_hashagg_import_slots_finalize", C.c_int,
+     [_P, _P, C.c_int32, C.c_int64, _COLP, _COLP, _I64P, _I64P, _I64P]),
+    ("qe_hashagg_version", C.c_int, [_P, C.POINTER(C.c_uint64)]),
     ("qe_hashagg_slot_capacity", C.c_int, [_P, C.c_int32, _I64P]),
     ("qe_hashagg_finalize_sizes", C.c_int, [_P, _I64P, _I64P]),
     ("qe_hashagg_export_keyed_sizes", C.c_int, [_P, C.c_int32, _I64P]),
@@ -268,6 +271,7 @@
     ("qe_comm_loopback_hub_destroy", C.c_int, [_P]),
     ("qe_comm_create_loopback", C.c_int, [_P, C.c_int32, C.c_int32, _P, C.POINTER(C.c_void_p)]),
     ("qe_hashagg_exchange", C.c_int, [_P, _P, _P, C.c_int64, _I64P]),
+    ("qe_hashagg_exchange_finalize", C.c_int, [_P, _P, _P, C.c_int64, _COLP, _COLP, _I64P, _I64P]),
     ("qe_hashagg_set_row_base", C.c_int, [_P, C.c_int64]),
     ("qe_hashagg_set_async", C.c_int, [_P, C.c_int32]),
     ("qe_hashagg_last_kernel_time", C.c_int, [_P, C.POINTER(C.c_double), C.POINTER(C.c_int32)]),
```

Result: no change. 277.6 billion rows/s, median of 2 (+1.2%).
